# Alexander-H-Liu/End-to-end-ASR-Pytorch

Hardware: AMD Instinct MI355X
Metric: audio frames/sec training (LAS+CTC, LibriSpeech 80-mel) (higher is better)
Workload: dtype f32; 1 GPU; cfg3: {"B": 32, "T": 1600, "D": 80, "V": 5000, "L": 64}; global_batch=32, parallelism=dp1

## Files before the change

### end-to-end-asr-pytorch_amd/_lib.py

```python
import ctypes
import os

_HERE = os.path.dirname(os.path.abspath(__file__))
LIB_PATH = os.path.join(_HERE, "csrc", "libasrk.so")

c_int, c_i64, c_f32, c_vp, c_sz = (ctypes.c_int, ctypes.c_int64, ctypes.c_float, ctypes.c_void_p,
                                   ctypes.c_size_t)
c_f64 = ctypes.c_double

SIGNATURES = {
    "asrk_version": (c_int, []),
    "asrk_strerror": (ctypes.c_char_p, [c_int]),
    "asrk_init": (c_int, [c_int]),
    "asrk_profile_enable": (None, [c_int]),
    "asrk_profile_families": (None, [ctypes.c_uint]),
    "asrk_profile_reset": (None, []),
    "asrk_profile_get": (c_int, [c_int, ctypes.POINTER(ctypes.c_double), ctypes.POINTER(c_i64)]),
    "asrk_profile_get_work": (c_int, [c_int, ctypes.POINTER(ctypes.c_double)]),
    "asrk_gemm_f32": (c_int, [c_int, c_int, c_int, c_int, c_int, c_f32, c_vp, c_int, c_vp, c_int,
                              c_f32, c_vp, c_int, c_vp, c_vp, c_int, c_int, c_vp, c_sz, c_vp]),
    "asrk_gemm_ws_bytes": (c_sz, [c_int, c_int, c_int, c_int]),
    "asrk_gemm_takes_split": (c_int, [c_int, c_int, c_int, c_int]),
    "asrk_gemm_plan_info": (c_int, [c_int, c_int, c_int, c_int, c_int, c_int, c_int, c_int, c_int, c_f32, c_int, c_int,
                                    c_int, c_vp]),
    "asrk_split_panel_bytes": (ctypes.c_size_t, [c_int, c_int, c_int]),
    "asrk_split_panel_f32": (c_int, [c_vp, c_int, c_int, c_int, c_int, c_vp, c_int, c_vp]),
    "asrk_gemm_panels_f32": (c_int, [c_int, c_int, c_int, c_f32, c_vp, c_int, c_int, c_int, c_int,
                                     c_vp, c_int, c_int, c_int, c_int, c_f32, c_vp, c_int, c_vp, c_vp, c_int, c_vp]),
    "asrk_gemm_panels_splitk_ws_bytes": (c_sz, [c_int, c_int, c_int]),
    "asrk_gemm_panels_splitk_f32": (c_int, [c_int, c_int, c_int, c_f32, c_vp, c_int, c_int, c_int, c_int,
                                            c_vp, c_int, c_int, c_int, c_int, c_f32, c_vp, c_int, c_vp, c_vp, c_int,
                                            c_vp, c_sz, c_int, c_vp]),
    "asrk_copy3d_f32": (c_int, [c_vp, c_vp, c_int, c_int, c_int, c_i64, c_i64, c_i64, c_i64, c_int,
                                c_vp]),
    "asrk_colsum_f32": (c_int, [c_vp, c_int, c_int, c_int, c_vp, c_int, c_vp]),
    "asrk_tanh_fwd_f32": (c_int, [c_vp, c_vp, c_i64, c_vp]),
    "asrk_tanh_bwd_f32": (c_int, [c_vp, c_vp, c_vp, c_i64, c_vp]),
    "asrk_log_softmax_fwd_f32": (c_int, [c_vp, c_vp, c_int, c_int, c_int, c_vp]),
    "asrk_log_softmax_bwd_f32": (c_int, [c_vp, c_vp, c_vp, c_int, c_int, c_int, c_vp]),
    "asrk_cross_entropy_fwd_f32": (c_int, [c_vp, c_int, c_int, c_int, c_vp, c_int, c_vp, c_vp, c_vp]),
    "asrk_cross_entropy_bwd_f32": (c_int, [c_vp, c_int, c_int, c_int, c_vp, c_int, c_vp, c_vp, c_vp,
                                           c_vp]),
    "asrk_cross_entropy_ls_fwd_f32": (c_int, [c_vp, c_int, c_int, c_int, c_vp, c_int, c_vp, c_vp, c_vp, c_vp]),
    "asrk_cross_entropy_ls_bwd_f32": (c_int, [c_vp, c_int, c_int, c_int, c_vp, c_int, c_f32, c_vp, c_vp, c_vp,
                                              c_vp]),
    "asrk_ctc_prefix_score_f32": (c_int, [c_vp, c_vp, c_vp, c_vp, c_vp, c_vp, c_vp, c_int, c_int, c_int,
                                          c_int, c_int, c_int, c_f32, c_vp]),
    "asrk_ctc_prefix_score_multi_f32": (c_int, [c_vp, c_vp, c_vp, c_vp, c_vp, c_vp, c_vp, c_vp, c_vp, c_int, c_int,
                                                c_int, c_int, c_int, c_int, c_int, c_f32, c_vp]),
    "asrk_ctc_prefix_beam_ws_bytes": (c_sz, [c_int, c_int]),
    "asrk_ctc_prefix_beam_ws_offsets": (c_int, [c_int, c_int, c_int] + [ctypes.POINTER(c_i64)] * 6),
    "asrk_ctc_prefix_beam_f32": (c_int, [c_vp, c_int, c_int, c_vp, c_int, c_int, c_vp, c_f32, c_int, c_int, c_int,
                                         c_int, c_int, c_vp, c_sz, c_vp]),
    "asrk_ctc_prefix_beam_multi_ws_bytes": (c_sz, [c_int, c_int, c_int, ctypes.POINTER(c_sz)]),
    "asrk_ctc_prefix_beam_multi_f32": (c_int, [c_vp, c_i64, c_int, c_int, c_int, c_vp, c_int, c_int, c_vp, c_f32,
                                               c_vp, c_vp, c_int, c_vp, c_vp, c_vp, c_vp, c_sz, c_vp]),
    "asrk_fbank_frames_f32": (c_int, [c_vp, c_i64, c_vp, c_vp, c_int, c_int, c_int, c_int, c_f32, c_int,
                                      c_vp]),
    "asrk_power_spectrum_f32": (c_int, [c_vp, c_vp, c_i64, c_int, c_vp]),
    "asrk_log_floor_f32": (c_int, [c_vp, c_i64, c_f32, c_vp]),
    "asrk_delta_f32": (c_int, [c_vp, c_vp, c_vp, c_int, c_int, c_int, c_int, c_vp]),
    "asrk_cmvn_f32": (c_int, [c_vp, c_vp, c_int, c_int, c_f32, c_vp]),
    "asrk_transpose_f32": (c_int, [c_vp, c_vp, c_int, c_int, c_vp]),
    "asrk_fbank_frames_batch_f32": (c_int, [c_vp, c_int, c_i64, c_vp, c_vp, c_int, c_int, c_vp, c_vp, c_int, c_int,
                                            c_int, c_f32, c_f32, c_int, c_vp]),
    "asrk_delta_cmvn_batch_f32": (c_int, [c_vp, c_vp, c_int, c_int, c_vp, c_int, c_int, c_int, c_f32, c_vp, c_int,
                                          c_vp]),
    "asrk_fbank_logmel_batch_f32": (c_int, [c_vp, c_int, c_i64, c_vp, c_vp, c_int, c_int, c_vp, c_vp, c_vp, c_vp, c_vp,
                                            c_int, c_int, c_vp, c_int, c_int, c_int, c_f32, c_f32, c_int, c_f32, c_vp]),
    "asrk_fbank_frames_dither_f32": (c_int, [c_vp, c_i64, c_vp, c_vp, c_int, c_int, c_int, c_int, c_f32, c_int, c_f32,
                                             ctypes.c_uint64, c_vp]),
    "asrk_fbank_frames_batch_dither_f32": (c_int, [c_vp, c_int, c_i64, c_vp, c_vp, c_int, c_int, c_vp, c_vp, c_int,
                                                   c_int, c_int, c_f32, c_f32, c_int, c_f32, c_vp, c_vp]),
    "asrk_fbank_logmel_batch_dither_f32": (c_int, [c_vp, c_int, c_i64, c_vp, c_vp, c_int, c_int, c_vp, c_vp, c_vp, c_vp,
                                                   c_vp, c_int, c_int, c_vp, c_int, c_int, c_int, c_f32, c_f32, c_int,
                                                   c_f32, c_f32, c_vp, c_vp]),
    "asrk_spec_augment_f32": (c_int, [c_vp, c_vp, c_int, c_int, c_int, c_int, c_int, c_vp, c_vp, c_int, c_int, c_f32,
                                      c_vp]),
    "asrk_resample_rows_f32": (c_int, [c_vp, c_int, c_i64, c_vp, c_vp, c_vp, c_vp, c_int, c_vp, c_vp, c_int, c_vp, c_i64,
                                       c_f32, c_vp]),
    "asrk_reverb_mix_ws_bytes": (c_sz, [c_int, c_i64]),
    "asrk_reverb_mix_f32": (c_int, [c_vp, c_int, c_i64, c_vp, c_vp, c_vp, c_i64, c_vp, c_vp, c_vp, c_vp, c_int, c_vp,
                                    c_vp, c_vp, c_i64, c_vp, c_vp, c_vp, c_int, c_vp, c_i64, c_f32, c_vp, c_sz, c_vp]),
    "asrk_lstm_ws_bytes": (c_sz, []),
    "asrk_lstm_xchg_bytes": (c_sz, [c_int, c_int, c_int, c_int, c_int, c_int]),
    "asrk_lstm_plan_workgroups": (c_int, [c_int, c_int, c_int, c_int, c_int, c_int]),
    "asrk_lstm_plan_info": (c_int, [c_int, c_int, c_int, c_int, c_int, c_int, c_int, c_vp]),
    "asrk_lstm_rec_fwd_f32": (c_int, [c_vp, c_vp, c_vp, c_vp, c_vp, c_int, c_int, c_int, c_int,
                                      c_vp, c_int, c_vp, c_int, c_vp]),
    "asrk_lstm_rec_bwd_f32": (c_int, [c_vp, c_vp, c_vp, c_vp, c_vp, c_int, c_int, c_int, c_int,
                                      c_vp, c_int, c_vp, c_vp, c_int, c_vp]),
    "asrk_lstm_rec_fwd_pyr_f32": (c_int, [c_vp, c_vp, c_vp, c_vp, c_vp, c_int, c_int, c_int, c_int,
                                          c_vp, c_int, c_vp, c_vp, c_int, c_int, c_int, c_vp]),
    "asrk_lstm_rec_fwd_len_f32": (c_int, [c_vp, c_vp, c_vp, c_vp, c_vp, c_vp, c_int, c_int, c_int, c_int,
                                          c_vp, c_int, c_vp, c_vp, c_int, c_int, c_int, c_vp]),
    "asrk_lstm_rec_bwd_pyr_f32": (c_int, [c_vp, c_vp, c_vp, c_vp, c_vp, c_int, c_int, c_int, c_int,
                                          c_vp, c_int, c_vp, c_vp, c_int, c_int, c_int, c_vp]),
    "asrk_lstm_plan_is_bf": (c_int, [c_int, c_int, c_int, c_int, c_int, c_int]),
    "asrk_lstm_rec_fwd_pyr_panel_f32": (c_int, [c_vp, c_vp, c_vp, c_vp, c_vp, c_int, c_int, c_int, c_int,
                                                c_vp, c_int, c_vp, c_vp, c_int, c_int, c_vp, c_int, c_vp]),
    "asrk_lstm_rec_bwd_pyr_panel_f32": (c_int, [c_vp, c_vp, c_vp, c_vp, c_vp, c_int, c_int, c_int, c_int,
                                                c_vp, c_int, c_vp, c_vp, c_int, c_int, c_vp, c_vp, c_int, c_vp]),
    "asrk_gru_rec_fwd_f32": (c_int, [c_vp, c_vp, c_vp, c_vp, c_int, c_int, c_int, c_int,
                                     c_vp, c_int, c_vp, c_vp, c_int, c_int, c_int, c_vp]),
    "asrk_gru_rec_bwd_f32": (c_int, [c_vp, c_vp, c_vp, c_vp, c_vp, c_int, c_int, c_int, c_int,
                                     c_vp, c_int, c_vp, c_vp, c_int, c_int, c_int, c_vp]),
    "asrk_lstm_check_error": (c_int, [c_vp, c_vp]),
    "asrk_loc_conv_fwd_f32": (c_int, [c_vp, c_vp, c_vp, c_int, c_int, c_int, c_int, c_int, c_vp]),
    "asrk_loc_conv_bwd_f32": (c_int, [c_vp, c_vp, c_vp, c_vp, c_vp, c_int, c_int, c_int, c_int, c_int,
                                      c_vp]),
    "asrk_attn_energy_fwd_f32": (c_int, [c_int, c_vp, c_vp, c_vp, c_vp, c_vp, c_vp, c_vp, c_vp, c_vp,
                                         c_int, c_int, c_int, c_int, c_int, c_f32, c_vp]),
    "asrk_attn_energy_bwd_f32": (c_int, [c_int, c_vp, c_vp, c_vp, c_vp, c_vp, c_vp, c_vp, c_vp, c_vp,
                                         c_vp, c_vp, c_vp, c_vp, c_vp, c_int, c_int, c_int, c_int,
                                         c_int, c_f32, c_vp]),
    "asrk_attn_context_fwd_f32": (c_int, [c_vp, c_vp, c_vp, c_int, c_int, c_int, c_i64, c_vp]),
    "asrk_attn_context_bwd_f32": (c_int, [c_vp, c_vp, c_vp, c_int, c_int, c_int, c_i64, c_vp]),
    "asrk_lstm_cell_fwd_f32": (c_int, [c_vp, c_vp, c_vp, c_vp, c_int, c_int, c_vp]),
    "asrk_lstm_cell_bwd_f32": (c_int, [c_vp, c_vp, c_vp, c_vp, c_vp, c_vp, c_int, c_int, c_vp]),
    "asrk_gru_cell_fwd_f32": (c_int, [c_vp, c_vp, c_i64, c_i64, c_vp, c_i64, c_vp, c_i64, c_int, c_int, c_vp]),
    "asrk_gru_cell_bwd_f32": (c_int, [c_vp, c_vp, c_i64, c_i64, c_vp, c_i64, c_vp, c_i64, c_vp, c_vp, c_i64,
                                      c_int, c_int, c_vp]),
    "asrk_embedding_fwd_f32": (c_int, [c_vp, c_vp, c_vp, c_i64, c_int, c_int, c_vp]),
    "asrk_embedding_bwd_f32": (c_int, [c_vp, c_vp, c_vp, c_i64, c_int, c_int, c_vp]),
    "asrk_emb_fuse_bwd_ws_bytes": (c_sz, [c_int] * 6),
    "asrk_emb_fuse_fwd_f32": (c_int, [c_vp, c_int, c_vp, c_vp, c_int, c_vp, c_int, c_int, c_f32, c_int, c_int, c_vp,
                                      c_vp, c_vp]),
    "asrk_emb_fuse_bwd_f32": (c_int, [c_vp, c_vp, c_int, c_vp, c_vp, c_int, c_vp, c_int, c_int, c_f32, c_vp, c_int,
                                      c_int, c_vp, c_vp, c_vp, c_vp, c_vp, c_sz, c_vp]),
    "asrk_cos_emb_loss_fwd_f32": (c_int, [c_vp, c_vp, c_i64, c_vp, c_int, c_int, c_int, c_vp, c_vp, c_vp, c_vp]),
    "asrk_cos_emb_loss_bwd_f32": (c_int, [c_vp, c_vp, c_i64, c_vp, c_int, c_int, c_int, c_vp, c_vp, c_vp, c_vp, c_vp]),
    "asrk_cos_emb_table_grad_f32": (c_int, [c_vp, c_vp, c_int, c_int, c_i64, c_vp, c_vp]),
    "asrk_nll_loss_fwd_f32": (c_int, [c_vp, c_int, c_int, c_int, c_vp, c_int, c_vp, c_vp]),
    "asrk_nll_loss_bwd_f32": (c_int, [c_int, c_int, c_int, c_vp, c_int, c_vp, c_vp, c_vp]),
    "asrk_l2norm_fwd_f32": (c_int, [c_vp, c_vp, c_vp, c_int, c_int, c_f32, c_vp]),
    "asrk_l2norm_bwd_f32": (c_int, [c_vp, c_vp, c_vp, c_vp, c_int, c_int, c_f32, c_vp]),
    "asrk_layer_norm_fwd_f32": (c_int, [c_vp, c_vp, c_vp, c_vp, c_vp, c_vp, c_int, c_int, c_f32, c_vp]),
    "asrk_layer_norm_bwd_f32": (c_int, [c_vp, c_vp, c_vp, c_vp, c_vp, c_vp, c_vp, c_vp, c_int, c_int,
                                        c_vp]),
    "asrk_dropout_f32": (c_int, [c_vp, c_vp, c_i64, c_f32, ctypes.c_uint64, ctypes.c_uint64, c_vp]),
    "asrk_adadelta_step_f32": (c_int, [c_vp, c_vp, c_vp, c_vp, c_i64, c_f64, c_f64, c_f64, c_vp, c_vp]),
    "asrk_adadelta_multi_f32": (c_int, [c_int, c_vp, c_vp, c_vp, c_vp, c_vp, c_f64, c_f64, c_f64, c_vp, c_vp]),
    "asrk_adam_multi_f32": (c_int, [c_int, c_vp, c_vp, c_vp, c_vp, c_vp, c_f64, c_f64, c_f64, c_f64, c_i64,
                                    c_vp, c_vp]),
    "asrk_adam_step_f32": (c_int, [c_vp, c_vp, c_vp, c_vp, c_i64, c_f64, c_f64, c_f64, c_f64, c_i64, c_vp,
                                   c_vp]),
    "asrk_token_crop_i64": (c_int, [c_vp, c_i64, c_int, c_int, c_i64, c_i64, c_int, c_vp, c_i64, c_vp, c_vp]),
    "asrk_edit_distance_i64": (c_int, [c_vp, c_i64, c_vp, c_vp, c_i64, c_vp, c_int, c_int, c_vp, c_vp]),
    "asrk_grad_norm_ws_bytes": (c_sz, [c_int, c_vp]),
    "asrk_grad_norm_multi_f32": (c_int, [c_int, c_vp, c_vp, c_f32, c_vp, c_vp, c_vp, c_sz, c_vp]),
    "asrk_fill_f32": (c_int, [c_vp, c_i64, c_f32, c_vp]),
    "asrk_topk_f32": (c_int, [c_vp, c_int, c_int, c_int, c_int, c_vp, c_vp, c_vp]),
    "asrk_beam_select_f32": (c_int, [c_vp] * 4 + [c_int] * 6 + [c_vp] * 19 + [c_vp]),
    "asrk_gather_rows_multi_f32": (c_int, [c_int, c_vp, c_vp, c_vp, c_vp, c_vp, c_vp, c_vp, c_int, c_vp]),
    "asrk_conv_out_size": (c_int, [c_int, c_int, c_int, c_int]),
    "asrk_im2col_f32": (c_int, [c_vp, c_vp] + [c_int] * 10 + [c_i64] * 4 + [c_vp]),
    "asrk_im2col_ld_f32": (c_int, [c_vp, c_vp] + [c_int] * 11 + [c_i64] * 4 + [c_vp]),
    "asrk_col2im_f32": (c_int, [c_vp, c_vp] + [c_int] * 10 + [c_i64] * 4 + [c_vp]),
    "asrk_im2col_cl_f32": (c_int, [c_vp, c_vp] + [c_int] * 10 + [c_i64] * 4 + [c_vp]),
    "asrk_col2im_cl_f32": (c_int, [c_vp, c_vp] + [c_int] * 10 + [c_i64] * 4 + [c_vp]),
    "asrk_conv_weight_reorder_f32": (c_int, [c_vp, c_vp, c_int, c_int, c_int, c_int, c_vp]),
    "asrk_conv3x3_supported": (c_int, [c_int] * 4),
    "asrk_conv3x3_plan_info": (c_int, [c_int] * 6 + [c_vp, c_int]),
    "asrk_conv3x3_weight_f32": (c_int, [c_vp, c_vp, c_int, c_int, c_int, c_vp]),
    "asrk_conv3x3_f32": (c_int, [c_vp] * 5 + [c_int] * 6 + [c_vp]),
    "asrk_conv3x3_wgrad_ws_bytes": (c_sz, [c_int] * 5),
    "asrk_conv3x3_wgrad_f32": (c_int, [c_vp] * 5 + [c_int] * 5 + [c_vp, c_sz, c_vp]),
    "asrk_conv3x3_first_supported": (c_int, [c_int] * 4),
    "asrk_conv3x3_first_f32": (c_int, [c_vp] * 4 + [c_int] * 5 + [c_i64] * 4 + [c_int, c_vp]),
    "asrk_conv3x3_len_f32": (c_int, [c_vp] * 5 + [c_int] * 6 + [c_vp]),
    "asrk_conv3x3_first_len_f32": (c_int, [c_vp] * 5 + [c_int] * 5 + [c_i64] * 4 + [c_int, c_vp]),
    "asrk_im2col_ld_len_f32": (c_int, [c_vp] * 3 + [c_int] * 11 + [c_i64] * 4 + [c_vp]),
    "asrk_im2col_cl_len_f32": (c_int, [c_vp] * 3 + [c_int] * 10 + [c_i64] * 4 + [c_vp]),
    "asrk_conv_zero_tail_f32": (c_int, [c_vp, c_vp, c_int, c_int, c_i64, c_vp]),
    "asrk_conv3x3_first_wgrad_ws_bytes": (c_sz, [c_int] * 5),
    "asrk_conv3x3_first_wgrad_f32": (c_int, [c_vp] * 5 + [c_int] * 5 + [c_i64] * 4 + [c_vp, c_sz, c_vp]),
    "asrk_relu_fwd_f32": (c_int, [c_vp, c_i64, c_vp]),
    "asrk_relu_bwd_f32": (c_int, [c_vp, c_vp, c_vp, c_i64, c_vp]),
    "asrk_maxpool2x2_fwd_f32": (c_int, [c_vp, c_vp, c_vp] + [c_int] * 4 + [c_i64] * 4 + [c_vp]),
    "asrk_maxpool2x2_bwd_f32": (c_int, [c_vp, c_vp, c_vp] + [c_int] * 4 + [c_i64] * 4 + [c_vp]),
    "asrk_speller_plan": (c_int, [c_vp, ctypes.POINTER(c_int), ctypes.POINTER(c_int)]),
    "asrk_speller_plan_info": (c_int, [c_vp, ctypes.POINTER(c_int)]),
    "asrk_speller_ctx_variant": (c_int, [c_vp, ctypes.POINTER(c_int)]),
    "asrk_speller_fwd_f32": (c_int, [c_vp, c_vp]),
    "asrk_speller_bwd_f32": (c_int, [c_vp, c_vp, c_vp]),
    "asrk_speller_step_f32": (c_int, [c_vp, c_int, c_vp, c_i64, c_vp, c_vp]),
    "asrk_speller_dvalue_f32": (c_int, [c_vp, c_i64, c_i64, c_vp, c_i64, c_i64, c_vp, c_int, c_int, c_int,
                                        c_int, c_vp]),
    "asrk_joint_score_f32": (c_int, [c_vp, c_vp, c_vp, c_vp, c_vp, c_vp, c_int, c_int, c_int, c_f64, c_f64,
                                     c_f64, c_vp]),
    "asrk_lstm_cell_fused_f32": (c_int, [c_vp, c_i64, c_int, c_vp, c_vp, c_vp, c_vp, c_vp, c_vp, c_vp, c_vp, c_int,
                                         c_int, c_vp]),
    "asrk_transpose_ld_f32": (c_int, [c_vp, c_i64, c_vp, c_i64, c_int, c_int, c_vp]),
    "asrk_flac_info": (c_int, [ctypes.c_char_p, ctypes.POINTER(c_int), ctypes.POINTER(c_int), ctypes.POINTER(c_int),
                               ctypes.POINTER(c_i64), c_vp]),
    "asrk_flac_decode_i32": (c_int, [ctypes.c_char_p, c_vp, c_i64, ctypes.POINTER(c_i64)]),
    "asrk_ctc_loss_fwd_f32": (c_int, [c_vp, c_i64, c_i64, c_int, c_int, c_int, c_vp, c_i64, c_int,
                                      c_vp, c_vp, c_int, c_vp, c_vp, c_vp, c_vp, c_vp]),
    "asrk_ctc_loss_bwd_f32": (c_int, [c_vp, c_i64, c_i64, c_int, c_int, c_int, c_vp, c_i64, c_int,
                                      c_vp, c_vp, c_int, c_vp, c_vp, c_vp, c_vp, c_vp, c_vp, c_i64,
                                      c_i64, c_vp]),
    "asrk_ctc_loss_fwd_ex_f32": (c_int, [c_vp, c_i64, c_i64, c_int, c_int, c_int, c_vp, c_i64, c_int,
                                         c_vp, c_vp, c_int, c_vp, c_vp, c_vp, c_vp, c_int, c_vp, c_vp, c_vp]),
    "asrk_ctc_loss_bwd_ex_f32": (c_int, [c_vp, c_i64, c_i64, c_int, c_int, c_int, c_vp, c_i64, c_int,
                                         c_vp, c_vp, c_int, c_vp, c_vp, c_vp, c_vp, c_vp, c_vp, c_i64,
                                         c_i64, c_int, c_vp]),
    "asrk_ctc_align_ws_bytes": (c_sz, [c_int, c_int, c_int, c_int]),
    "asrk_ctc_align_f32": (c_int, [c_vp, c_i64, c_i64, c_int, c_int, c_int, c_vp, c_i64, c_int, c_vp, c_vp, c_int,
                                   c_int, c_vp, c_vp, c_vp, c_vp, c_vp, c_vp, c_sz, c_vp]),
}

_lib = None


class AsrkError(RuntimeError):
    pass


def load():
    global _lib
    if _lib is not None:
        return _lib
    if not os.path.exists(LIB_PATH):
        raise AsrkError(
            "libasrk.so not found at %s - build it with `python __graft_entry__.py` "
            "(hipcc --offload-arch=gfx950). There is no CPU fallback for the product path." % LIB_PATH)
    try:
        import torch
    except ImportError:
        pass
    lib = ctypes.CDLL(LIB_PATH)
    for name, (res, args) in SIGNATURES.items():
        fn = getattr(lib, name)
        fn.restype = res
        fn.argtypes = args
    _lib = lib
    return lib


def strerror(rc):
    return load().asrk_strerror(int(rc)).decode()


def check(rc, what=""):
    if rc != 0:
        raise AsrkError("%s failed: %s (rc=%d)" % (what or "asrk call", strerror(rc), rc))
```

### end-to-end-asr-pytorch_amd/csrc/lstm_rec.hip

```cpp
#include "lstm_rec_common.h"

extern "C" int asrk_cu_count_(void);
extern "C" size_t asrk_split_panel_stride_(int rows, int K);

using namespace asrk_rec;

namespace {

__global__ __launch_bounds__(256) void sentinel_fill_kernel(u32x4 *__restrict__ p, size_t n16) {
    const u32x4 v = {0xFFFFFFFFu, 0xFFFFFFFFu, 0xFFFFFFFFu, 0xFFFFFFFFu};
    for (size_t base = (size_t)blockIdx.x * 1024; base < n16; base += (size_t)gridDim.x * 1024) {
#pragma unroll
        for (int u = 0; u < 4; ++u) {
            const size_t i = base + u * 256 + threadIdx.x;
            if (i < n16) p[i] = v;
        }
    }
}

inline int sentinel_fill(void *xchg, size_t floats, hipStream_t s) {
    const size_t n16 = floats / 4;
    if (n16 * 4 != floats || (reinterpret_cast<uintptr_t>(xchg) & 15) != 0)
        return (int)hipMemsetAsync(xchg, 0xFF, floats * 4, s);
    hipLaunchKernelGGL(sentinel_fill_kernel, dim3(2048), dim3(256), 0, s, reinterpret_cast<u32x4 *>(xchg), n16);
    return (int)hipGetLastError();
}

__global__ __launch_bounds__(256) void sentinel_fill_tail_kernel(u32x4 *__restrict__ x, int groups, int T, int r0,
                                                                 unsigned step16) {
    const u32x4 v = {0xFFFFFFFFu, 0xFFFFFFFFu, 0xFFFFFFFFu, 0xFFFFFFFFu};
    const unsigned n = (unsigned)(T - r0) * step16;
    const int g = blockIdx.y;
    u32x4 *q = x + ((size_t)g * T + r0) * step16;
    for (unsigned i = blockIdx.x * 256 + threadIdx.x; i < n; i += gridDim.x * 256) q[i] = v;
}

inline int sentinel_fill_tail(void *xchg, int groups, int T, size_t step_floats, hipStream_t s) {
    const int r0 = std::max(0, T - 2);
    const unsigned step16 = (unsigned)(step_floats / 4);
    const unsigned n = (unsigned)(T - r0) * step16;
    hipLaunchKernelGGL(sentinel_fill_tail_kernel, dim3(std::max(1u, std::min(64u, (n + 1023) / 1024)), groups), dim3(256),
                       0, s, reinterpret_cast<u32x4 *>(xchg), groups, T, r0, step16);
    return (int)hipGetLastError();
}

inline int canary_words(int nwg) { return ((4 * nwg + 63) / 64) * 64; }

unsigned long long *g_dbg_buf = nullptr;
int g_dbg_steps = 0;

inline void chunk_groups(int ndir, int nbg, int gmax, int &ndir_l, int &nbg_l, int &launches) {
    ndir_l = gmax >= ndir ? ndir : 1;
    nbg_l = std::max(1, std::min(nbg, gmax / ndir_l));
    launches = ((ndir + ndir_l - 1) / ndir_l) * ((nbg + nbg_l - 1) / nbg_l);
}

FwdPlan plan_fwd(int T, int B, int H, int ndir, int ncu, int flags) {
    const AsrkKnobs &kn = asrk_knobs_();
    FwdPlan best{};
    best.ok = false;
    long best_cost = -1;
    const int kg = (H + 15) / 16;
    const int kgw_need = (kg + 3) / 4;
    const int KGW = kgw_need <= 4 ? 4 : kgw_need <= 8 ? 8 : kgw_need <= 16 ? 16 : 0;
    if (!KGW) return best;
    const int HP = KGW * 4 * 16 + 8;
    static const int combos[6][2] = {{1, 1}, {1, 2}, {2, 1}, {2, 2}, {1, 4}, {4, 1}};
    const int oc = 1;
    for (auto &c : combos) {
        const int MT = c[0], NT = c[1];
        if (kn.is_set(kn.fwd_mt) && kn.fwd_mt != MT) continue;
        if (kn.is_set(kn.fwd_nt) && kn.fwd_nt != NT) continue;
        const int U = 4 * MT, BG = 16 * NT;
        const int nwg = (H + U - 1) / U, nbg = (B + BG - 1) / BG;
        const long wgs = (long)ndir * nbg * nwg;
        if (wgs > (long)ncu * oc) continue;
        const size_t red1 = (size_t)4 * MT * NT * RED_PITCH * 16;
        size_t lds = (size_t)MT * 16 * HP * 4 + 2 * red1 + 16;
        int db = 1;
        const size_t lds_cap = (size_t)158 * 1024 / (wgs > ncu ? oc : 1);
        if (lds > lds_cap) {
            lds -= red1;
            db = 0;
        }
        if (lds > lds_cap) continue;
        const long cost = (long)MT * NT * 1000 - nbg;
        if (best_cost < 0 || cost < best_cost) {
            best_cost = cost;
            best = FwdPlan{MT, NT, KGW, U, nwg, nbg, BG, HP, kg, db, lds,
                           (size_t)ndir * nbg * T * ((size_t)kg * NT * 256 + canary_words(nwg)), true,
                           ndir, nbg};
        }
    }
    if (best.ok) {
        const bool no_bf = (flags & ASRK_REC_F32_MFMA) != 0;
        if (!no_bf && best.MT == 2 && (H == 512 || H == 1024)) {
            const size_t wl = (size_t)2 * 2 * (H / 32) * 1024;
            const size_t red1 = (size_t)4 * 2 * best.NT * RED_PITCH * 16;
            size_t lds = wl + 2 * red1 + 16;
            int db = 1;
            if (lds > (size_t)158 * 1024) { lds -= red1; db = 0; }
            if (lds <= (size_t)158 * 1024) {
                best.bf = 1;
                best.db = db;
                best.lds = lds;
                best.xfloats = (size_t)ndir * best.nbg * T *
                               ((size_t)(H / 32) * best.NT * 3 * 256 + canary_words(best.nwg));
            }
            const bool no16 = kn.get(kn.rec_bf_mt4, 1) == 0;
            const int nbg16 = (B + 15) / 16;
            if (best.bf && !no16 && H == 1024 && (long)ndir * nbg16 * (H / 16) <= ncu) {
                best.MT = 4; best.NT = 1; best.U = 16; best.BG = 16;
                best.nwg = H / 16; best.nbg = nbg16; best.ndir_l = ndir; best.nbg_l = nbg16;
                best.db = 0;
                best.lds = (size_t)4 * (H / 32) * 1024 + (size_t)4 * 4 * RED_PITCH * 16 + 16;
                best.xfloats = (size_t)ndir * nbg16 * T * ((size_t)(H / 32) * 3 * 256 + canary_words(best.nwg));
            }
        }
        return best;
    }
    for (auto &c : combos) {
        const int MT = c[0], NT = c[1];
        const int U = 4 * MT, BG = 16 * NT;
        const int nwg = (H + U - 1) / U, nbg = (B + BG - 1) / BG;
        if (nwg > ncu) continue;
        const size_t red1 = (size_t)4 * MT * NT * RED_PITCH * 16;
        size_t lds = (size_t)MT * 16 * HP * 4 + 2 * red1 + 16;
        int db = 1;
        if (lds > (size_t)158 * 1024) { lds -= red1; db = 0; }
        if (lds > (size_t)158 * 1024) continue;
        int ndir_l, nbg_l, launches;
        chunk_groups(ndir, nbg, ncu / nwg, ndir_l, nbg_l, launches);
        const long cost = (long)launches * MT * NT * 1000;
        if (best_cost < 0 || cost < best_cost) {
            best_cost = cost;
            best = FwdPlan{MT, NT, KGW, U, nwg, nbg, BG, HP, kg, db, lds,
                           (size_t)ndir_l * nbg_l * T * ((size_t)kg * NT * 256 + canary_words(nwg)), true,
                           ndir_l, nbg_l};
        }
    }
    return best;
}


inline size_t bwd_lds(int kg, int UB, int NT, int RK, int &HPb, int &KP) {
    const int CH = bwd_ring_kgroups(NT, RK);
    HPb = ((kg - RK + CH - 1) / CH) * CH * 16;
    KP = 4 * HPb + 8;
    return (size_t)UB * KP * 4 + (size_t)HPb * 4 + (size_t)2 * 4 * NT * RED_PITCH * 16 + 16;
}
inline int bwd_rk_options(int kg, int H, int NT, int (&opts)[2]) {
    opts[0] = 0;
    const int kg_plain = (H & 15) ? kg - 1 : kg;
    if (NT == 1 && 32 + bwd_ring_kgroups(1, 32) <= kg_plain) {
        opts[1] = 32;
        return 2;
    }
    return 1;
}

BwdPlan plan_bwd(int T, int B, int H, int ndir, int ncu, int flags) {
    const AsrkKnobs &kn = asrk_knobs_();
    BwdPlan best{};
    best.ok = false;
    const int kg = (H + 15) / 16;
    static const int ubs[3] = {16, 8, 4};
    static const int nts[3] = {1, 2, 4};
    const int oc = 1;
    for (int UB : ubs) {
        if (kn.is_set(kn.bwd_ub) && kn.bwd_ub != UB) continue;
        for (int NT : nts) {
            if (kn.is_set(kn.bwd_nt) && kn.bwd_nt != NT) continue;
            int rks[2];
            const int nrk = bwd_rk_options(kg, H, NT, rks);
            for (int ri = 0; ri < nrk; ++ri) {
                const int RK = rks[ri];
                int HPb, KP;
                const size_t lds = bwd_lds(kg, UB, NT, RK, HPb, KP);
                const int BG = 16 * NT;
                const int nwg = (H + UB - 1) / UB, nbg = (B + BG - 1) / BG;
                const long wgs = (long)ndir * nbg * nwg;
                if (wgs > (long)ncu * oc) continue;
                if (lds > (size_t)158 * 1024 / (wgs > ncu ? oc : 1)) continue;
                best = BwdPlan{NT, UB, nwg, nbg, BG, HPb, KP, kg, lds,
                               (size_t)ndir * nbg * T * ((size_t)4 * kg * NT * 256 + canary_words(nwg)),
                               true, ndir, nbg, RK};
                const bool no_bf = (flags & ASRK_REC_F32_MFMA) != 0;
                if (!no_bf && NT == 1 && UB == 16 && BG == 16 && (H == 512 || H == 1024)) {
                    const int KS = H / 32, KL = H == 1024 ? 11 : 0;
                    best.bf = 1;
                    best.lds = (size_t)4 * KL * 3 * 1024 + (size_t)2 * 4 * RED_PITCH * 16 + 2 * 6144 + 16;
                    best.xfloats = (size_t)ndir * nbg * T * ((size_t)4 * KS * 3 * 256 + canary_words(nwg));
                }
                return best;
            }
        }
    }
    long best_cost = -1;
    for (int UB : ubs) {
        for (int NT : nts) {
            int rks[2];
            const int nrk = bwd_rk_options(kg, H, NT, rks);
            for (int ri = 0; ri < nrk; ++ri) {
                const int RK = rks[ri];
                int HPb, KP;
                const size_t lds = bwd_lds(kg, UB, NT, RK, HPb, KP);
                const int BG = 16 * NT;
                const int nwg = (H + UB - 1) / UB, nbg = (B + BG - 1) / BG;
                if (nwg > ncu || lds > (size_t)158 * 1024) continue;
                int ndir_l, nbg_l, launches;
                chunk_groups(ndir, nbg, ncu / nwg, ndir_l, nbg_l, launches);
                const long cost = (long)launches * NT * 1000 + (16 / UB);
                if (best_cost < 0 || cost < best_cost) {
                    best_cost = cost;
                    best = BwdPlan{NT, UB, nwg, nbg, BG, HPb, KP, kg, lds,
                                   (size_t)ndir_l * nbg_l * T * ((size_t)4 * kg * NT * 256 + canary_words(nwg)),
                                   true, ndir_l, nbg_l, RK};
                }
            }
        }
    }
    return best;
}

int rec_fwd_impl(bool gru, float *G, const float *whh_f, const float *whh_r, float *Y, float *C, int T, int B,
                 int H, int ndir, void *xchg, int xchg_prefilled, void *ws, float *Y2, int pyr_mode,
                 int pyr_rate, int flags, void *stream, const int64_t *lens = nullptr, void *x2_panel = nullptr);
int rec_bwd_impl(bool gru, float *gates, const float *whh_f, const float *whh_r, const float *C,
                 const float *dY, int T, int B, int H, int ndir, void *xchg, int xchg_prefilled, void *ws,
                 float *db, int pyr_mode, int pyr_rate, int flags, void *stream, void *dg_panel = nullptr,
                 void *dgt_panel = nullptr);

}


extern "C" void asrk_lstm_set_debug_(void *buf, int steps) {
    g_dbg_buf = reinterpret_cast<unsigned long long *>(buf);
    g_dbg_steps = steps;
}

extern "C" size_t asrk_lstm_ws_bytes(void) { return WS_WORDS * sizeof(unsigned); }

extern "C" int asrk_lstm_plan_workgroups(int T, int B, int H, int ndir, int backward, int flags) {
    int info[ASRK_LSTM_PLAN_INFO_LEN];
    return asrk_lstm_plan_info(T, B, H, ndir, backward, flags, 0, info) == ASRK_OK ? info[11] : 0;
}

extern "C" size_t asrk_lstm_xchg_bytes(int T, int B, int H, int ndir, int backward, int flags) {
    int info[ASRK_LSTM_PLAN_INFO_LEN];
    if (asrk_lstm_plan_info(T, B, H, ndir, backward, flags, 0, info) != ASRK_OK) return 0;
    return ((size_t)info[13] << 31) | (size_t)info[12];
}

extern "C" int asrk_lstm_rec_fwd_f32(float *G, const float *whh_f, const float *whh_r, float *Y,
                                     float *C, int T, int B, int H, int ndir, void *xchg,
                                     int xchg_prefilled, void *ws, int flags, void *stream) {
    return asrk_lstm_rec_fwd_pyr_f32(G, whh_f, whh_r, Y, C, T, B, H, ndir, xchg, xchg_prefilled, ws, nullptr,
                                     0, 1, flags, stream);
}

extern "C" int asrk_lstm_rec_fwd_pyr_f32(float *G, const float *whh_f, const float *whh_r, float *Y,
                                         float *C, int T, int B, int H, int ndir, void *xchg,
                                         int xchg_prefilled, void *ws, float *Y2, int pyr_mode,
                                         int pyr_rate, int flags, void *stream) {
    if (!C) return ASRK_EINVAL;
    return rec_fwd_impl(false, G, whh_f, whh_r, Y, C, T, B, H, ndir, xchg, xchg_prefilled, ws, Y2, pyr_mode,
                        pyr_rate, flags, stream);
}

extern "C" int asrk_lstm_rec_fwd_pyr_panel_f32(float *G, const float *whh_f, const float *whh_r, float *Y,
                                               float *C, int T, int B, int H, int ndir, void *xchg,
                                               int xchg_prefilled, void *ws, float *Y2, int pyr_mode,
                                               int pyr_rate, void *x2_panel, int flags, void *stream) {
    if (!C || !x2_panel) return ASRK_EINVAL;
    return rec_fwd_impl(false, G, whh_f, whh_r, Y, C, T, B, H, ndir, xchg, xchg_prefilled, ws, Y2, pyr_mode,
                        pyr_rate, flags, stream, nullptr, x2_panel);
}

extern "C" int asrk_lstm_plan_is_bf(int T, int B, int H, int ndir, int backward, int flags) {
    int info[ASRK_LSTM_PLAN_INFO_LEN];
    return asrk_lstm_plan_info(T, B, H, ndir, backward, flags, 0, info) == ASRK_OK ? info[0] : 0;
}

extern "C" int asrk_lstm_plan_info(int T, int B, int H, int ndir, int backward, int flags, int ncu, int *info) {
    if (!info || ncu < 0) return ASRK_EINVAL;
    for (int i = 0; i < ASRK_LSTM_PLAN_INFO_LEN; ++i) info[i] = 0;
    if (flags < 0) return ASRK_EINVAL;
    if (T < 0 || B <= 0 || H <= 0 || (ndir != 1 && ndir != 2)) return ASRK_EINVAL;
    if (T == 0) return ASRK_OK;
    if (H % 4 != 0) return ASRK_ESHAPE;
    if (ncu == 0) ncu = asrk_cu_count_();
    if (ncu <= 0) return ASRK_EDEVICE;
    int nbg_l, ndir_l, nbg;
    size_t xbytes;
    if (backward) {
        const BwdPlan pl = plan_bwd(T, B, H, ndir, ncu, flags);
        if (!pl.ok) return ASRK_ESHAPE;
        info[0] = pl.bf; info[1] = pl.UB; info[2] = pl.NT; info[3] = pl.bf ? 0 : pl.RK; info[4] = 0;
        info[8] = pl.nwg; info[10] = (int)pl.lds;
        ndir_l = pl.ndir_l; nbg_l = pl.nbg_l; nbg = pl.nbg; xbytes = pl.xfloats * 4;
    } else {
        const FwdPlan pl = plan_fwd(T, B, H, ndir, ncu, flags);
        if (!pl.ok) return ASRK_ESHAPE;
        info[0] = pl.bf; info[1] = pl.MT; info[2] = pl.NT; info[3] = pl.bf ? H / 128 : pl.KGW; info[4] = pl.db;
        info[8] = pl.nwg; info[10] = (int)pl.lds;
        ndir_l = pl.ndir_l; nbg_l = pl.nbg_l; nbg = pl.nbg; xbytes = pl.xfloats * 4;
    }
    info[5] = ((ndir + ndir_l - 1) / ndir_l) * ((nbg + nbg_l - 1) / nbg_l);
    info[6] = ndir_l; info[7] = nbg_l; info[9] = nbg;
    info[11] = ndir_l * nbg_l * info[8];
    info[12] = (int)(xbytes & 0x7fffffffu); info[13] = (int)(xbytes >> 31);
    info[14] = ncu;
    return ASRK_OK;
}

extern "C" int asrk_lstm_rec_fwd_len_f32(float *G, const float *whh_f, const float *whh_r, float *Y,
                                         float *C, const int64_t *lens, int T, int B, int H, int ndir, void *xchg,
                                         int xchg_prefilled, void *ws, float *Y2, int pyr_mode,
                                         int pyr_rate, int flags, void *stream) {
    if (!C || !lens) return ASRK_EINVAL;
    return rec_fwd_impl(false, G, whh_f, whh_r, Y, C, T, B, H, ndir, xchg, xchg_prefilled, ws, Y2, pyr_mode,
                        pyr_rate, flags, stream, lens);
}

extern "C" int asrk_gru_rec_fwd_f32(float *G, const float *whh_f, const float *whh_r, float *Y, int T, int B,
                                    int H, int ndir, void *xchg, int xchg_prefilled, void *ws, float *Y2,
                                    int pyr_mode, int pyr_rate, int flags, void *stream) {
    return rec_fwd_impl(true, G, whh_f, whh_r, Y, nullptr, T, B, H, ndir, xchg, xchg_prefilled, ws, Y2,
                        pyr_mode, pyr_rate, flags, stream);
}

extern "C" int asrk_gru_rec_bwd_f32(float *gates, const float *whh_f, const float *whh_r, const float *Y,
                                    const float *dY, int T, int B, int H, int ndir, void *xchg,
                                    int xchg_prefilled, void *ws, float *db, int pyr_mode, int pyr_rate,
                                    int flags, void *stream) {
    return rec_bwd_impl(true, gates, whh_f, whh_r, Y, dY, T, B, H, ndir, xchg, xchg_prefilled, ws, db,
                        pyr_mode, pyr_rate, flags, stream);
}

namespace {
int rec_fwd_impl(bool gru, float *G, const float *whh_f, const float *whh_r, float *Y, float *C, int T, int B,
                 int H, int ndir, void *xchg, int xchg_prefilled, void *ws, float *Y2, int pyr_mode,
                 int pyr_rate, int flags, void *stream, const int64_t *lens, void *x2_panel) {
    const AsrkKnobs &kn = asrk_knobs_();
    if (flags < 0 || pyr_mode < 0 || pyr_mode > 2 || pyr_rate < 1) return ASRK_EINVAL;
    const bool y2_empty = pyr_mode == 1 && T / pyr_rate == 0;
    if (pyr_mode != 0 && !Y2 && !y2_empty) return ASRK_EINVAL;
    if (T < 0 || B <= 0 || H <= 0 || (ndir != 1 && ndir != 2)) return ASRK_EINVAL;
    if (T == 0) return ASRK_OK;
    if (!G || !whh_f || (ndir == 2 && !whh_r) || !Y || (!gru && !C) || !ws || !xchg) return ASRK_EINVAL;
    if (H % 4 != 0) return ASRK_ESHAPE;
    if ((reinterpret_cast<uintptr_t>(xchg) & 15) != 0) return ASRK_EINVAL;
    const int ncu = asrk_cu_count_();
    if (ncu <= 0) return ASRK_EDEVICE;
    FwdPlan pl = plan_fwd(T, B, H, ndir, ncu, flags);
    if (!pl.ok) return ASRK_ESHAPE;
    hipStream_t s = (hipStream_t)stream;
    RecFwdArgs a;
    a.G = G; a.whh[0] = whh_f; a.whh[1] = ndir == 2 ? whh_r : whh_f;
    a.Y = Y; a.C = C; a.X = reinterpret_cast<float *>(xchg);
    a.err = reinterpret_cast<unsigned *>(ws);
    a.T = T; a.B = B; a.H = H; a.ldg = ndir * 4 * H; a.ldy = ndir * H;
    a.U = pl.U; a.nwg = pl.nwg; a.BG = pl.BG; a.HP = pl.HP; a.kgp = pl.kgp;
    a.canw = canary_words(pl.nwg);
    a.poll_mode = kn.get(kn.fwd_poll, 0);
    a.poll_mode |= (kn.get(kn.fwd_presleep, 8) & 0xff) << 8;
    a.dbg = g_dbg_buf; a.dbg_steps = kn.is_set(kn.dbg_noload) ? -1 : g_dbg_steps;
    a.Y2 = pyr_mode ? Y2 : nullptr; a.pyr_mode = pyr_mode; a.pyr_rate = pyr_rate;
    a.lens = lens;
    a.P2 = nullptr; a.p2_stride = 0;
    if (x2_panel) {
        if (!pl.bf || pyr_mode == 2 || lens || (ndir * H) % 8 != 0 || (reinterpret_cast<uintptr_t>(x2_panel) & 15))
            return ASRK_ESHAPE;
        const int r = pyr_mode == 1 ? pyr_rate : 1;
        a.P2 = reinterpret_cast<unsigned char *>(x2_panel);
        a.p2_stride = asrk_split_panel_stride_((T / r) * B, r * ndir * H);
        if (pyr_mode == 0) { a.pyr_rate = 1; }
    }
    const bool one_launch = pl.ndir_l >= ndir && pl.nbg_l >= pl.nbg;
    a.rearm = (flags & ASRK_REC_REARM) && one_launch ? 1 : 0;
    asrk_prof_begin_(PROF_LSTM_FWD, s);
    int rc = ASRK_OK;
    bool first = true;
    for (int d0 = 0; d0 < ndir && rc == ASRK_OK; d0 += pl.ndir_l)
        for (int g0 = 0; g0 < pl.nbg && rc == ASRK_OK; g0 += pl.nbg_l) {
            a.ndir = std::min(pl.ndir_l, ndir - d0);
            a.nbg = std::min(pl.nbg_l, pl.nbg - g0);
            a.dir0 = d0; a.bg0 = g0;
            if (!(first && xchg_prefilled)) { const int frc = sentinel_fill(xchg, pl.xfloats, s); if (frc) return frc; }
            first = false;
            const int grid = a.ndir * a.nbg * pl.nwg;
            rc = pl.bf ? launch_fwd_bf(gru, a, pl, H, grid, s) : launch_fwd_f32(gru, a, pl, grid, s);
        }
    if (rc == ASRK_OK && (flags & ASRK_REC_REARM)) {
        const int frc = a.rearm ? sentinel_fill_tail(xchg, ndir * pl.nbg, T, pl.xfloats / ((size_t)ndir * pl.nbg * T), s)
                                : sentinel_fill(xchg, pl.xfloats, s);
        if (frc) rc = frc;
    }
    asrk_prof_end_(PROF_LSTM_FWD, s);
    return rc;
}
}

extern "C" int asrk_lstm_rec_bwd_f32(float *gates, const float *whh_f, const float *whh_r,
                                     const float *C, const float *dY, int T, int B, int H, int ndir,
                                     void *xchg, int xchg_prefilled, void *ws, float *db, int flags, void *stream) {
    return asrk_lstm_rec_bwd_pyr_f32(gates, whh_f, whh_r, C, dY, T, B, H, ndir, xchg, xchg_prefilled, ws, db,
                                     0, 1, flags, stream);
}

extern "C" int asrk_lstm_rec_bwd_pyr_f32(float *gates, const float *whh_f, const float *whh_r,
                                         const float *C, const float *dY, int T, int B, int H, int ndir,
                                         void *xchg, int xchg_prefilled, void *ws, float *db,
                                         int pyr_mode, int pyr_rate, int flags, void *stream) {
    return rec_bwd_impl(false, gates, whh_f, whh_r, C, dY, T, B, H, ndir, xchg, xchg_prefilled, ws, db,
                        pyr_mode, pyr_rate, flags, stream);
}

extern "C" int asrk_lstm_rec_bwd_pyr_panel_f32(float *gates, const float *whh_f, const float *whh_r,
                                               const float *C, const float *dY, int T, int B, int H, int ndir,
                                               void *xchg, int xchg_prefilled, void *ws, float *db,
                                               int pyr_mode, int pyr_rate, void *dg_panel, void *dgt_panel, int flags,
                                               void *stream) {
    if (!dg_panel && !dgt_panel) return ASRK_EINVAL;
    return rec_bwd_impl(false, gates, whh_f, whh_r, C, dY, T, B, H, ndir, xchg, xchg_prefilled, ws, db,
                        pyr_mode, pyr_rate, flags, stream, dg_panel, dgt_panel);
}

namespace {
int rec_bwd_impl(bool gru, float *gates, const float *whh_f, const float *whh_r, const float *C,
                 const float *dY, int T, int B, int H, int ndir, void *xchg, int xchg_prefilled, void *ws,
                 float *db, int pyr_mode, int pyr_rate, int flags, void *stream, void *dg_panel, void *dgt_panel) {
    const AsrkKnobs &kn = asrk_knobs_();
    if (flags < 0 || pyr_mode < 0 || pyr_mode > 2 || pyr_rate < 1) return ASRK_EINVAL;
    const bool dy_empty = pyr_mode == 1 && T / pyr_rate == 0;
    if (T < 0 || B <= 0 || H <= 0 || (ndir != 1 && ndir != 2)) return ASRK_EINVAL;
    if (T == 0) return ASRK_OK;
    if (!gates || !whh_f || (ndir == 2 && !whh_r) || !C || (!dY && !dy_empty) || !ws || !xchg) return ASRK_EINVAL;
    if (H % 4 != 0) return ASRK_ESHAPE;
    if ((reinterpret_cast<uintptr_t>(xchg) & 15) != 0) return ASRK_EINVAL;
    const int ncu = asrk_cu_count_();
    if (ncu <= 0) return ASRK_EDEVICE;
    BwdPlan pl = plan_bwd(T, B, H, ndir, ncu, flags);
    if (!pl.ok) return ASRK_ESHAPE;
    hipStream_t s = (hipStream_t)stream;
    RecBwdArgs a;
    a.G = gates; a.whh[0] = whh_f; a.whh[1] = ndir == 2 ? whh_r : whh_f;
    a.C = C; a.dY = dY; a.X = reinterpret_cast<float *>(xchg);
    a.err = reinterpret_cast<unsigned *>(ws);
    a.T = T; a.B = B; a.H = H; a.ldg = ndir * 4 * H; a.ldy = ndir * H;
    a.UB = pl.UB; a.nwg = pl.nwg; a.BG = pl.BG; a.HPb = pl.HPb; a.KP = pl.KP;
    a.kgp = pl.kgp; a.canw = canary_words(pl.nwg);
    a.poll_mode = kn.get(kn.bwd_poll, 1);
    if (kn.is_set(kn.bwd_presleep)) a.poll_mode |= (kn.bwd_presleep & 0xff) << 8;
    a.dbg = g_dbg_buf; a.dbg_steps = kn.is_set(kn.dbg_noload) ? -1 : g_dbg_steps;
    a.db = db;
    a.pyr_mode = pyr_mode; a.pyr_rate = pyr_rate;
    a.PG = nullptr; a.pg_stride = 0;
    if (dg_panel) {
        if (!pl.bf || gru || (reinterpret_cast<uintptr_t>(dg_panel) & 15)) return ASRK_ESHAPE;
        a.PG = reinterpret_cast<unsigned char *>(dg_panel);
        a.pg_stride = asrk_split_panel_stride_(T * B, ndir * 4 * H);
    }
    a.PT = nullptr; a.pt_stride = 0;
    if (dgt_panel) {
        if (!pl.bf || gru || B % 16 != 0 || (reinterpret_cast<uintptr_t>(dgt_panel) & 15)) return ASRK_ESHAPE;
        a.PT = reinterpret_cast<unsigned char *>(dgt_panel);
        a.pt_stride = asrk_split_panel_stride_(ndir * 4 * H, T * B);
    }
    const bool one_launch = pl.ndir_l >= ndir && pl.nbg_l >= pl.nbg;
    a.rearm = (flags & ASRK_REC_REARM) && one_launch ? 1 : 0;
    a.no_dg = (flags & ASRK_REC_BWD_NO_DG) && (dg_panel || dgt_panel) ? 1 : 0;
    if (db) ASRK_HIP(hipMemsetAsync(db, 0, (size_t)ndir * 4 * H * sizeof(float), s));
    asrk_prof_begin_(PROF_LSTM_BWD, s);
    int rc = ASRK_OK;
    bool first = true;
    for (int d0 = 0; d0 < ndir && rc == ASRK_OK; d0 += pl.ndir_l)
        for (int g0 = 0; g0 < pl.nbg && rc == ASRK_OK; g0 += pl.nbg_l) {
            a.ndir = std::min(pl.ndir_l, ndir - d0);
            a.nbg = std::min(pl.nbg_l, pl.nbg - g0);
            a.dir0 = d0; a.bg0 = g0;
            if (!(first && xchg_prefilled)) { const int frc = sentinel_fill(xchg, pl.xfloats, s); if (frc) return frc; }
            first = false;
            const int grid = a.ndir * a.nbg * pl.nwg;
            rc = pl.bf ? launch_bwd_bf(gru, a, pl, grid, s) : launch_bwd_f32(gru, a, pl, grid, s);
        }
    if (rc == ASRK_OK && (flags & ASRK_REC_REARM)) {
        const int frc = a.rearm ? sentinel_fill_tail(xchg, ndir * pl.nbg, T, pl.xfloats / ((size_t)ndir * pl.nbg * T), s)
                                : sentinel_fill(xchg, pl.xfloats, s);
        if (frc) rc = frc;
    }
    asrk_prof_end_(PROF_LSTM_BWD, s);
    return rc;
}
}

extern "C" int asrk_lstm_check_error(void *ws, void *stream) {
    if (!ws) return ASRK_EINVAL;
    hipStream_t s = (hipStream_t)stream;
    unsigned e = 0;
    unsigned *errp = reinterpret_cast<unsigned *>(ws);
    ASRK_HIP(hipMemcpyAsync(&e, errp, sizeof(unsigned), hipMemcpyDeviceToHost, s));
    ASRK_HIP(hipStreamSynchronize(s));
    if (e != 0) {
        ASRK_HIP(hipMemsetAsync(errp, 0, sizeof(unsigned), s));
        return ASRK_ETIMEOUT;
    }
    return ASRK_OK;
}
```

### end-to-end-asr-pytorch_amd/csrc/lstm_rec_bwd_bf.hip

```cpp
#include "lstm_rec_common.h"

namespace asrk_rec {
namespace {

template <bool GRU, int KS, int NREG>
__global__ __launch_bounds__(256) void lstm_rec_bwd_bf_kernel(RecBwdArgs p) {
    extern __shared__ __attribute__((aligned(16))) float smem[];
    constexpr int CH = 8;
    constexpr int KL = KS - NREG;
    constexpr int KQ = KS / 4;
    static_assert(KS >= CH, "ring longer than the slice");
    static_assert(KS % 4 == 0, "unit range of a wave is a whole number of k-steps");
    const int tid = threadIdx.x, lane = tid & 63, wave = __builtin_amdgcn_readfirstlane(tid >> 6);
    const int ngroups = p.ndir * p.nbg;
    const int group = blockIdx.x % ngroups, wg = blockIdx.x / ngroups;
    const int dir = p.dir0 + group % p.ndir, bg = p.bg0 + group / p.ndir;
    const int u0 = wg * 16, b0 = bg * 16;
    const int nb = min(16, p.B - b0);
    const int H = p.H;

    unsigned char *Wl = reinterpret_cast<unsigned char *>(smem);
    f32x4 *red = reinterpret_cast<f32x4 *>(Wl + (size_t)4 * KL * 3 * 1024);
    unsigned char *stage = reinterpret_cast<unsigned char *>(red + 2 * 4 * RED_PITCH);
    unsigned char *stage_t = stage + 4 * 3 * 2 * 16 * 16;
    int *abort_flag = reinterpret_cast<int *>(stage_t + 4 * 3 * 2 * 16 * 16);

    const int m16 = lane & 15, q4 = lane >> 4;
    bf16x8_t areg[NREG > 0 ? NREG : 1][3];
    {
        const float *W = p.whh[dir];
#pragma unroll
        for (int js = 0; js < KS; ++js) {
            const int gate = js / KQ;
            const bool live = !GRU || gate < 3;
            unsigned h0[8], h1[8], h2[8];
#pragma unroll
            for (int e = 0; e < 8; ++e) {
                const int j = (wave * KQ + js % KQ) * 32 + q4 * 8 + e;
                split3(live ? W[((size_t)gate * H + j) * H + u0 + m16] : 0.f, h0[e], h1[e], h2[e]);
            }
            u32x4 w0, w1, w2;
#pragma unroll
            for (int q = 0; q < 4; ++q) {
                w0[q] = h0[2 * q] | (h0[2 * q + 1] << 16);
                w1[q] = h1[2 * q] | (h1[2 * q + 1] << 16);
                w2[q] = h2[2 * q] | (h2[2 * q + 1] << 16);
            }
            if (js < NREG) {
                areg[js][0] = __builtin_bit_cast(bf16x8_t, w0);
                areg[js][1] = __builtin_bit_cast(bf16x8_t, w1);
                areg[js][2] = __builtin_bit_cast(bf16x8_t, w2);
            } else {
                unsigned char *d = Wl + ((size_t)((wave * KL + (js - NREG)) * 3) * 64 + lane) * 16;
                *reinterpret_cast<u32x4 *>(d) = w0;
                *reinterpret_cast<u32x4 *>(d + 1024) = w1;
                *reinterpret_cast<u32x4 *>(d + 2048) = w2;
            }
        }
        if (tid == 0) *abort_flag = 0;
    }
    __syncthreads();
    const unsigned char *a_lds = Wl + ((size_t)(wave * KL * 3) * 64 + lane) * 16;

    const int ul = tid & 15, bl = tid >> 4;
    const int c_unit = u0 + ul, c_b = b0 + bl;
    const bool c_valid = bl < nb;
    const int c_red = (red_slot((ul >> 2) * 16 + bl)) * 4 + (ul & 3);
    float dc_carry = 0.f;
    float dbsum[4] = {0.f, 0.f, 0.f, 0.f};

    const size_t gate_floats = (size_t)KS * 3 * 256;
    const size_t data_floats = 4 * gate_floats;
    const size_t step_floats = data_floats + (size_t)p.canw;
    float *xgroup = p.X + (size_t)group * p.T * step_floats;
    const unsigned voff = (m16 < nb && p.dbg_steps != -1) ? (unsigned)(lane * 16) : 0x7ff00000u;
    const unsigned frag_base = (unsigned)(wave * KQ * 3 * 1024);
    auto frag_off = [](int js) { return (unsigned)(((js / KQ) * KS + js % KQ) * 3 * 1024); };
    const int can_lo = wave * p.nwg, can_cnt = p.nwg;
    unsigned char *st_w = stage + (ul >> 3) * 256 + bl * 16 + (ul & 7) * 2;
    unsigned char *st_t = stage_t + (bl >> 3) * 256 + ul * 16 + (bl & 7) * 2;
    int pt_src[2];
    size_t pt_dst[2];
    int pt_half[2];
    bool pt_on[2];
#pragma unroll
    for (int i = 0; i < 2; ++i) {
        const int idx = tid + 256 * i;
        const int u = idx & 15, rest = idx >> 4, hb = rest & 1, gp = rest >> 1;
        const int r = gp / 3, pl = gp - r * 3;
        pt_on[i] = idx < 384;
        pt_src[i] = ((gp * 2 + hb) * 16 + u) * 16;
        const int row = (dir * 4 + r) * H + u0 + u;
        pt_dst[i] = (size_t)(row >> 6) * p.pt_stride + (size_t)pl * 1024 + (row & 63) * 16;
        pt_half[i] = hb;
    }
    const int xks = u0 >> 5, xq4 = (u0 & 31) >> 3;
    int ch_src[2], pg_row[2];
    unsigned ch_dst[2];
    size_t pg_col[2];
    bool ch_on[2];
#pragma unroll
    for (int i = 0; i < 2; ++i) {
        const int idx = lane + 64 * i;
        const int nl = idx / 24, c = idx - nl * 24, n = wave * 4 + nl;
        const int r = c / 6, pl = (c % 6) >> 1, half = c & 1;
        ch_on[i] = idx < 96 && n < nb;
        ch_src[i] = ((r * 3 + pl) * 2 + half) * 256 + n * 16;
        ch_dst[i] = (unsigned)((((r * KS + xks) * 3 + pl) * 64 + (xq4 + half) * 16 + n) * 16);
        pg_row[i] = b0 + n;
        pg_col[i] = (size_t)((((dir * 4 + r) * H + u0 + half * 8) >> 3) * 3 + pl) * 1024;
    }

    for (int s = 0; s < p.T; ++s) {
        const int t = dir == 0 ? p.T - 1 - s : s;
        const int tp = dir == 0 ? t - 1 : t + 1;

        float vi = 0.f, vf = 0.f, vg = 0.f, vo = 0.f, vc = 0.f, vcp = 0.f, vdy = 0.f;
        if (c_valid) {
            const size_t row = (size_t)t * p.B + c_b;
            const float *g = p.G + row * p.ldg + dir * 4 * H + c_unit;
            vi = g[0];
            vf = g[(size_t)H];
            vg = g[(size_t)2 * H];
            vo = g[(size_t)3 * H];
            vc = p.C[row * p.ldy + dir * H + c_unit];
            if (p.pyr_mode == 0) {
                vdy = p.dY[row * p.ldy + dir * H + c_unit];
            } else {
                const int r = p.pyr_rate, tq = t / r, tr = t - tq * r;
                if (p.pyr_mode == 1 ? tq < p.T / r : tr == 0) {
                    const size_t ld2 = p.pyr_mode == 1 ? (size_t)r * p.ldy : (size_t)p.ldy;
                    const size_t off = p.pyr_mode == 1 ? (size_t)tr * p.ldy : 0;
                    vdy = p.dY[((size_t)tq * p.B + c_b) * ld2 + off + dir * H + c_unit];
                }
            }
            if (tp >= 0 && tp < p.T) vcp = p.C[((size_t)tp * p.B + c_b) * p.ldy + dir * H + c_unit];
        }

        f32x4 acc[3];
        acc[0] = acc[1] = acc[2] = f32x4{0.f, 0.f, 0.f, 0.f};

        auto mfma6 = [&](const bf16x8_t (&a)[3], const u32x4 (&b)[3]) {
            acc[0] = __builtin_amdgcn_mfma_f32_16x16x32_bf16(a[2], __builtin_bit_cast(bf16x8_t, b[0]), acc[0], 0, 0, 0);
            acc[1] = __builtin_amdgcn_mfma_f32_16x16x32_bf16(a[1], __builtin_bit_cast(bf16x8_t, b[1]), acc[1], 0, 0, 0);
            acc[2] = __builtin_amdgcn_mfma_f32_16x16x32_bf16(a[0], __builtin_bit_cast(bf16x8_t, b[2]), acc[2], 0, 0, 0);
            acc[0] = __builtin_amdgcn_mfma_f32_16x16x32_bf16(a[1], __builtin_bit_cast(bf16x8_t, b[0]), acc[0], 0, 0, 0);
            acc[1] = __builtin_amdgcn_mfma_f32_16x16x32_bf16(a[0], __builtin_bit_cast(bf16x8_t, b[1]), acc[1], 0, 0, 0);
            acc[2] = __builtin_amdgcn_mfma_f32_16x16x32_bf16(a[0], __builtin_bit_cast(bf16x8_t, b[0]), acc[2], 0, 0, 0);
        };
        auto a_frag = [&](bf16x8_t (&a)[3], int js) {
            if (js < NREG) {
                a[0] = areg[js][0]; a[1] = areg[js][1]; a[2] = areg[js][2];
            } else {
                const unsigned char *q = a_lds + (size_t)(js - NREG) * 3 * 1024;
                a[0] = *reinterpret_cast<const bf16x8_t *>(q);
                a[1] = *reinterpret_cast<const bf16x8_t *>(q + 1024);
                a[2] = *reinterpret_cast<const bf16x8_t *>(q + 2048);
            }
        };

        REC_STAMP(0);
        if (s > 0) {
            __amdgpu_buffer_rsrc_t rs = __builtin_amdgcn_make_buffer_rsrc(
                (void *)(xgroup + (size_t)(s - 1) * step_floats), 0, (int)(step_floats * 4), 0x00020000);
            u32x4 bf[CH][3];
            unsigned spins = 0;
            unsigned long long t0 = 0;
            bool ok = true;
            for (int z = (p.poll_mode >> 8) & 0xff; z > 0; z -= 8) __builtin_amdgcn_s_sleep(8);
            ok = wait_canaries(reinterpret_cast<const unsigned *>(
                                       xgroup + (size_t)(s - 1) * step_floats + data_floats) + can_lo,
                               can_cnt, p.err, lane, p.poll_mode);
            REC_STAMP(7);
            bool bad = false;
            if (ok) {
#pragma unroll
                for (int c = 0; c < CH; ++c)
#pragma unroll
                    for (int pl = 0; pl < 3; ++pl)
                        bf[c][pl] = __builtin_amdgcn_raw_buffer_load_b128(
                            rs, voff, frag_base + frag_off(c) + (unsigned)(pl * 1024), 0);
                __builtin_amdgcn_sched_barrier(0);
                REC_STAMP(1);
#pragma unroll
                for (int js = 0; js < KS; ++js) {
                    bf16x8_t a[3];
                    a_frag(a, js);
                    mfma6(a, bf[js % CH]);
                    __builtin_amdgcn_sched_barrier(0);
                    if (js + CH < KS) {
#pragma unroll
                        for (int pl = 0; pl < 3; ++pl)
                            bf[js % CH][pl] = __builtin_amdgcn_raw_buffer_load_b128(
                                rs, voff, frag_base + frag_off(js + CH) + (unsigned)(pl * 1024), 0);
                        __builtin_amdgcn_sched_barrier(0);
                    }
                }
            }
            bad = any_nan(acc[0] + acc[1] + acc[2]);
            if (ok && __any(bad)) {
                acc[0] = acc[1] = acc[2] = f32x4{0.f, 0.f, 0.f, 0.f};
#pragma unroll
                for (int c0 = 0; c0 < KS; c0 += CH) {
                    while (ok) {
#pragma unroll
                        for (int c = 0; c < CH; ++c)
#pragma unroll
                            for (int pl = 0; pl < 3; ++pl)
                                bf[c][pl] = __builtin_amdgcn_raw_buffer_load_b128(
                                    rs, voff, frag_base + frag_off(c0 + c) + (unsigned)(pl * 1024), 16);
                        __builtin_amdgcn_sched_barrier(0);
                        bool b2 = false;
#pragma unroll
                        for (int c = 0; c < CH; ++c)
#pragma unroll
                            for (int pl = 0; pl < 3; ++pl) b2 |= has_sentinel(__builtin_bit_cast(f32x4, bf[c][pl]));
                        if (!__any(b2)) break;
                        if (!spin_ok(spins, t0, p.err, lane)) ok = false;
                    }
                    if (ok) {
#pragma unroll
                        for (int c = 0; c < CH; ++c) {
                            bf16x8_t a[3];
                            a_frag(a, c0 + c);
                            mfma6(a, bf[c]);
                        }
                    }
                }
            }
            if (!ok && lane == 0) *abort_flag = 1;
        }
        REC_STAMP(2);
        f32x4 *redw = red + (s & 1) * 4 * RED_PITCH;
        redw[wave * RED_PITCH + red_slot(lane)] = acc[0] + acc[1] + acc[2];
        REC_STAMP(3);
        __syncthreads();
        if (*abort_flag) break;
        REC_STAMP(4);

        const float *redf = reinterpret_cast<const float *>(redw);
        float *xstep = xgroup + (size_t)s * step_floats;
        float dgs[4] = {0.f, 0.f, 0.f, 0.f}, xg[4] = {0.f, 0.f, 0.f, 0.f};
        if (c_valid) {
            float rec = 0.f;
#pragma unroll
            for (int w = 0; w < 4; ++w) rec += redf[w * RED_PITCH * 4 + c_red];
            if (GRU) {
                const float dh = vdy + rec + dc_carry;
                const float r = vi, z = vf, n = vg, hn = vo, hp = vcp;
                const float dn = dh * (1.f - z) * (1.f - n * n);
                const float dz = dh * (hp - n) * z * (1.f - z);
                const float dr = dn * hn * r * (1.f - r);
                dc_carry = dh * z;
                dgs[0] = dr; dgs[1] = dz; dgs[2] = dn; dgs[3] = dn * r;
                xg[0] = dr; xg[1] = dz; xg[2] = dn * r; xg[3] = 0.f;
            } else {
                const float dh = vdy + rec;
                const float tc = fast_tanh(vc);
                const float dcell = dh * vo * (1.f - tc * tc) + dc_carry;
                dc_carry = dcell * vf;
                dgs[0] = dcell * vg * vi * (1.f - vi);
                dgs[1] = dcell * vcp * vf * (1.f - vf);
                dgs[2] = dcell * vi * (1.f - vg * vg);
                dgs[3] = dh * tc * vo * (1.f - vo);
#pragma unroll
                for (int r = 0; r < 4; ++r) xg[r] = dgs[r];
            }
#pragma unroll
            for (int r = 0; r < 4; ++r) dbsum[r] += dgs[r];
        }
#pragma unroll
        for (int r = 0; r < 4; ++r) {
            unsigned h0, h1, h2;
            split3(xg[r], h0, h1, h2);
            *reinterpret_cast<unsigned short *>(st_w + (r * 3 + 0) * 512) = (unsigned short)h0;
            *reinterpret_cast<unsigned short *>(st_w + (r * 3 + 1) * 512) = (unsigned short)h1;
            *reinterpret_cast<unsigned short *>(st_w + (r * 3 + 2) * 512) = (unsigned short)h2;
            if (!GRU && p.PT) {
                *reinterpret_cast<unsigned short *>(st_t + (r * 3 + 0) * 512) = (unsigned short)h0;
                *reinterpret_cast<unsigned short *>(st_t + (r * 3 + 1) * 512) = (unsigned short)h1;
                *reinterpret_cast<unsigned short *>(st_t + (r * 3 + 2) * 512) = (unsigned short)h2;
            }
        }
        __builtin_amdgcn_fence(__ATOMIC_RELEASE, "wavefront");
        __builtin_amdgcn_wave_barrier();
        __builtin_amdgcn_fence(__ATOMIC_ACQUIRE, "wavefront");
        {
            __amdgpu_buffer_rsrc_t xrs = __builtin_amdgcn_make_buffer_rsrc(
                (void *)xstep, 0, (int)(step_floats * 4), 0x00020000);
            u32x4 v[2];
#pragma unroll
            for (int i = 0; i < 2; ++i)
                if (ch_on[i]) {
                    v[i] = *reinterpret_cast<const u32x4 *>(stage + ch_src[i]);
                    __builtin_amdgcn_raw_buffer_store_b128(v[i], xrs, ch_dst[i], 0, 16);
                }
            if (lane == 0)
                __hip_atomic_store(reinterpret_cast<unsigned *>(xstep + data_floats) + 4 * wg + wave,
                                   (unsigned)(s + 1), RLX_AGENT);
            if (!GRU && p.PG) {
#pragma unroll
                for (int i = 0; i < 2; ++i)
                    if (ch_on[i]) {
                        const int m = t * p.B + pg_row[i];
                        *reinterpret_cast<u32x4 *>(p.PG + (size_t)(m >> 6) * p.pg_stride + pg_col[i] + (m & 63) * 16) = v[i];
                    }
            }
        }
        REC_STAMP(5);
        if (c_valid && !p.no_dg) {
            float *g = p.G + ((size_t)t * p.B + c_b) * p.ldg + dir * 4 * H + c_unit;
#pragma unroll
            for (int r = 0; r < 4; ++r) g[(size_t)r * H] = dgs[r];
        }
        if (!GRU && p.PT) {
            __syncthreads();
#pragma unroll
            for (int i = 0; i < 2; ++i)
                if (pt_on[i]) {
                    const int c = (t * p.B + b0 + pt_half[i] * 8) >> 3;
                    *reinterpret_cast<u32x4 *>(p.PT + pt_dst[i] + (size_t)c * 3072) =
                        *reinterpret_cast<const u32x4 *>(stage_t + pt_src[i]);
                }
        }
        if (p.rearm && s >= 2)
            rearm_region(xgroup + (size_t)(s - 2) * step_floats, step_floats, wg, p.nwg, tid, (int)blockDim.x);
        REC_STAMP(6);
    }
    if (p.db && !*abort_flag) {
        __syncthreads();
        float *sdb = reinterpret_cast<float *>(red);
#pragma unroll
        for (int r = 0; r < 4; ++r) sdb[tid * 4 + r] = c_valid ? dbsum[r] : 0.f;
        __syncthreads();
        if (tid < 64) {
            const int u = tid & 15, r = tid >> 4;
            float a = 0.f;
            for (int b = 0; b < 16; ++b) a += sdb[(b * 16 + u) * 4 + r];
            unsafeAtomicAdd(p.db + (size_t)dir * 4 * H + (size_t)r * H + u0 + u, a);
        }
    }
}

template <bool GRU, int KS, int NREG>
int launch_bwd_bf(const RecBwdArgs &a, int grid, size_t lds, hipStream_t s) {
    auto kern = lstm_rec_bwd_bf_kernel<GRU, KS, NREG>;
    ASRK_HIP(hipFuncSetAttribute(reinterpret_cast<const void *>(kern),
                                 hipFuncAttributeMaxDynamicSharedMemorySize, (int)lds));
    hipLaunchKernelGGL(kern, dim3(grid), dim3(256), lds, s, a);
    ASRK_LAUNCH_CHECK();
    return ASRK_OK;
}

}

int launch_bwd_bf(bool gru, const RecBwdArgs &a, const BwdPlan &pl, int grid, hipStream_t s) {
    if (a.H == 1024) return gru ? launch_bwd_bf<true, 32, 21>(a, grid, pl.lds, s) : launch_bwd_bf<false, 32, 21>(a, grid, pl.lds, s);
    return gru ? launch_bwd_bf<true, 16, 16>(a, grid, pl.lds, s) : launch_bwd_bf<false, 16, 16>(a, grid, pl.lds, s);
}

}
```

### end-to-end-asr-pytorch_amd/csrc/lstm_rec_common.h

```cpp
#pragma once
#include "common.h"
#include "knobs.h"
#include <algorithm>
#include <cstdlib>

namespace asrk_rec {

constexpr int WS_WORDS = 1024;
constexpr unsigned SENT = 0xFFFFFFFFu;
constexpr unsigned long long TIMEOUT_TICKS = 300000000ull;

struct RecFwdArgs {
    float *G;
    const float *whh[2];
    float *Y, *C;
    float *X;
    unsigned *err;
    int T, B, H, ndir, ldg, ldy;
    int U, nwg, nbg, BG, HP, kgp, canw, poll_mode;
    int dir0, bg0;
    unsigned long long *dbg;
    int dbg_steps;
    float *Y2;
    int pyr_mode, pyr_rate;
    const int64_t *lens;
    int rearm;
    unsigned char *P2;
    size_t p2_stride;
};

struct RecBwdArgs {
    float *G;
    const float *whh[2];
    const float *C, *dY;
    float *X;
    unsigned *err;
    int T, B, H, ndir, ldg, ldy;
    int UB, nwg, nbg, BG, HPb, KP, kgp, canw, poll_mode;
    int dir0, bg0;
    unsigned long long *dbg;
    int dbg_steps;
    float *db;
    int pyr_mode, pyr_rate;
    int rearm;
    int no_dg;
    unsigned char *PG;
    size_t pg_stride;
    unsigned char *PT;
    size_t pt_stride;
};

#define REC_STAMP_W(ph)                                                                       \
    do {                                                                                      \
        if (p.dbg && blockIdx.x == 0 && lane == 0 && s < p.dbg_steps && wave < 4)             \
            p.dbg[((size_t)s * 4 + wave) * 8 + (ph)] = __builtin_readcyclecounter();          \
    } while (0)
#define REC_STAMP(ph)                                                                         \
    do {                                                                                      \
        if (p.dbg && blockIdx.x == 0 && lane == 0 && s < p.dbg_steps)                         \
            p.dbg[((size_t)s * 4 + wave) * 8 + (ph)] = __builtin_readcyclecounter();          \
    } while (0)

__device__ __forceinline__ bool has_sentinel(const f32x4 &v) {
    const u32x4 u = __builtin_bit_cast(u32x4, v);
    return (u[0] == SENT) | (u[1] == SENT) | (u[2] == SENT) | (u[3] == SENT);
}

__device__ __forceinline__ bool any_nan(const f32x4 &v) {
    return (v[0] != v[0]) | (v[1] != v[1]) | (v[2] != v[2]) | (v[3] != v[3]);
}

__device__ __forceinline__ bool spin_ok(unsigned &spins, unsigned long long &t0, unsigned *err,
                                        int lane) {
    __builtin_amdgcn_s_sleep(1);
    if ((++spins & 127u) == 0) {
        const unsigned long long now = wall_clock64();
        if (t0 == 0) t0 = now;
        const unsigned e = __hip_atomic_load(err, RLX_AGENT);
        if (e != 0 || now - t0 > TIMEOUT_TICKS) {
            if (lane == 0) __hip_atomic_store(err, 1u, RLX_AGENT);
            return false;
        }
    }
    return true;
}

__device__ __forceinline__ bool wait_canaries(const unsigned *cb, int cnt, unsigned *err, int lane,
                                              int mode) {
    const bool pipelined = mode & 1;
    unsigned spins = 0;
    unsigned long long t0 = 0;
    if (cnt > 128 || !pipelined) {
        for (;;) {
            bool good = true;
            for (int j = lane; j < cnt; j += 64) good &= (__hip_atomic_load(cb + j, RLX_AGENT) != SENT);
            if (__all(good)) return true;
            if (!spin_ok(spins, t0, err, lane)) return false;
        }
    }
    const bool a0 = lane < cnt, a1 = lane + 64 < cnt;
    const unsigned *p0 = cb + (a0 ? lane : 0), *p1 = cb + (a1 ? lane + 64 : 0);
    unsigned x0 = a0 ? __hip_atomic_load(p0, RLX_AGENT) : 0u, y0 = a1 ? __hip_atomic_load(p1, RLX_AGENT) : 0u;
    __builtin_amdgcn_s_sleep(3);
    unsigned x1 = a0 ? __hip_atomic_load(p0, RLX_AGENT) : 0u, y1 = a1 ? __hip_atomic_load(p1, RLX_AGENT) : 0u;
    __builtin_amdgcn_s_sleep(3);
    unsigned x2 = a0 ? __hip_atomic_load(p0, RLX_AGENT) : 0u, y2 = a1 ? __hip_atomic_load(p1, RLX_AGENT) : 0u;
    for (;;) {
        const bool good = (x0 != SENT) & (y0 != SENT);
        if (__all(good)) return true;
        x0 = x1; y0 = y1; x1 = x2; y1 = y2;
        if (!spin_ok(spins, t0, err, lane)) return false;
        __builtin_amdgcn_s_sleep(2);
        x2 = a0 ? __hip_atomic_load(p0, RLX_AGENT) : 0u;
        y2 = a1 ? __hip_atomic_load(p1, RLX_AGENT) : 0u;
    }
}

__host__ __device__ constexpr int bwd_ring_kgroups(int NT, int RK = 0) { return NT == 1 ? 8 : 16 / NT; }


__device__ __forceinline__ void rearm_region(float *region, size_t floats, int wg, int nwg, int tid, int nthreads) {
    const unsigned n16 = (unsigned)(floats >> 2);
    const unsigned per = (n16 + (unsigned)nwg - 1u) / (unsigned)nwg;
    const unsigned lo = (unsigned)wg * per, hi = min(lo + per, n16);
    u32x4 *q = reinterpret_cast<u32x4 *>(region);
    const u32x4 v = {SENT, SENT, SENT, SENT};
    for (unsigned i = lo + (unsigned)tid; i < hi; i += (unsigned)nthreads) q[i] = v;
}

__device__ __forceinline__ float fast_sigmoid(float x) {
    return __builtin_amdgcn_rcpf(1.0f + __expf(-x));
}
__device__ __forceinline__ float fast_tanh(float x) {
    return 1.0f - 2.0f * __builtin_amdgcn_rcpf(__expf(2.0f * x) + 1.0f);
}

constexpr int RED_PITCH = 72;
__device__ __forceinline__ int red_slot(int lane) { return lane + 2 * (lane >> 4); }

template <int ACC>
__device__ __forceinline__ f32x4 acc_sum(const f32x4 (&a)[ACC]) {
    f32x4 r = a[0];
#pragma unroll
    for (int i = 1; i < ACC; ++i) r += a[i];
    return r;
}


typedef __bf16 bf16x8_t __attribute__((ext_vector_type(8)));
typedef unsigned int u32x2 __attribute__((ext_vector_type(2)));

__device__ __forceinline__ void split3(float a, unsigned &b0, unsigned &b1, unsigned &b2) {
    const __bf16 h0 = (__bf16)a;
    const float r1 = a - (float)h0;
    const __bf16 h1 = (__bf16)r1;
    const __bf16 h2 = (__bf16)(r1 - (float)h1);
    b0 = __builtin_bit_cast(unsigned short, h0);
    b1 = __builtin_bit_cast(unsigned short, h1);
    b2 = __builtin_bit_cast(unsigned short, h2);
}

struct FwdPlan {
    int MT, NT, KGW, U, nwg, nbg, BG, HP, kgp, db;
    size_t lds, xfloats;
    bool ok;
    int ndir_l, nbg_l;
    int bf;
};


struct BwdPlan {
    int NT, UB, nwg, nbg, BG, HPb, KP, kgp;
    size_t lds, xfloats;
    bool ok;
    int ndir_l, nbg_l;
    int RK;
    int bf;
};


int launch_fwd_f32(bool gru, const RecFwdArgs &a, const FwdPlan &pl, int grid, hipStream_t s);
int launch_fwd_bf(bool gru, const RecFwdArgs &a, const FwdPlan &pl, int H, int grid, hipStream_t s);
int launch_bwd_f32(bool gru, const RecBwdArgs &a, const BwdPlan &pl, int grid, hipStream_t s);
int launch_bwd_bf(bool gru, const RecBwdArgs &a, const BwdPlan &pl, int grid, hipStream_t s);

}
```

### end-to-end-asr-pytorch_amd/ops.py

```python
import collections
import contextlib
import ctypes

import numpy as np
import torch
from torch.autograd import Function

from . import _lib

_ws_cache = {}


def _L():
    return _lib.load()


def _require_gpu(t):
    if not t.is_cuda:
        raise _lib.AsrkError("asrk ops need tensors on the MI355X (got %s); the product path has no "
                             "CPU fallback" % t.device)


def _p(t):
    return ctypes.c_void_p(t.data_ptr()) if t is not None else ctypes.c_void_p(0)


_raw_stream = getattr(torch._C, "_cuda_getCurrentRawStream", None)
_raw_device = getattr(torch._C, "_cuda_getDevice", None)


def _stream():
    if _raw_stream is not None and _raw_device is not None:
        return ctypes.c_void_p(_raw_stream(_raw_device()))
    return ctypes.c_void_p(torch.cuda.current_stream().cuda_stream)


def _f32c(t):
    if t.dtype != torch.float32:
        t = t.float()
    return t if t.is_contiguous() else t.contiguous()


def lstm_workspace(device):
    key = (device.type, device.index if device.index is not None else torch.cuda.current_device())
    ws = _ws_cache.get(key)
    if ws is None:
        ws = torch.zeros(int(_L().asrk_lstm_ws_bytes()), dtype=torch.uint8, device=device)
        _ws_cache[key] = ws
    return ws


import os as _os
_GEMM_SPLIT_FLAG = {0: 1, 1: 0, 2: 2}
_gemm_state = {"split": max(0, min(2, int(_os.environ.get("ASRK_GEMM_SPLIT", "1")))), "lds_hint": 0}


def set_gemm_split(mode):
    _gemm_state["split"] = max(0, min(2, int(mode)))


def get_gemm_split():
    return _gemm_state["split"]


def gemm_flags():
    return _GEMM_SPLIT_FLAG[_gemm_state["split"]] | ((_gemm_state["lds_hint"] & 0xff) << 8)


def gemm_takes_split(M, N, K):
    return bool(_L().asrk_gemm_takes_split(M, N, K, gemm_flags()))


def rec_flags(backward):
    return 1 if _os.environ.get("ASRK_REC_BF_BWD" if backward else "ASRK_REC_BF", "1") == "0" else 0


ASRK_REC_REARM = 2
ASRK_REC_BWD_NO_DG = 4
_XCHG_REARM = _os.environ.get("ASRK_XCHG_REARM", "1") != "0"
_XCHG_POOL_CAP = int(float(_os.environ.get("ASRK_XCHG_POOL_GB", "24")) * (1 << 30))
_xchg_pool = {"free": {}, "bytes": 0, "tick": 0, "stats": {"hit": 0, "miss": 0, "evicted": 0}}


def _size_class(n):
    if n <= 4096:
        return 4096
    q = 1 << (int(n - 1).bit_length() - 3)
    return (n + q - 1) // q * q


def _pool_evict(pool, need):
    while pool["bytes"] + need > _XCHG_POOL_CAP:
        victim = None
        for key, lst in pool["free"].items():
            for i, e in enumerate(lst):
                if victim is None or e[2] < victim[2][2]:
                    victim = (key, i, e)
        if victim is None:
            return
        key, i, e = victim
        pool["free"][key].pop(i)
        pool["bytes"] -= e[0].numel()
        pool["stats"]["evicted"] += 1


class _Exchange:

    __slots__ = ("buf", "prefilled", "flags", "key", "need", "armed")

    def __init__(self, L, T, B, H, ndir, backward, device):
        base = rec_flags(backward)
        n = int(L.asrk_lstm_xchg_bytes(T, B, H, ndir, backward, base))
        if n == 0:
            raise _lib.AsrkError("LSTM shape T=%d B=%d H=%d ndir=%d is not supported by the persistent "
                                 "gfx950 recurrence kernels" % (T, B, H, ndir))
        self.flags = base | (ASRK_REC_REARM if _XCHG_REARM else 0)
        self.need = n
        self.key = (device.index, torch.cuda.current_stream(device).cuda_stream)
        if not _XCHG_REARM:
            self.buf, self.prefilled, self.armed = torch.empty(n, dtype=torch.uint8, device=device), 0, 0
            return
        free = _xchg_pool["free"].get(self.key, ())
        best = None
        for i, e in enumerate(free):
            if e[0].numel() >= n:
                rank = (e[1] < n, e[0].numel())
                if best is None or rank < best[0]:
                    best = (rank, i)
        if best is not None:
            e = free.pop(best[1])
            _xchg_pool["bytes"] -= e[0].numel()
            self.buf, self.armed = e[0], e[1]
        else:
            self.buf, self.armed = torch.empty(_size_class(n), dtype=torch.uint8, device=device), 0
        self.prefilled = 1 if self.armed >= n else 0
        _xchg_pool["stats"]["hit" if self.prefilled else "miss"] += 1

    def done(self):
        if not _XCHG_REARM:
            return
        n = self.buf.numel()
        if n > _XCHG_POOL_CAP:
            return
        _pool_evict(_xchg_pool, n)
        _xchg_pool["tick"] += 1
        _xchg_pool["free"].setdefault(self.key, []).append([self.buf, max(self.armed, self.need), _xchg_pool["tick"]])
        _xchg_pool["bytes"] += n


def drop_exchange_pool():
    _xchg_pool["free"].clear()
    _xchg_pool["bytes"] = 0


def pool_stats():
    return {"exchange": dict(_xchg_pool["stats"], held_bytes=_xchg_pool["bytes"]),
            "panels": dict(_panel_pool["stats"], held_bytes=_panel_pool["bytes"])}


def check_errors(device=None):
    for key, ws in list(_ws_cache.items()):
        rc = _L().asrk_lstm_check_error(_p(ws), _stream())
        if rc != 0:
            drop_exchange_pool()
        _lib.check(rc, "lstm grid sync")


_defer = {"enabled": True, "side": {}, "pending": {}, "cb_armed": False, "release": []}


def set_deferred_weight_grads(flag):
    join_deferred()
    _defer["enabled"] = bool(flag)


def join_deferred():
    for dev, ev in list(_defer["pending"].items()):
        torch.cuda.current_stream(dev).wait_event(ev)
    _defer["pending"].clear()


def deferred_stream(device):
    dev = torch.device(device)
    if dev.index is None:
        dev = torch.device(dev.type, torch.cuda.current_device())
    return _defer["side"].get(dev) if dev in _defer["pending"] else None


def _end_of_backward():
    _defer["cb_armed"] = False
    join_deferred()
    rel, _defer["release"] = _defer["release"], []
    for pnl in rel:
        pnl.release()


def _can_defer(*weights):
    return _defer["enabled"] and all(w is None or (w.is_leaf and w.grad is None) for w in weights)


_BG_FORCED = _os.environ.get("ASRK_SIDE_BG")
_BG_HINT = int(_BG_FORCED) if _BG_FORCED is not None else 0


_gemm_phase_hooks = []


def on_gemm_phase(fn):
    _gemm_phase_hooks.append(fn)
    return fn


def remove_gemm_phase_hook(fn):
    if fn in _gemm_phase_hooks:
        _gemm_phase_hooks.remove(fn)


def _gemm_phase_begins():
    for fn in list(_gemm_phase_hooks):
        fn()


def _defer_beside_bptt():
    return _BG_HINT > 0 or _os.environ.get("ASRK_DEFER_WIDE", "0") == "1"


def _note_bptt_plan(L, T, B, H, ndir):
    global _BG_HINT
    if _BG_FORCED is None:
        wgs = int(L.asrk_lstm_plan_workgroups(T, B, H, ndir, 1, rec_flags(1)))
        cus = torch.cuda.get_device_properties(torch.cuda.current_device()).multi_processor_count
        _BG_HINT = 96 if 0 < 2 * wgs <= cus else 0


class _SideStream:

    def __init__(self, device, inputs, background=True):
        self.device = torch.device(device)
        self.inputs = inputs
        self.hint = _BG_HINT if background else 0

    def __enter__(self):
        dev = self.device
        side = _defer["side"].get(dev)
        if side is None:
            side = torch.cuda.Stream(device=dev)
            _defer["side"][dev] = side
        main = torch.cuda.current_stream(dev)
        ev = torch.cuda.Event()
        ev.record(main)
        side.wait_event(ev)
        for t in self.inputs:
            if t is not None:
                t.record_stream(side)
        self.main, self.side = main, side
        self.ctx = torch.cuda.stream(side)
        self.ctx.__enter__()
        self.prev_hint = _gemm_state["lds_hint"]
        if self.hint:
            _gemm_state["lds_hint"] = self.hint
        return self

    def keep(self, *outs):
        for t in outs:
            if t is not None:
                t.record_stream(self.main)

    def __exit__(self, *exc):
        _gemm_state["lds_hint"] = self.prev_hint
        self.ctx.__exit__(*exc)
        done = torch.cuda.Event()
        done.record(self.side)
        _defer["pending"][self.device] = done
        if not _defer["cb_armed"]:
            try:
                torch.autograd.Variable._execution_engine.queue_callback(_end_of_backward)
                _defer["cb_armed"] = True
            except RuntimeError:
                join_deferred()
        return False


_grad_dest = {"fn": None}


def set_grad_destination(fn):
    _grad_dest["fn"] = fn


def grad_out(weight, shape, device):
    fn = _grad_dest["fn"]
    if fn is not None and weight is not None:
        t = fn(weight, tuple(shape))
        if t is not None:
            return t
    return torch.empty(shape, dtype=torch.float32, device=device)


def grad_has_destination(*weights):
    fn = _grad_dest["fn"]
    return fn is not None and all(w is not None and fn(w, tuple(w.shape)) is not None for w in weights)


def gemm(transA, transB, M, N, K, A, lda, B, ldb, C, ldc, alpha=1.0, beta=0.0, bias=None, bias2=None,
         splitk=0):
    _require_gpu(C)
    ra, ca = (K, M) if transA else (M, K)
    rb, cb = (N, K) if transB else (K, N)
    for name, t, r, c, ld in (("A", A, ra, ca, lda), ("B", B, rb, cb, ldb), ("C", C, M, N, ldc)):
        avail = t.untyped_storage().nbytes() // t.element_size() - t.storage_offset()
        if r > 0 and c > 0 and (ld < c or avail < (r - 1) * ld + c):
            raise _lib.AsrkError("gemm: operand {} ({} elements behind the pointer) too small for {}x{} "
                                 "with ld {}".format(name, avail, r, c, ld))
    L = _L()
    flags = gemm_flags()
    nws = int(L.asrk_gemm_ws_bytes(M, N, K, flags)) if splitk <= 0 else 0
    ws = torch.empty((nws,), dtype=torch.uint8, device=C.device) if nws else None
    _lib.check(L.asrk_gemm_f32(int(transA), int(transB), M, N, K, alpha, _p(A), lda, _p(B), ldb,
                               beta, _p(C), ldc, _p(bias), _p(bias2), splitk, flags, _p(ws), nws, _stream()),
               "gemm")


class SplitPanel:

    def __init__(self, src, ld, rows, K, trans):
        _require_gpu(src)
        L = _L()
        need = (K - 1) * ld + rows if trans else (rows - 1) * ld + K
        avail = src.untyped_storage().nbytes() // src.element_size() - src.storage_offset()
        if ld < (rows if trans else K) or avail < need:
            raise _lib.AsrkError("split panel: source too small for {}x{} (trans={}) with ld {}".format(
                rows, K, trans, ld))
        self.rows, self.K = rows, K
        self.flags = 0
        self.buf = torch.empty((L.asrk_split_panel_bytes(rows, K, self.flags),), dtype=torch.uint8,
                               device=src.device)
        _lib.check(L.asrk_split_panel_f32(_p(src), ld, rows, K, int(trans), _p(self.buf), self.flags, _stream()),
                   "split_panel")


import weakref as _weakref
_REC_PANELS = _os.environ.get("ASRK_REC_PANELS", "1") != "0"
_REC_SKIP_DG = True
_panel_pool = {"free": {}, "bytes": 0, "tick": 0, "seen": {}, "stats": {"hit": 0, "miss": 0, "skipped": 0, "evicted": 0}}
_panel_state = {"hint": False, "handover": None,
                "stats": {"emitted": 0, "consumed": 0, "dg": 0, "dgt": 0, "no_dg": 0, "dw_ih_splitk": 0}}


class _BlankPanel:
    __slots__ = ("buf", "rows", "K", "flags", "key")

    @staticmethod
    def take(rows, K, device):
        key = (device.index, torch.cuda.current_stream(device).cuda_stream, rows, K)
        free = _panel_pool["free"].get(key)
        if free:
            e = free.pop()
            _panel_pool["bytes"] -= e[0].numel()
            _panel_pool["stats"]["hit"] += 1
            return _BlankPanel(rows, K, key, e[0])
        seen = _panel_pool["seen"]
        if key not in seen:
            if len(seen) > 4096:
                seen.clear()
            seen[key] = 1
            _panel_pool["stats"]["skipped"] += 1
            return None
        _panel_pool["stats"]["miss"] += 1
        n = int(_L().asrk_split_panel_bytes(rows, K, 0))
        buf = torch.empty((n,), dtype=torch.uint8, device=device)
        _lib.check(_L().asrk_fill_f32(_p(buf), n // 4, 0.0, _stream()), "fill")
        return _BlankPanel(rows, K, key, buf)

    def __init__(self, rows, K, key, buf):
        self.rows, self.K, self.flags, self.key, self.buf = rows, K, 0, key, buf

    def release(self):
        n = self.buf.numel()
        if n > _XCHG_POOL_CAP:
            return
        _pool_evict(_panel_pool, n)
        _panel_pool["tick"] += 1
        _panel_pool["free"].setdefault(self.key, []).append([self.buf, 0, _panel_pool["tick"]])
        _panel_pool["bytes"] += n


def set_panel_hint(flag):
    _panel_state["hint"] = bool(flag)


def _take_handover(x):
    h, _panel_state["handover"] = _panel_state["handover"], None
    if h is None:
        return None
    ref, version, panel = h
    if ref() is x and x._version == version and panel.rows == x.shape[0] * x.shape[1] and panel.K == x.shape[2]:
        return panel
    panel.release()
    return None


def gemm_panels(M, N, K, A, a_row0, a_k0, B, b_row0, b_k0, C, ldc, alpha=1.0, beta=0.0, bias=None, bias2=None,
                splitk=None):
    _require_gpu(C)
    avail = C.untyped_storage().nbytes() // C.element_size() - C.storage_offset()
    if ldc < N or avail < (M - 1) * ldc + N:
        raise _lib.AsrkError("gemm_panels: C too small for {}x{} with ld {}".format(M, N, ldc))
    if A.flags != B.flags:
        raise _lib.AsrkError("gemm_panels: the two panels were built in different layouts")
    L = _L()
    if splitk is None:
        _lib.check(L.asrk_gemm_panels_f32(M, N, K, alpha, _p(A.buf), A.rows, A.K, a_row0, a_k0, _p(B.buf), B.rows,
                                          B.K, b_row0, b_k0, beta, _p(C), ldc, _p(bias), _p(bias2), A.flags,
                                          _stream()), "gemm_panels")
        return
    nws = int(L.asrk_gemm_panels_splitk_ws_bytes(M, N, splitk))
    ws = torch.empty((nws,), dtype=torch.uint8, device=C.device)
    _lib.check(L.asrk_gemm_panels_splitk_f32(M, N, K, alpha, _p(A.buf), A.rows, A.K, a_row0, a_k0, _p(B.buf), B.rows,
                                             B.K, b_row0, b_k0, beta, _p(C), ldc, _p(bias), _p(bias2), splitk, _p(ws),
                                             nws, A.flags, _stream()), "gemm_panels")


def zeros(shape, device):
    t = torch.empty(shape, dtype=torch.float32, device=device)
    if t.numel():
        _lib.check(_L().asrk_fill_f32(_p(t), t.numel(), 0.0, _stream()), "fill")
    return t


def copy_flat(dst, src):
    n = src.numel()
    if n:
        copy3d(src, dst, 1, 1, n, 0, 0, 0, 0)


def copy3d(src, dst, n0, n1, n2, ss0, ss1, ds0, ds1, accumulate=False):
    _require_gpu(dst)
    _lib.check(_L().asrk_copy3d_f32(_p(src), _p(dst), n0, n1, n2, ss0, ss1, ds0, ds1,
                                    int(accumulate), _stream()), "copy3d")


def colsum(X, M, N, ldx, out, accumulate=False):
    _lib.check(_L().asrk_colsum_f32(_p(X), M, N, ldx, _p(out), int(accumulate), _stream()), "colsum")


class LinearFn(Function):

    @staticmethod
    def forward(ctx, x, weight, bias):
        _require_gpu(x)
        x2 = _f32c(x).reshape(-1, x.shape[-1])
        w = _f32c(weight)
        M, K = x2.shape
        N = w.shape[0]
        if w.dim() != 2 or w.shape[1] != K or (bias is not None and bias.numel() != N):
            raise RuntimeError("linear: input [..., {}] cannot be multiplied with weight {} (bias {})".format(
                K, tuple(w.shape), None if bias is None else tuple(bias.shape)))
        y = torch.empty((M, N), dtype=torch.float32, device=x.device)
        gemm(0, 1, M, N, K, x2, K, w, K, y, N, bias=bias)
        ctx.save_for_backward(x2, w)
        ctx.has_bias = bias is not None
        ctx.bias_ref = bias
        ctx.in_shape = x.shape
        return y.reshape(*x.shape[:-1], N)

    @staticmethod
    def backward(ctx, dy):
        x2, w = ctx.saved_tensors
        M, K = x2.shape
        N = w.shape[0]
        dy2 = _f32c(dy).reshape(M, N)
        dx = dw = db = None
        if ctx.needs_input_grad[0]:
            dx = torch.empty((M, K), dtype=torch.float32, device=dy.device)
            gemm(0, 0, M, K, N, dy2, N, w, K, dx, K)
            dx = dx.reshape(ctx.in_shape)
        def param_grads():
            dw_ = db_ = None
            if ctx.needs_input_grad[1]:
                dw_ = grad_out(w, (N, K), dy.device)
                gemm(1, 0, N, K, M, dy2, N, x2, K, dw_, K)
            if ctx.has_bias and ctx.needs_input_grad[2]:
                db_ = torch.empty((N,), dtype=torch.float32, device=dy.device)
                colsum(dy2, M, N, N, db_)
            return dw_, db_

        if M >= 1024 and _can_defer(w, ctx.bias_ref) and _defer_beside_bptt():
            with _SideStream(dy.device, (dy2, x2)) as side:
                dw, db = param_grads()
                side.keep(dw, db)
        else:
            dw, db = param_grads()
        return dx, dw, db


def linear(x, weight, bias=None):
    if not torch.is_grad_enabled():
        _require_gpu(x)
        x2 = _f32c(x).reshape(-1, x.shape[-1])
        w = _f32c(weight)
        M, K = x2.shape
        N = w.shape[0]
        if w.dim() != 2 or w.shape[1] != K or (bias is not None and bias.numel() != N):
            raise RuntimeError("linear: input [..., {}] cannot be multiplied with weight {} (bias {})".format(
                K, tuple(w.shape), None if bias is None else tuple(bias.shape)))
        y = torch.empty((M, N), dtype=torch.float32, device=x.device)
        gemm(0, 1, M, N, K, x2, K, w, K, y, N, bias=bias)
        return y.reshape(*x.shape[:-1], N)
    return LinearFn.apply(x, weight, bias)


class TanhFn(Function):
    @staticmethod
    def forward(ctx, x):
        _require_gpu(x)
        xc = _f32c(x)
        y = torch.empty_like(xc)
        _lib.check(_L().asrk_tanh_fwd_f32(_p(xc), _p(y), xc.numel(), _stream()), "tanh")
        ctx.save_for_backward(y)
        return y

    @staticmethod
    def backward(ctx, dy):
        (y,) = ctx.saved_tensors
        dyc = _f32c(dy)
        dx = torch.empty_like(y)
        _lib.check(_L().asrk_tanh_bwd_f32(_p(y), _p(dyc), _p(dx), y.numel(), _stream()), "tanh_bwd")
        return dx


def tanh(x):
    return TanhFn.apply(x)


def tanh_(x):
    _require_gpu(x)
    assert x.is_contiguous() and x.dtype == torch.float32
    _lib.check(_L().asrk_tanh_fwd_f32(_p(x), _p(x), x.numel(), _stream()), "tanh")
    return x


class LogSoftmaxFn(Function):

    @staticmethod
    def forward(ctx, x):
        _require_gpu(x)
        xc = _f32c(x)
        V = xc.shape[-1]
        rows = xc.numel() // V
        y = torch.empty_like(xc)
        _lib.check(_L().asrk_log_softmax_fwd_f32(_p(xc), _p(y), rows, V, V, _stream()), "log_softmax")
        ctx.save_for_backward(y)
        return y

    @staticmethod
    def backward(ctx, dy):
        (y,) = ctx.saved_tensors
        V = y.shape[-1]
        rows = y.numel() // V
        dyc = _f32c(dy)
        dx = torch.empty_like(y)
        _lib.check(_L().asrk_log_softmax_bwd_f32(_p(y), _p(dyc), _p(dx), rows, V, V, _stream()),
                   "log_softmax_bwd")
        return dx


def log_softmax(x):
    if not torch.is_grad_enabled():
        _require_gpu(x)
        xc = _f32c(x)
        V = xc.shape[-1]
        y = torch.empty_like(xc)
        _lib.check(_L().asrk_log_softmax_fwd_f32(_p(xc), _p(y), xc.numel() // V, V, V, _stream()), "log_softmax")
        return y
    return LogSoftmaxFn.apply(x)


def topk(x, k):
    _require_gpu(x)
    xc = _f32c(x.detach())
    V = xc.shape[-1]
    rows = xc.numel() // V
    vals = torch.empty(xc.shape[:-1] + (k,), dtype=torch.float32, device=x.device)
    idx = torch.empty(xc.shape[:-1] + (k,), dtype=torch.int64, device=x.device)
    _lib.check(_L().asrk_topk_f32(_p(xc), rows, V, V, k, _p(vals), _p(idx), _stream()), "topk")
    return vals, idx


def argmax(x):
    return topk(x, 1)[1].squeeze(-1)


def token_crop(ids, pad_idx=0, eos_idx=1, ignore_repeat=False):
    _require_gpu(ids)
    x = ids.to(torch.int64)
    if x.dim() != 2:
        raise _lib.AsrkError("token_crop expects [B, T] ids")
    if x.stride(1) != 1:
        x = x.contiguous()
    B, T = x.shape
    out = torch.zeros((B, max(T, 1)), dtype=torch.int64, device=x.device)
    n = torch.zeros((B,), dtype=torch.int32, device=x.device)
    _lib.check(_L().asrk_token_crop_i64(_p(x), x.stride(0) if B else T, B, T, pad_idx, eos_idx, int(ignore_repeat),
                                        _p(out), out.stride(0), _p(n), _stream()), "token_crop")
    return out, n


def edit_distance(a, a_len, b, b_len):
    _require_gpu(a)
    a, b = a.to(torch.int64).contiguous(), b.to(torch.int64).contiguous()
    a_len, b_len = a_len.to(torch.int32).contiguous(), b_len.to(torch.int32).contiguous()
    B = a.shape[0]
    if b.shape[0] != B or a_len.numel() != B or b_len.numel() != B:
        raise _lib.AsrkError("edit_distance: batch sizes differ")
    if b.shape[1] > 4096 and a.shape[1] <= 4096:
        a, a_len, b, b_len = b, b_len, a, a_len
    d = torch.empty((B,), dtype=torch.int32, device=a.device)
    _lib.check(_L().asrk_edit_distance_i64(_p(a), a.shape[1], _p(a_len), _p(b), b.shape[1], _p(b_len), B,
                                           b.shape[1], _p(d), _stream()), "edit_distance")
    return d


class SwapBTFn(Function):

    @staticmethod
    def forward(ctx, x):
        _require_gpu(x)
        xc = _f32c(x)
        A, B, F = xc.shape
        y = torch.empty((B, A, F), dtype=torch.float32, device=x.device)
        copy3d(xc, y, A, B, F, B * F, F, F, A * F)
        return y

    @staticmethod
    def backward(ctx, dy):
        return SwapBTFn.apply(dy)


def swap_bt(x):
    return SwapBTFn.apply(x)


class PyramidFn(Function):

    @staticmethod
    def forward(ctx, x, rate, style):
        _require_gpu(x)
        xc = _f32c(x)
        T, B, F = xc.shape
        ctx.meta = (T, B, F, rate, style)
        if style == "concat":
            To = T // rate
            y = torch.empty((To, B, rate * F), dtype=torch.float32, device=x.device)
            for j in range(rate):
                copy3d(xc[j:], y[:, :, j * F:], To, B, F, rate * B * F, F, B * rate * F, rate * F)
        else:
            To = (T + rate - 1) // rate
            y = torch.empty((To, B, F), dtype=torch.float32, device=x.device)
            copy3d(xc, y, To, B, F, rate * B * F, F, B * F, F)
        return y

    @staticmethod
    def backward(ctx, dy):
        T, B, F, rate, style = ctx.meta
        dyc = _f32c(dy)
        if style == "concat" and T % rate == 0:
            dx = torch.empty((T, B, F), dtype=torch.float32, device=dy.device)
        else:
            dx = zeros((T, B, F), dy.device)
        if style == "concat":
            To = T // rate
            for j in range(rate):
                copy3d(dyc[:, :, j * F:], dx[j:], To, B, F, B * rate * F, rate * F, rate * B * F, F)
        else:
            To = (T + rate - 1) // rate
            copy3d(dyc, dx, To, B, F, B * F, F, rate * B * F, F)
        return dx, None, None


def pyramid(x_tm, rate, style):
    return PyramidFn.apply(x_tm, rate, style)


def _pyramid_out(T, B, F, rate, style, dev, zero=False):
    mode = {None: 0, 'concat': 1, 'drop': 2}[style if rate > 1 else None]
    if mode == 0:
        return 0, None
    shape = (T // rate, B, rate * F) if mode == 1 else ((T + rate - 1) // rate, B, F)
    return mode, zeros(shape, dev) if zero else torch.empty(shape, dtype=torch.float32, device=dev)


def _db_in_kernel(has_bias, B):
    return has_bias and B <= 32


@contextlib.contextmanager
def _bptt_launch(L, T, B, H, ndir, has_bias, G, dev):
    _note_bptt_plan(L, T, B, H, ndir)
    x = _Exchange(L, T, B, H, ndir, 1, dev)
    db_all = torch.empty((ndir, 4 * H), dtype=torch.float32, device=dev) if has_bias else None
    yield x, db_all
    x.done()
    if has_bias and not _db_in_kernel(has_bias, B):
        colsum(G, T * B, ndir * 4 * H, ndir * 4 * H, db_all)
    _gemm_phase_begins()


STREAM = "STREAM"
SIDE_ALL = "SIDE_ALL"
SIDE_REVERSE_SHARED = "SIDE_REVERSE_SHARED"
SIDE_REVERSE = "SIDE_REVERSE"
IH_PANELS, IH_SPLITK, IH_F32 = "panels", "panels_splitk", "f32"
LstmBwdPlan = collections.namedtuple("LstmBwdPlan", "pG pGT db_in_kernel skip_dg rows_ih dw_ih_route dw_hh_panels "
                                                    "schedule defer_release")


def lstm_bwd_plan(T, B, Din, H, ndir, has_bias, needs_dx, stacked, can_defer, to_scratch, beside_bptt, bf_bwd, share_env,
                  skip_dg_switch, takes_split, take_panel):
    M = T * B
    pG = pGT = None
    if bf_bwd and needs_dx and stacked and takes_split(M, Din, 8 * H):
        pG = take_panel(M, 8 * H)
    share0 = share_env and T > 1 and H % 128 == 0 and B % 8 == 0 and takes_split(4 * H, H, (T - 1) * B)
    if bf_bwd and share0 and B % 16 == 0 and not beside_bptt:
        pGT = take_panel(ndir * 4 * H, M)
    rows_ih = 8 * H if stacked and (needs_dx or not can_defer) and to_scratch else 4 * H
    wide_ih = Din % 4 == 0 and takes_split(rows_ih, Din, M)
    narrow_ih = pGT is not None and Din % 4 == 0 and not wide_ih
    if narrow_ih and stacked and to_scratch:
        rows_ih = 8 * H
    db_in_kernel = _db_in_kernel(has_bias, B)
    skip_dg = bool(skip_dg_switch and pGT is not None and Din % 4 == 0 and (not needs_dx or pG is not None)
                   and (db_in_kernel or not has_bias))
    if not (can_defer and (beside_bptt or not needs_dx)):
        schedule = STREAM
    elif needs_dx or ndir == 1:
        schedule = SIDE_ALL
    elif pGT is None:
        schedule = SIDE_REVERSE
    elif Din % 4 == 0:
        schedule = STREAM
    else:
        schedule = SIDE_REVERSE_SHARED
    panels = bool(share0) and schedule != SIDE_REVERSE
    route = IH_SPLITK if narrow_ih else IH_PANELS if panels and wide_ih else IH_F32
    return LstmBwdPlan(pG, pGT, db_in_kernel, skip_dg, rows_ih, route, panels, schedule, schedule == SIDE_REVERSE_SHARED)


class LSTMLayerFn(Function):

    @staticmethod
    def forward(ctx, x, w_ih_f, w_hh_f, b_ih_f, b_hh_f, w_ih_r, w_hh_r, b_ih_r, b_hh_r, pyr_rate=1,
                pyr_style=None):
        _require_gpu(x)
        L = _L()
        xc = _f32c(x)
        T, B, Din = xc.shape
        H = w_hh_f.shape[1]
        ndir = 2 if w_ih_r is not None else 1
        dev = x.device
        M = T * B
        G = torch.empty((M, ndir * 4 * H), dtype=torch.float32, device=dev)
        w_ih_f, w_hh_f = _f32c(w_ih_f), _f32c(w_hh_f)
        w_stack = None
        if ndir == 2:
            w_ih_r, w_hh_r = _f32c(w_ih_r), _f32c(w_hh_r)
        if ndir == 2 and H >= 768 and _os.environ.get("ASRK_STACK_DIRS", "1") != "0":
            if (w_ih_f.untyped_storage().data_ptr() == w_ih_r.untyped_storage().data_ptr()
                    and w_ih_r.storage_offset() == w_ih_f.storage_offset() + 4 * H * Din):
                w_stack = w_ih_f.as_strided((8 * H, Din), (Din, 1))
            else:
                w_stack = torch.empty((8 * H, Din), dtype=torch.float32, device=dev)
                copy_flat(w_stack[:4 * H], w_ih_f)
                copy_flat(w_stack[4 * H:], w_ih_r)
            if b_ih_f is not None:
                b1 = torch.empty((2, 8 * H), dtype=torch.float32, device=dev)
                for row, (bf_, br_) in enumerate(((b_ih_f, b_ih_r), (b_hh_f, b_hh_r))):
                    copy_flat(b1[row, :4 * H], _f32c(bf_.detach()))
                    copy_flat(b1[row, 4 * H:], _f32c(br_.detach()))
                b1, b2 = b1[0], b1[1]
            else:
                b1 = b2 = None
            x_panel = _take_handover(x) if x is xc else None
            if x_panel is not None and gemm_takes_split(M, 8 * H, Din):
                pW = SplitPanel(w_stack, Din, 8 * H, Din, False)
                gemm_panels(M, 8 * H, Din, x_panel, 0, 0, pW, 0, 0, G, 8 * H, bias=b1, bias2=b2)
                del pW
                _panel_state["stats"]["consumed"] += 1
            else:
                gemm(0, 1, M, 8 * H, Din, xc, Din, w_stack, Din, G, 8 * H, bias=b1, bias2=b2)
            if x_panel is not None:
                x_panel.release()
        else:
            gemm(0, 1, M, 4 * H, Din, xc, Din, w_ih_f, Din, G, ndir * 4 * H, bias=b_ih_f, bias2=b_hh_f)
            if ndir == 2:
                gemm(0, 1, M, 4 * H, Din, xc, Din, w_ih_r, Din, G[:, 4 * H:], ndir * 4 * H, bias=b_ih_r,
                     bias2=b_hh_r)
        Y = torch.empty((M, ndir * H), dtype=torch.float32, device=dev)
        C = torch.empty((M, ndir * H), dtype=torch.float32, device=dev)
        ws = lstm_workspace(dev)
        xc_ = _Exchange(L, T, B, H, ndir, 0, dev)
        mode, Y2 = _pyramid_out(T, B, ndir * H, pyr_rate, pyr_style, dev)
        rate = max(1, pyr_rate)
        out_panel = None
        if (_REC_PANELS and _panel_state["hint"] and mode in (0, 1) and (mode == 0 or T // rate > 0) and
                (ndir * H) % 8 == 0 and L.asrk_lstm_plan_is_bf(T, B, H, ndir, 0, rec_flags(0))):
            r_ = rate if mode == 1 else 1
            out_panel = _BlankPanel.take((T // r_) * B, r_ * ndir * H, dev)
        if out_panel is not None:
            _panel_state["stats"]["emitted"] += 1
            _lib.check(L.asrk_lstm_rec_fwd_pyr_panel_f32(_p(G), _p(w_hh_f), _p(w_hh_r), _p(Y), _p(C), T, B, H, ndir,
                                                         _p(xc_.buf), xc_.prefilled, _p(ws), _p(Y2), mode, rate,
                                                         _p(out_panel.buf), xc_.flags, _stream()), "lstm_rec_fwd")
        else:
            _lib.check(L.asrk_lstm_rec_fwd_pyr_f32(_p(G), _p(w_hh_f), _p(w_hh_r), _p(Y), _p(C), T, B, H, ndir,
                                                   _p(xc_.buf), xc_.prefilled, _p(ws), _p(Y2), mode, rate,
                                                   xc_.flags, _stream()), "lstm_rec_fwd")
        xc_.done()
        ctx.pyr = (mode, max(1, pyr_rate))
        ctx.dims = (T, B, Din, H, ndir)
        ctx.has_bias = b_ih_f is not None
        ctx.bias_refs = (b_ih_f, b_hh_f, b_ih_r, b_hh_r)
        ctx.save_for_backward(xc, w_ih_f, w_hh_f, w_ih_r, w_hh_r, G, C, Y, w_stack)
        ctx.consumed = False
        out = Y2 if mode else Y.view(T, B, ndir * H)
        if _panel_state["handover"] is not None:
            _panel_state["handover"][2].release()
            _panel_state["handover"] = None
        if out_panel is not None:
            _panel_state["handover"] = (_weakref.ref(out), out._version, out_panel)
        return out

    @staticmethod
    def backward(ctx, dY):
        L = _L()
        xc, w_ih_f, w_hh_f, w_ih_r, w_hh_r, G, C, Y, w_stack = ctx.saved_tensors
        if ctx.consumed:
            raise RuntimeError("LSTMLayerFn: backward twice (the gate buffer is reused in place)")
        ctx.consumed = True
        T, B, Din, H, ndir = ctx.dims
        dev = dY.device
        M = T * B
        ldg, ldy = ndir * 4 * H, ndir * H
        mode, rate = ctx.pyr
        dYc = _f32c(dY)
        ws = lstm_workspace(dev)
        needs_dx = ctx.needs_input_grad[0]
        w_ih, w_hh = (w_ih_f, w_ih_r), (w_hh_f, w_hh_r)
        with _bptt_launch(L, T, B, H, ndir, ctx.has_bias, G, dev) as (xc_, db_all):
            plan = lstm_bwd_plan(T, B, Din, H, ndir, ctx.has_bias, needs_dx, w_stack is not None,
                                 _can_defer(w_ih_f, w_hh_f, w_ih_r, w_hh_r, *ctx.bias_refs),
                                 not grad_has_destination(*w_ih[:ndir]), _defer_beside_bptt(),
                                 bool(_REC_PANELS and L.asrk_lstm_plan_is_bf(T, B, H, ndir, 1, rec_flags(1))),
                                 _os.environ.get("ASRK_SHARE_PANELS", "1") != "0", _REC_SKIP_DG, gemm_takes_split,
                                 lambda rows, K: _BlankPanel.take(rows, K, dev))
            pG, pGT = plan.pG, plan.pGT
            stats = _panel_state["stats"]
            stats["dg"] += pG is not None
            stats["dgt"] += pGT is not None
            stats["no_dg"] += plan.skip_dg
            stats["dw_ih_splitk"] += (plan.dw_ih_route == IH_SPLITK) * (1 if plan.rows_ih == 8 * H else ndir)
            db = db_all if plan.db_in_kernel else None
            if pG is not None or pGT is not None:
                _lib.check(L.asrk_lstm_rec_bwd_pyr_panel_f32(_p(G), _p(w_hh_f), _p(w_hh_r), _p(C), _p(dYc), T, B, H,
                                                             ndir, _p(xc_.buf), xc_.prefilled, _p(ws), _p(db), mode, rate,
                                                             _p(pG.buf if pG is not None else None),
                                                             _p(pGT.buf if pGT is not None else None),
                                                             xc_.flags | (ASRK_REC_BWD_NO_DG if plan.skip_dg else 0),
                                                             _stream()), "lstm_rec_bwd")
            else:
                _lib.check(L.asrk_lstm_rec_bwd_pyr_f32(_p(G), _p(w_hh_f), _p(w_hh_r), _p(C), _p(dYc), T, B, H,
                                                       ndir, _p(xc_.buf), xc_.prefilled, _p(ws), _p(db), mode, rate,
                                                       xc_.flags, _stream()), "lstm_rec_bwd")
        dG = G
        f32 = dict(dtype=torch.float32, device=dev)
        dx = None
        if needs_dx:
            dx = torch.empty((M, Din), **f32)
            if pG is not None:
                pWT = SplitPanel(w_stack, Din, Din, 8 * H, True)
                gemm_panels(M, Din, 8 * H, pG, 0, 0, pWT, 0, 0, dx, Din)
                del pWT
                pG.release()
            elif w_stack is not None:
                gemm(0, 0, M, Din, 8 * H, dG, ldg, w_stack, Din, dx, Din)
            else:
                gemm(0, 0, M, Din, 4 * H, dG, ldg, w_ih_f, Din, dx, Din)
                if ndir == 2:
                    gemm(0, 0, M, Din, 4 * H, dG[:, 4 * H:], ldg, w_ih_r, Din, dx, Din, beta=1.0)
            dx = dx.view(T, B, Din)
        panels = {} if pGT is None else {"dGT": pGT}
        dw_ih_stack = []

        def panel(name, src, ld, rows):
            if name not in panels:
                panels[name] = SplitPanel(src, ld, rows, M, True)
            return panels[name]

        def dg_gemm(Mo, No, Ko, m0, k0, pB, b_row0, b_k0, out, ldo, splitk=None):
            gemm_panels(Mo, No, Ko, panel("dGT", dG, ldg, ldg), m0, k0, pB, b_row0, b_k0, out, ldo, splitk=splitk)

        def dw_ih_of(d):
            stacked = plan.rows_ih == 8 * H
            if not (stacked and dw_ih_stack):
                out = torch.empty((8 * H, Din), **f32) if stacked else grad_out(w_ih[d], (4 * H, Din), dev)
                m0 = 0 if stacked else d * 4 * H
                if plan.dw_ih_route == IH_F32:
                    gemm(1, 0, plan.rows_ih, Din, M, dG[:, m0:], ldg, xc, Din, out, Din)
                else:
                    dg_gemm(plan.rows_ih, Din, M, m0, 0, panel("XT", xc, Din, Din), 0, 0, out, Din,
                            0 if plan.dw_ih_route == IH_SPLITK else None)
                if not stacked:
                    return out
                dw_ih_stack.append(out)
            return dw_ih_stack[0][d * 4 * H:(d + 1) * 4 * H]

        def dw_hh_of(d):
            if T <= 1:
                return zeros((4 * H, H), dev)
            out, Mh = grad_out(w_hh[d], (4 * H, H), dev), (T - 1) * B
            if plan.dw_hh_panels:
                dg_gemm(4 * H, H, Mh, d * 4 * H, B if d == 0 else 0, panel("YT", Y, ldy, ldy), d * H, 0 if d == 0 else B,
                        out, H)
            elif d == 0:
                gemm(1, 0, 4 * H, H, Mh, dG[B:], ldg, Y, ldy, out, H)
            else:
                gemm(1, 0, 4 * H, H, Mh, dG[:, 4 * H:], ldg, Y[B:, H:], ldy, out, H)
            return out

        def param_grads(d):
            if plan.dw_hh_panels:
                dw_hh = dw_hh_of(d)
                dw_ih = dw_ih_of(d)
            else:
                dw_ih = dw_ih_of(d)
                dw_hh = dw_hh_of(d)
            db = db2 = None
            if ctx.has_bias:
                db = db_all[d]
                db2 = db.clone()
            return dw_ih, dw_hh, db, db2

        if plan.schedule == STREAM:
            grads = [param_grads(d) for d in range(ndir)]
        elif plan.schedule == SIDE_ALL:
            with _SideStream(dev, (dG, xc, Y, db_all)) as side:
                grads = [param_grads(d) for d in range(ndir)]
                side.keep(*[t for g in grads for t in g])
        else:
            inputs = (dG, xc, Y, db_all)
            if plan.schedule == SIDE_REVERSE_SHARED:
                inputs += (pGT.buf, panel("YT", Y, ldy, ldy).buf)
            with _SideStream(dev, inputs, background=False) as side:
                g1 = param_grads(1)
                side.keep(*g1)
            grads = [param_grads(0), g1]
        if pGT is not None:
            if plan.defer_release or _defer["pending"]:
                _defer["release"].append(pGT)
            else:
                pGT.release()
        if ndir == 1:
            grads.append((None, None, None, None))
        return (dx,) + grads[0] + grads[1] + (None, None)


class Copy3dFn(Function):

    @staticmethod
    def forward(ctx, src, out_shape, n0, n1, n2, ss0, ss1, ds0, ds1):
        _require_gpu(src)
        s = _f32c(src)
        dst = zeros(out_shape, src.device)
        copy3d(s, dst, n0, n1, n2, ss0, ss1, ds0, ds1)
        ctx.meta = (tuple(src.shape), n0, n1, n2, ss0, ss1, ds0, ds1)
        return dst

    @staticmethod
    def backward(ctx, g):
        shape, n0, n1, n2, ss0, ss1, ds0, ds1 = ctx.meta
        gs = zeros(shape, g.device)
        copy3d(_f32c(g), gs, n0, n1, n2, ds0, ds1, ss0, ss1)
        return (gs,) + (None,) * 8


def _pad_lstm_params(params, H, Hp):
    w_ih, w_hh, b_ih, b_hh = params
    Din = w_ih.shape[1]
    w_ih_p = Copy3dFn.apply(w_ih, (4 * Hp, Din), 4, H, Din, H * Din, Din, Hp * Din, Din)
    w_hh_p = Copy3dFn.apply(w_hh, (4 * Hp, Hp), 4, H, H, H * H, H, Hp * Hp, Hp)
    b_ih_p = Copy3dFn.apply(b_ih, (4 * Hp,), 1, 4, H, 0, H, 0, Hp)
    b_hh_p = Copy3dFn.apply(b_hh, (4 * Hp,), 1, 4, H, 0, H, 0, Hp)
    return w_ih_p, w_hh_p, b_ih_p, b_hh_p


def lstm_layer(x_tm, params_f, params_r=None, pyramid=None):
    H = params_f[1].shape[1]
    if pyramid is not None and pyramid[0] > 1:
        if H % 4 != 0 or _os.environ.get("ASRK_FUSE_PYRAMID", "1") == "0":
            return PyramidFn.apply(lstm_layer(x_tm, params_f, params_r), pyramid[0], pyramid[1])
        pr = params_r if params_r is not None else (None, None, None, None)
        return LSTMLayerFn.apply(x_tm, *params_f, *pr, pyramid[0], pyramid[1])
    if H % 4 != 0:
        Hp = (H + 3) // 4 * 4
        ndir = 2 if params_r is not None else 1
        pf = _pad_lstm_params(params_f, H, Hp)
        pr = _pad_lstm_params(params_r, H, Hp) if params_r is not None else (None,) * 4
        T, B = x_tm.shape[0], x_tm.shape[1]
        yp = LSTMLayerFn.apply(x_tm, *pf, *pr)
        return Copy3dFn.apply(yp, (T, B, ndir * H), T * B, ndir, H, ndir * Hp, Hp, ndir * H, H)
    pr = params_r if params_r is not None else (None, None, None, None)
    return LSTMLayerFn.apply(x_tm, *params_f, *pr)


def lstm_layer_packed(x_tm, params_f, params_r, lens, pyramid=None):
    _require_gpu(x_tm)
    if torch.is_grad_enabled() and x_tm.requires_grad:
        raise _lib.AsrkError("lstm_layer_packed is inference-only")
    L = _L()
    xc = _f32c(x_tm)
    T, B, Din = xc.shape
    w_ih_f, w_hh_f, b_ih_f, b_hh_f = (None if t is None else _f32c(t.detach()) for t in params_f)
    H = w_hh_f.shape[1]
    if H % 4 != 0:
        raise _lib.AsrkError("lstm_layer_packed: hidden size must be a multiple of 4")
    ndir = 2 if params_r is not None else 1
    dev = xc.device
    M = T * B
    G = torch.empty((M, ndir * 4 * H), dtype=torch.float32, device=dev)
    gemm(0, 1, M, 4 * H, Din, xc, Din, w_ih_f, Din, G, ndir * 4 * H, bias=b_ih_f, bias2=b_hh_f)
    w_hh_r = None
    if ndir == 2:
        w_ih_r, w_hh_r, b_ih_r, b_hh_r = (None if t is None else _f32c(t.detach()) for t in params_r)
        gemm(0, 1, M, 4 * H, Din, xc, Din, w_ih_r, Din, G[:, 4 * H:], ndir * 4 * H, bias=b_ih_r, bias2=b_hh_r)
    lens_d = torch.as_tensor(lens).to(device=dev, dtype=torch.int64).contiguous()
    Y = zeros((M, ndir * H), dev)
    C = torch.empty((M, ndir * H), dtype=torch.float32, device=dev)
    rate, style = pyramid if pyramid is not None else (1, None)
    mode, Y2 = _pyramid_out(T, B, ndir * H, rate, style, dev, zero=True)
    ws = lstm_workspace(dev)
    xc_ = _Exchange(L, T, B, H, ndir, 0, dev)
    _lib.check(L.asrk_lstm_rec_fwd_len_f32(_p(G), _p(w_hh_f), _p(w_hh_r), _p(Y), _p(C), _p(lens_d), T, B, H, ndir,
                                           _p(xc_.buf), xc_.prefilled, _p(ws), _p(Y2), mode, max(1, rate), xc_.flags,
                                           _stream()), "lstm_rec_fwd_len")
    xc_.done()
    return Y2 if mode else Y.view(T, B, ndir * H)


CTC_ZERO_INFINITY = 1


class CTCLossFn(Function):

    @staticmethod
    def forward(ctx, log_probs, targets, input_lengths, target_lengths, blank, reduction, zero_infinity=False,
                count_out=None):
        _require_gpu(log_probs)
        L = _L()
        if log_probs.dtype != torch.float32:
            log_probs = log_probs.float()
        if log_probs.stride(2) != 1:
            log_probs = log_probs.contiguous()
        T, B, V = log_probs.shape
        dev = log_probs.device
        targets = torch.as_tensor(targets).to(device=dev, dtype=torch.int64)
        if targets.dim() != 2:
            raise _lib.AsrkError("CTCLoss: only padded 2-D targets [B, L] are supported "
                                 "(reference passes txt [B,L], bin/train_asr.py:123)")
        targets = targets.contiguous()
        il = torch.as_tensor(input_lengths).to(device=dev, dtype=torch.int64).contiguous()
        tl = torch.as_tensor(target_lengths).to(device=dev, dtype=torch.int64).contiguous()
        Lmax = targets.shape[1]
        S = 2 * Lmax + 1
        alpha = torch.empty((B, T, S), dtype=torch.float32, device=dev)
        lpg = torch.empty((B, T, S), dtype=torch.float32, device=dev)
        beta = torch.empty((B, T, S), dtype=torch.float32, device=dev) if ctx.needs_input_grad[0] else None
        nll = torch.empty((B,), dtype=torch.float32, device=dev)
        if zero_infinity:
            loss = torch.empty((B,), dtype=torch.float32, device=dev)
            if count_out is not None and B == 0:
                count_out.zero_()
            _lib.check(L.asrk_ctc_loss_fwd_ex_f32(_p(log_probs), log_probs.stride(0), log_probs.stride(1), T,
                                                  B, V, _p(targets), targets.stride(0), Lmax, _p(il),
                                                  _p(tl), blank, _p(alpha), _p(beta), _p(lpg), _p(nll),
                                                  CTC_ZERO_INFINITY, _p(loss), _p(count_out), _stream()), "ctc_fwd")
        else:
            loss = nll
            _lib.check(L.asrk_ctc_loss_fwd_f32(_p(log_probs), log_probs.stride(0), log_probs.stride(1), T,
                                               B, V, _p(targets), targets.stride(0), Lmax, _p(il),
                                               _p(tl), blank, _p(alpha), _p(beta), _p(lpg), _p(nll),
                                               _stream()), "ctc_fwd")
        ctx.save_for_backward(log_probs, targets, il, tl, alpha, beta, lpg, nll)
        ctx.meta = (T, B, V, Lmax, blank, reduction, bool(zero_infinity))
        if reduction == "mean":
            return (loss / tl.clamp(min=1).to(torch.float32)).mean()
        if reduction == "sum":
            return loss.sum()
        return loss

    @staticmethod
    def backward(ctx, gout):
        L = _L()
        log_probs, targets, il, tl, alpha, beta, lpg, nll = ctx.saved_tensors
        T, B, V, Lmax, blank, reduction, zero_infinity = ctx.meta
        dev = log_probs.device
        if reduction == "mean":
            gscale = gout.to(torch.float32) / (tl.clamp(min=1).to(torch.float32) * B)
        elif reduction == "sum":
            gscale = gout.to(torch.float32).expand(B)
        else:
            gscale = gout.to(torch.float32)
        gscale = gscale.contiguous()
        if log_probs.stride(1) > log_probs.stride(0):
            grad = torch.empty((B, T, V), dtype=torch.float32, device=dev).transpose(0, 1)
        else:
            grad = torch.empty((T, B, V), dtype=torch.float32, device=dev)
        if zero_infinity:
            _lib.check(L.asrk_ctc_loss_bwd_ex_f32(_p(log_probs), log_probs.stride(0), log_probs.stride(1), T,
                                                  B, V, _p(targets), targets.stride(0), Lmax, _p(il),
                                                  _p(tl), blank, _p(alpha), _p(beta), _p(lpg), _p(nll), _p(gscale),
                                                  _p(grad), grad.stride(0), grad.stride(1), CTC_ZERO_INFINITY,
                                                  _stream()), "ctc_bwd")
        else:
            _lib.check(L.asrk_ctc_loss_bwd_f32(_p(log_probs), log_probs.stride(0), log_probs.stride(1), T,
                                               B, V, _p(targets), targets.stride(0), Lmax, _p(il),
                                               _p(tl), blank, _p(alpha), _p(beta), _p(lpg), _p(nll), _p(gscale),
                                               _p(grad), grad.stride(0), grad.stride(1), _stream()),
                       "ctc_bwd")
        return grad, None, None, None, None, None, None, None


class CTCLoss(torch.nn.Module):

    def __init__(self, blank=0, reduction="mean", zero_infinity=False):
        super().__init__()
        if reduction not in ("none", "mean", "sum"):
            raise ValueError("CTCLoss: unknown reduction %r" % (reduction,))
        self.blank = blank
        self.reduction = reduction
        self.zero_infinity = bool(zero_infinity)
        self.n_infeasible = None

    def forward(self, log_probs, targets, input_lengths, target_lengths):
        if not self.zero_infinity:
            return CTCLossFn.apply(log_probs, targets, input_lengths, target_lengths, self.blank,
                                   self.reduction)
        _require_gpu(log_probs)
        self.n_infeasible = torch.empty((), dtype=torch.int32, device=log_probs.device)
        return CTCLossFn.apply(log_probs, targets, input_lengths, target_lengths, self.blank,
                               self.reduction, True, self.n_infeasible)


ALIGN_BP_AUTO, ALIGN_BP_LDS, ALIGN_BP_GLOBAL = 0, 1, 2

CTCAlignment = collections.namedtuple("CTCAlignment", ["states", "tokens", "spans", "score"])


@torch.no_grad()
def ctc_align(log_probs, targets, input_lengths, target_lengths, blank=0, flags=ALIGN_BP_AUTO, stamps=None):
    _require_gpu(log_probs)
    L = _L()
    if log_probs.dim() != 3:
        raise _lib.AsrkError("ctc_align: log_probs must be [T, B, V]")
    if log_probs.dtype != torch.float32:
        log_probs = log_probs.float()
    if log_probs.stride(2) != 1:
        log_probs = log_probs.contiguous()
    T, B, V = log_probs.shape
    dev = log_probs.device
    targets = torch.as_tensor(targets).to(device=dev, dtype=torch.int64)
    if targets.dim() != 2:
        raise _lib.AsrkError("ctc_align: only padded 2-D targets [B, L] are supported")
    targets = targets.contiguous()
    il = torch.as_tensor(input_lengths).to(device=dev, dtype=torch.int64).contiguous()
    tl = torch.as_tensor(target_lengths).to(device=dev, dtype=torch.int64).contiguous()
    if targets.shape[0] != B or il.numel() != B or tl.numel() != B:
        raise _lib.AsrkError("ctc_align: targets / lengths do not match the batch of log_probs")
    Lmax = targets.shape[1]
    states = torch.empty((B, T), dtype=torch.int32, device=dev)
    tokens = torch.empty((B, T), dtype=torch.int32, device=dev)
    spans = torch.empty((B, Lmax, 2), dtype=torch.int32, device=dev)
    score = torch.empty((B,), dtype=torch.float32, device=dev)
    need = L.asrk_ctc_align_ws_bytes(B, T, Lmax, flags)
    ws = torch.empty((need,), dtype=torch.uint8, device=dev) if need else None
    _lib.check(L.asrk_ctc_align_f32(_p(log_probs), log_probs.stride(0), log_probs.stride(1), T, B, V, _p(targets),
                                    targets.stride(0), Lmax, _p(il), _p(tl), blank, flags, _p(states), _p(tokens),
                                    _p(spans), _p(score), _p(stamps), _p(ws), need, _stream()), "ctc_align")
    return CTCAlignment(states, tokens, spans, score)


def _check_label_smoothing(eps):
    if isinstance(eps, bool) or not isinstance(eps, (int, float)) or not 0.0 <= eps < 1.0:
        raise ValueError("label_smoothing must be a number in [0, 1), got %r" % (eps,))
    return float(eps)


class CrossEntropyFn(Function):

    @staticmethod
    def forward(ctx, logits, targets, ignore_index, label_smoothing=0.0):
        _require_gpu(logits)
        eps = _check_label_smoothing(label_smoothing)
        x = _f32c(logits)
        R, V = x.shape
        tg = targets.to(device=x.device, dtype=torch.int64).contiguous()
        lse = torch.empty((R,), dtype=torch.float32, device=x.device)
        ctx.ignore_index = ignore_index
        ctx.label_smoothing = eps
        if eps == 0.0:
            sums = torch.empty((2,), dtype=torch.float32, device=x.device)
            _lib.check(_L().asrk_cross_entropy_fwd_f32(_p(x), R, V, V, _p(tg), ignore_index, _p(lse),
                                                       _p(sums), _stream()), "cross_entropy")
            ctx.save_for_backward(x, tg, lse, sums)
            return sums[0] / sums[1]
        smooth = torch.empty((R,), dtype=torch.float32, device=x.device)
        sums = torch.empty((3,), dtype=torch.float32, device=x.device)
        _lib.check(_L().asrk_cross_entropy_ls_fwd_f32(_p(x), R, V, V, _p(tg), ignore_index, _p(lse), _p(smooth),
                                                      _p(sums), _stream()), "cross_entropy_ls")
        ctx.save_for_backward(x, tg, lse, sums)
        return ((1.0 - eps) * sums[0] + eps * sums[2]) / sums[1]

    @staticmethod
    def backward(ctx, gout):
        x, tg, lse, sums = ctx.saved_tensors
        R, V = x.shape
        gscale = (gout.to(torch.float32) / sums[1]).reshape(1).contiguous()
        dx = torch.empty_like(x)
        if ctx.label_smoothing == 0.0:
            _lib.check(_L().asrk_cross_entropy_bwd_f32(_p(x), R, V, V, _p(tg), ctx.ignore_index, _p(lse),
                                                       _p(gscale), _p(dx), _stream()), "cross_entropy_bwd")
        else:
            _lib.check(_L().asrk_cross_entropy_ls_bwd_f32(_p(x), R, V, V, _p(tg), ctx.ignore_index,
                                                          ctx.label_smoothing, _p(lse), _p(gscale), _p(dx),
                                                          _stream()), "cross_entropy_ls_bwd")
        return dx, None, None, None


class CrossEntropyLoss(torch.nn.Module):

    def __init__(self, ignore_index=-100, reduction="mean", label_smoothing=0.0):
        super().__init__()
        assert reduction == "mean"
        self.ignore_index = ignore_index
        self.label_smoothing = _check_label_smoothing(label_smoothing)

    def forward(self, logits, targets):
        if self.label_smoothing == 0.0:
            return CrossEntropyFn.apply(logits, targets, self.ignore_index)
        return CrossEntropyFn.apply(logits, targets, self.ignore_index, self.label_smoothing)


class NLLLossFn(Function):

    @staticmethod
    def forward(ctx, logp, targets, ignore_index):
        _require_gpu(logp)
        x = _f32c(logp)
        R, V = x.shape
        tg = targets.to(device=x.device, dtype=torch.int64).contiguous()
        if tg.numel() != R:
            raise RuntimeError("nll_loss: %d targets for %d rows" % (tg.numel(), R))
        sums = torch.empty((2,), dtype=torch.float32, device=x.device)
        _lib.check(_L().asrk_nll_loss_fwd_f32(_p(x), R, V, V, _p(tg), ignore_index, _p(sums), _stream()), "nll_loss")
        ctx.ignore_index, ctx.shape = ignore_index, (R, V)
        ctx.save_for_backward(tg, sums)
        return sums[0] / sums[1]

    @staticmethod
    def backward(ctx, gout):
        tg, sums = ctx.saved_tensors
        R, V = ctx.shape
        gscale = (gout.to(torch.float32) / sums[1]).reshape(1).contiguous()
        dx = torch.empty((R, V), dtype=torch.float32, device=tg.device)
        _lib.check(_L().asrk_nll_loss_bwd_f32(R, V, V, _p(tg), ctx.ignore_index, _p(gscale), _p(dx), _stream()),
                   "nll_loss_bwd")
        return dx, None, None


class NLLLoss(torch.nn.Module):

    def __init__(self, ignore_index=-100, reduction="mean"):
        super().__init__()
        assert reduction == "mean"
        self.ignore_index = ignore_index

    def forward(self, logp, targets):
        return NLLLossFn.apply(logp, targets, self.ignore_index)


class LayerNormFn(Function):

    @staticmethod
    def forward(ctx, x, weight, bias, eps):
        _require_gpu(x)
        xc = _f32c(x)
        D = xc.shape[-1]
        if weight.numel() != D or bias.numel() != D:
            raise RuntimeError("layer_norm: normalized_shape {} does not match input [..., {}]".format(
                tuple(weight.shape), D))
        rows = xc.numel() // D
        w, b = _f32c(weight), _f32c(bias)
        y = torch.empty_like(xc)
        mean = torch.empty((rows,), dtype=torch.float32, device=x.device)
        rstd = torch.empty((rows,), dtype=torch.float32, device=x.device)
        _lib.check(_L().asrk_layer_norm_fwd_f32(_p(xc), _p(w), _p(b), _p(y), _p(mean), _p(rstd), rows, D,
                                                float(eps), _stream()), "layer_norm")
        ctx.save_for_backward(xc, w, mean, rstd)
        return y

    @staticmethod
    def backward(ctx, dy):
        xc, w, mean, rstd = ctx.saved_tensors
        D = xc.shape[-1]
        rows = xc.numel() // D
        dyc = _f32c(dy)
        dx = torch.empty_like(xc) if ctx.needs_input_grad[0] else None
        want_p = ctx.needs_input_grad[1] or ctx.needs_input_grad[2]
        dw = torch.empty((D,), dtype=torch.float32, device=dy.device) if want_p else None
        db = torch.empty((D,), dtype=torch.float32, device=dy.device) if want_p else None
        _lib.check(_L().asrk_layer_norm_bwd_f32(_p(xc), _p(w), _p(dyc), _p(mean), _p(rstd), _p(dx), _p(dw),
                                                _p(db), rows, D, _stream()), "layer_norm_bwd")
        return dx, dw, db, None


def layer_norm(x, weight, bias, eps):
    return LayerNormFn.apply(x, weight, bias, eps)


class DropoutFn(Function):

    @staticmethod
    def forward(ctx, x, p, seed):
        _require_gpu(x)
        xc = _f32c(x)
        y = torch.empty_like(xc)
        _lib.check(_L().asrk_dropout_f32(_p(xc), _p(y), xc.numel(), float(p), seed, 0, _stream()), "dropout")
        ctx.p, ctx.seed = float(p), seed
        return y

    @staticmethod
    def backward(ctx, dy):
        dyc = _f32c(dy)
        dx = torch.empty_like(dyc)
        _lib.check(_L().asrk_dropout_f32(_p(dyc), _p(dx), dyc.numel(), ctx.p, ctx.seed, 0, _stream()),
                   "dropout_bwd")
        return dx, None, None


def dropout(x, p, training, seed=None):
    if not training or p == 0:
        return x
    if p >= 1:
        raise ValueError("dropout probability has to be in [0, 1), got {}".format(p))
    if seed is None:
        seed = int(torch.randint(0, 2 ** 62, (1,)).item())
    return DropoutFn.apply(x, p, seed)


def spec_augment(x, lens, params, n_fmask, n_tmask, fill=0.0, channels=1):
    _require_gpu(x)
    xc = _f32c(x.detach())
    if xc.dim() != 3:
        raise ValueError("spec_augment expects [B, T, F] features, got %s" % (tuple(xc.shape),))
    B, T, F = xc.shape
    P = 2 + 2 * int(n_fmask) + 2 * int(n_tmask)
    if channels <= 0 or F % channels != 0:
        raise ValueError("feature width %d is no multiple of %d channels" % (F, channels))
    if (lens.dtype != torch.int64 or lens.device != xc.device or tuple(lens.shape) != (B,)
            or not lens.is_contiguous()):
        raise ValueError("lens must be a contiguous int64 [B] tensor on x's device")
    if (params.dtype != torch.int32 or params.device != xc.device or tuple(params.shape) != (B, P)
            or not params.is_contiguous()):
        raise ValueError("params must be a contiguous int32 [B, %d] tensor on x's device" % P)
    y = torch.empty_like(xc)
    _lib.check(_L().asrk_spec_augment_f32(_p(xc), _p(y), B, T, F, F // channels, channels, _p(lens), _p(params),
                                          int(n_fmask), int(n_tmask), float(fill), _stream()), "spec_augment")
    return y


_RESAMPLE_TAPS = {}
RESAMPLE_LOWPASS_WIDTH = 6
RESAMPLE_ROLLOFF = 0.99


def resample_width(orig, new):
    return -(-100 * RESAMPLE_LOWPASS_WIDTH * orig // (99 * min(orig, new)))


def resample_taps(orig, new):
    W = float(RESAMPLE_LOWPASS_WIDTH)
    base = min(orig, new) * RESAMPLE_ROLLOFF
    width = resample_width(orig, new)
    j = np.arange(new, dtype=np.float64)[:, None]
    k = np.arange(2 * width + orig, dtype=np.float64)[None, :]
    t = np.clip((-j / new + (k - width) / orig) * base, -W, W)
    return np.sinc(t) * np.cos(np.pi * t / (2.0 * W)) ** 2 * (base / orig)


def _resample_taps_dev(orig, new, device):
    key = (orig, new, str(device))
    tab = _RESAMPLE_TAPS.get(key)
    if tab is None:
        tab = torch.from_numpy(np.ascontiguousarray(resample_taps(orig, new), dtype=np.float32)).to(device)
        _RESAMPLE_TAPS[key] = tab
    return tab


def resample_rows(x, n_host, ratio_idx, ratios, scale=1.0):
    _require_gpu(x)
    if x.dim() != 2 or x.dtype not in (torch.int16, torch.float32) or not x.is_contiguous():
        raise ValueError("resample_rows expects a contiguous [B, ld_in] int16 or float32 batch")
    B, ld_in = x.shape
    n = np.ascontiguousarray(np.asarray(n_host, dtype=np.int64).reshape(-1))
    idx = np.ascontiguousarray(np.asarray(ratio_idx, dtype=np.int32).reshape(-1))
    rat = np.ascontiguousarray(np.asarray(ratios, dtype=np.int32).reshape(-1, 2))
    if n.shape[0] != B or idx.shape[0] != B:
        raise ValueError("resample_rows: %d rows, %d lengths, %d ratio indices" % (B, n.shape[0], idx.shape[0]))
    if B and (rat.shape[0] == 0 or idx.min() < 0 or idx.max() >= rat.shape[0] or rat.min() < 1):
        raise ValueError("resample_rows: ratio index outside the %d ratio(s) given, or a non-positive ratio"
                         % rat.shape[0])
    n_out = (rat[idx, 1].astype(np.int64) * n + rat[idx, 0] - 1) // rat[idx, 0] if B else np.zeros(0, np.int64)
    ld_out = (int(n_out.max()) + 3) // 4 * 4 if B else 0
    y = torch.empty((B, ld_out), dtype=torch.float32, device=x.device)
    if B == 0:
        return y, n_out
    tabs = [None if (o, w) == (1, 1) else _resample_taps_dev(int(o), int(w), x.device) for o, w in rat.tolist()]
    taps = (ctypes.c_void_p * len(tabs))(*[None if t is None else t.data_ptr() for t in tabs])
    meta = torch.empty(B + (B + 1) // 2, dtype=torch.int64).pin_memory()
    meta[:B] = torch.from_numpy(n)
    meta[B:].view(torch.int32)[:B] = torch.from_numpy(idx)
    meta_dev = meta.to(x.device, non_blocking=True)
    _lib.check(_L().asrk_resample_rows_f32(_p(x), x.element_size(), ld_in, n.ctypes.data, meta_dev.data_ptr(),
                                           idx.ctypes.data, meta_dev.data_ptr() + 8 * B, B, rat.ctypes.data, taps,
                                           rat.shape[0], _p(y), ld_out, float(scale), _stream()), "resample_rows")
    return y, n_out


REVERB_MAX_TAPS = 8192


class RirBank:

    def __init__(self, responses, device="cuda"):
        hs = [np.ascontiguousarray(np.asarray(h, dtype=np.float32).reshape(-1)) for h in responses]
        if not hs:
            raise ValueError("RirBank: no impulse response")
        for h in hs:
            if not 1 <= h.shape[0] <= REVERB_MAX_TAPS or not np.all(np.isfinite(h)):
                raise ValueError("RirBank: an impulse response has 1..%d finite samples, got %d"
                                 % (REVERB_MAX_TAPS, h.shape[0]))
        self.lens = np.asarray([h.shape[0] for h in hs], dtype=np.int32)
        self.peaks = np.asarray([int(np.argmax(np.abs(h))) for h in hs], dtype=np.int32)
        self.ld = (int(self.lens.max()) + 3) // 4 * 4
        host = np.zeros((len(hs), self.ld), dtype=np.float32)
        for r, h in enumerate(hs):
            host[r, :h.shape[0]] = h
        self.taps = torch.from_numpy(host).to(device)
        self.meta = torch.from_numpy(np.concatenate([self.lens, self.peaks])).to(device)

    def __len__(self):
        return int(self.lens.shape[0])


def reverb_mix(x, n_host, bank=None, rir_idx=None, noise=None, m_host=None, snr_lin=None, scale=1.0):
    _require_gpu(x)
    if x.dim() != 2 or x.dtype not in (torch.int16, torch.float32) or not x.is_contiguous():
        raise ValueError("reverb_mix expects a contiguous [B, ld_in] int16 or float32 batch")
    B, ld_in = x.shape
    n = np.ascontiguousarray(np.asarray(n_host, dtype=np.int64).reshape(-1))
    idx = np.full(B, -1, dtype=np.int32) if rir_idx is None else \
        np.ascontiguousarray(np.asarray(rir_idx, dtype=np.int32).reshape(-1))
    m = np.zeros(B, dtype=np.int64) if m_host is None else \
        np.ascontiguousarray(np.asarray(m_host, dtype=np.int64).reshape(-1))
    snr = np.ones(B, dtype=np.float32) if snr_lin is None else \
        np.ascontiguousarray(np.asarray(snr_lin, dtype=np.float32).reshape(-1))
    if not (n.shape[0] == idx.shape[0] == m.shape[0] == snr.shape[0] == B):
        raise ValueError("reverb_mix: %d rows, %d lengths, %d response indices, %d noise lengths, %d ratios"
                         % (B, n.shape[0], idx.shape[0], m.shape[0], snr.shape[0]))
    if bank is None and B and idx.max() >= 0:
        raise ValueError("reverb_mix: a row asks for an impulse response and no bank was given")
    if bank is not None and bank.taps.device != x.device:
        raise ValueError("reverb_mix: the bank lives on %s, the batch on %s" % (bank.taps.device, x.device))
    if noise is None:
        if B and m.max() > 0:
            raise ValueError("reverb_mix: a row asks for noise and no noise batch was given")
        ld_v = 0
    else:
        _require_gpu(noise)
        if (noise.dim() != 2 or noise.shape[0] != B or noise.dtype != x.dtype or not noise.is_contiguous()
                or noise.device != x.device):
            raise ValueError("reverb_mix: noise must be a contiguous [B, ld_v] batch of x's dtype on x's device")
        ld_v = noise.shape[1]
    if B and not (np.all(np.isfinite(snr)) and snr.min() > 0.0):
        raise ValueError("reverb_mix: snr_lin must be positive and finite")
    ld_out = (int(n.max()) + 3) // 4 * 4 if B else 0
    out = torch.empty((B, ld_out), dtype=torch.float32, device=x.device)
    if B == 0:
        return out
    L = _L()
    ws_bytes = int(L.asrk_reverb_mix_ws_bytes(B, int(max(n.max(), 0))))
    ws = torch.empty((max(ws_bytes, 8) // 8,), dtype=torch.float64, device=x.device)
    meta = torch.empty(3 * B, dtype=torch.int64).pin_memory()
    meta[:B] = torch.from_numpy(n)
    meta[B:2 * B] = torch.from_numpy(m)
    meta[2 * B:].view(torch.int32)[:B] = torch.from_numpy(idx)
    meta[2 * B:].view(torch.float32)[B:2 * B] = torch.from_numpy(snr)
    md = meta.to(x.device, non_blocking=True)
    base = md.data_ptr()
    R = 0 if bank is None else len(bank)
    _lib.check(L.asrk_reverb_mix_f32(
        _p(x), x.element_size(), ld_in, n.ctypes.data, base,
        None if bank is None else _p(bank.taps), 0 if bank is None else bank.ld,
        None if bank is None else bank.lens.ctypes.data, None if bank is None else bank.meta.data_ptr(),
        None if bank is None else bank.peaks.ctypes.data, None if bank is None else bank.meta.data_ptr() + 4 * R, R,
        idx.ctypes.data, base + 16 * B, _p(noise), ld_v, m.ctypes.data, base + 8 * B, base + 20 * B, B, _p(out), ld_out,
        float(scale), _p(ws), ws_bytes, _stream()), "reverb_mix")
    return out
```

### include/asrk.h

```cpp
#ifndef ASRK_H
#define ASRK_H

#include <stddef.h>
#include <stdint.h>

#ifdef __cplusplus
extern "C" {
#endif

#define ASRK_OK 0
#define ASRK_EINVAL (-1)
#define ASRK_ESHAPE (-2)
#define ASRK_EWORKSPACE (-3)
#define ASRK_EDEVICE (-4)
#define ASRK_ETIMEOUT (-5)

int asrk_version(void);
const char *asrk_strerror(int rc);
int asrk_init(int device);

void asrk_profile_enable(int on);
void asrk_profile_families(unsigned mask);
void asrk_profile_reset(void);
int asrk_profile_get(int id, double *total_ms, int64_t *launches);
int asrk_profile_get_work(int id, double *flops);
#define ASRK_PROF_GEMM 0
#define ASRK_PROF_LSTM_FWD 1
#define ASRK_PROF_LSTM_BWD 2
#define ASRK_PROF_CTC 3
#define ASRK_PROF_ROWOPS 4
#define ASRK_PROF_ATTN 5
#define ASRK_PROF_CELL 6
#define ASRK_PROF_FBANK 7
#define ASRK_PROF_GEMM_BG 8
#define ASRK_PROF_SPELLER 9
#define ASRK_PROF_CONV 10
#define ASRK_PROF_SPLIT 11
#define ASRK_PROF_OPTIM 12

int asrk_gemm_f32(int transA, int transB, int M, int N, int K, float alpha,
                  const float *A, int lda, const float *B, int ldb, float beta,
                  float *C, int ldc, const float *bias, const float *bias2, int splitk,
                  int flags, void *ws, size_t ws_bytes, void *stream);

#define ASRK_GEMM_SPLIT_AUTO 0
#define ASRK_GEMM_SPLIT_OFF 1
#define ASRK_GEMM_SPLIT_ALWAYS 2
#define ASRK_GEMM_LDS_HINT(kib) (((kib) & 0xff) << 8)
size_t asrk_gemm_ws_bytes(int M, int N, int K, int flags);
int asrk_gemm_takes_split(int M, int N, int K, int flags);

#define ASRK_GEMM_PLAN_INFO_LEN 16
int asrk_gemm_plan_info(int transA, int transB, int M, int N, int K, int lda, int ldb, int ldc, int align,
                        float beta, int splitk, int flags, int ncu, int *info);

size_t asrk_split_panel_bytes(int rows, int K, int flags);
int asrk_split_panel_f32(const float *src, int ld, int rows, int K, int trans, void *panel, int flags, void *stream);
int asrk_gemm_panels_f32(int M, int N, int K, float alpha, const void *A_panel, int a_rows, int a_K,
                         int a_row0, int a_k0, const void *B_panel, int b_rows, int b_K, int b_row0, int b_k0,
                         float beta, float *C, int ldc, const float *bias, const float *bias2, int flags,
                         void *stream);
size_t asrk_gemm_panels_splitk_ws_bytes(int M, int N, int splitk);
int asrk_gemm_panels_splitk_f32(int M, int N, int K, float alpha, const void *A_panel, int a_rows, int a_K,
                                int a_row0, int a_k0, const void *B_panel, int b_rows, int b_K, int b_row0, int b_k0,
                                float beta, float *C, int ldc, const float *bias, const float *bias2, int splitk,
                                void *ws, size_t ws_bytes, int flags, void *stream);

int asrk_copy3d_f32(const float *src, float *dst, int n0, int n1, int n2,
                    int64_t s_stride0, int64_t s_stride1, int64_t d_stride0, int64_t d_stride1,
                    int accumulate, void *stream);

int asrk_colsum_f32(const float *X, int M, int N, int ldx, float *out, int accumulate,
                    void *stream);

int asrk_tanh_fwd_f32(const float *x, float *y, int64_t n, void *stream);
int asrk_tanh_bwd_f32(const float *y, const float *dy, float *dx, int64_t n, void *stream);

int asrk_log_softmax_fwd_f32(const float *x, float *y, int rows, int cols, int ld,
                             void *stream);
int asrk_log_softmax_bwd_f32(const float *y, const float *dy, float *dx, int rows, int cols,
                             int ld, void *stream);

int asrk_topk_f32(const float *x, int rows, int cols, int ld, int k, float *values,
                  int64_t *indices, void *stream);

int asrk_token_crop_i64(const int64_t *ids, int64_t ld, int B, int T, int64_t pad_idx, int64_t eos_idx,
                        int ignore_repeat, int64_t *out, int64_t ld_out, int32_t *out_len, void *stream);
int asrk_edit_distance_i64(const int64_t *a, int64_t lda, const int32_t *a_len, const int64_t *b, int64_t ldb,
                           const int32_t *b_len, int B, int max_b_len, int32_t *dist, void *stream);

int asrk_cross_entropy_fwd_f32(const float *logits, int rows, int V, int ld,
                               const int64_t *targets, int ignore_index, float *row_lse,
                               float *sums, void *stream);
int asrk_cross_entropy_bwd_f32(const float *logits, int rows, int V, int ld,
                               const int64_t *targets, int ignore_index, const float *row_lse,
                               const float *gscale, float *dlogits, void *stream);

int asrk_cross_entropy_ls_fwd_f32(const float *logits, int rows, int V, int ld, const int64_t *targets,
                                  int ignore_index, float *row_lse, float *row_smooth, float *sums, void *stream);
int asrk_cross_entropy_ls_bwd_f32(const float *logits, int rows, int V, int ld, const int64_t *targets,
                                  int ignore_index, float label_smoothing, const float *row_lse, const float *gscale,
                                  float *dlogits, void *stream);

size_t asrk_lstm_ws_bytes(void);
#define ASRK_REC_F32_MFMA 1
#define ASRK_REC_REARM 2
#define ASRK_REC_BWD_NO_DG 4
size_t asrk_lstm_xchg_bytes(int T, int B, int H, int ndir, int backward, int flags);
int asrk_lstm_plan_workgroups(int T, int B, int H, int ndir, int backward, int flags);
#define ASRK_LSTM_PLAN_INFO_LEN 16
int asrk_lstm_plan_info(int T, int B, int H, int ndir, int backward, int flags, int ncu, int *info);
int asrk_lstm_rec_fwd_f32(float *G, const float *whh_f, const float *whh_r, float *Y, float *C,
                          int T, int B, int H, int ndir, void *xchg, int xchg_prefilled, void *ws,
                          int flags, void *stream);
int asrk_lstm_rec_fwd_pyr_f32(float *G, const float *whh_f, const float *whh_r, float *Y, float *C,
                              int T, int B, int H, int ndir, void *xchg, int xchg_prefilled, void *ws,
                              float *Y2, int pyr_mode, int pyr_rate, int flags, void *stream);
int asrk_lstm_rec_bwd_pyr_f32(float *gates, const float *whh_f, const float *whh_r, const float *C,
                              const float *dY, int T, int B, int H, int ndir, void *xchg,
                              int xchg_prefilled, void *ws, float *db, int pyr_mode, int pyr_rate,
                              int flags, void *stream);
int asrk_lstm_plan_is_bf(int T, int B, int H, int ndir, int backward, int flags);
int asrk_lstm_rec_fwd_pyr_panel_f32(float *G, const float *whh_f, const float *whh_r, float *Y, float *C,
                                    int T, int B, int H, int ndir, void *xchg, int xchg_prefilled, void *ws,
                                    float *Y2, int pyr_mode, int pyr_rate, void *x2_panel, int flags, void *stream);
int asrk_lstm_rec_bwd_pyr_panel_f32(float *gates, const float *whh_f, const float *whh_r, const float *C,
                                    const float *dY, int T, int B, int H, int ndir, void *xchg,
                                    int xchg_prefilled, void *ws, float *db, int pyr_mode, int pyr_rate,
                                    void *dg_panel, void *dgt_panel, int flags, void *stream);
int asrk_lstm_rec_fwd_len_f32(float *G, const float *whh_f, const float *whh_r, float *Y, float *C,
                              const int64_t *lens, int T, int B, int H, int ndir, void *xchg,
                              int xchg_prefilled, void *ws, float *Y2, int pyr_mode, int pyr_rate, int flags,
                              void *stream);
int asrk_gru_rec_fwd_f32(float *G, const float *whh_f, const float *whh_r, float *Y, int T, int B, int H,
                         int ndir, void *xchg, int xchg_prefilled, void *ws, float *Y2, int pyr_mode,
                         int pyr_rate, int flags, void *stream);
int asrk_gru_rec_bwd_f32(float *gates, const float *whh_f, const float *whh_r, const float *Y,
                         const float *dY, int T, int B, int H, int ndir, void *xchg, int xchg_prefilled,
                         void *ws, float *db, int pyr_mode, int pyr_rate, int flags, void *stream);
int asrk_lstm_rec_bwd_f32(float *gates, const float *whh_f, const float *whh_r, const float *C,
                          const float *dY, int T, int B, int H, int ndir, void *xchg,
                          int xchg_prefilled, void *ws, float *db, int flags, void *stream);
int asrk_lstm_check_error(void *ws, void *stream);

size_t asrk_ctc_prefix_beam_ws_bytes(int beam, int T);
int asrk_ctc_prefix_beam_ws_offsets(int beam, int T, int buf, int64_t *nb_off, int64_t *len_off, int64_t *tok_off,
                                    int64_t *parent_off, int64_t *last_off, int64_t *gidx_off);
int asrk_ctc_prefix_beam_f32(const float *ctc, int T, int V, const unsigned char *allowed, int beam, int cand,
                             const float *lm, float lm_weight, int t0, int t1, int cur_buf, int init,
                             int lm_step_follows, void *ws, size_t ws_bytes, void *stream);
size_t asrk_ctc_prefix_beam_multi_ws_bytes(int U, int beam, int Tmax, size_t *slab_stride);
int asrk_ctc_prefix_beam_multi_f32(const float *ctc, int64_t ctc_row_stride, int U, int Tmax, int V,
                                   const unsigned char *allowed, int beam, int cand, const float *lm, float lm_weight,
                                   const int *frames, const int *t_start, int j, int *out_parent, int *out_last,
                                   int *out_gidx, void *ws, size_t ws_bytes, void *stream);

int asrk_loc_conv_fwd_f32(const float *prev_att, const float *Wc, float *c, int B, int N, int T,
                          int K, int ks, void *stream);
int asrk_loc_conv_bwd_f32(const float *dc, const float *prev_att, const float *Wc,
                          float *dprev_att, float *dWc_acc, int B, int N, int T, int K, int ks,
                          void *stream);
int asrk_attn_energy_fwd_f32(int loc, const float *key, const float *q, const float *c,
                             const float *Wp, const float *we, const float *be,
                             const int64_t *lens, float *attn, float *e_scratch, int B, int N, int T,
                             int A, int K, float temperature, void *stream);
int asrk_attn_energy_bwd_f32(int loc, const float *key, const float *q, const float *c,
                             const float *Wp, const float *we, const int64_t *lens,
                             const float *attn, const float *dattn, float *dkey_acc, float *dq,
                             float *dc, float *dWp_acc, float *dwe_acc, float *dbe_acc, int B,
                             int N, int T, int A, int K, float temperature, void *stream);
int asrk_attn_context_fwd_f32(const float *attn, const float *value, float *ctx, int BN, int T,
                              int Dv, int64_t ctx_stride, void *stream);
int asrk_attn_context_bwd_f32(const float *dctx, const float *value, float *dattn, int BN, int T,
                              int Dv, int64_t dctx_stride, void *stream);

int asrk_lstm_cell_fwd_f32(float *gates, const float *c_prev, float *c, float *h, int B, int H,
                           void *stream);
int asrk_lstm_cell_bwd_f32(float *gates, const float *c_prev, const float *c, const float *dh,
                           const float *dc_in, float *dc_prev, int B, int H, void *stream);

int asrk_gru_cell_fwd_f32(float *gi, const float *gh, int64_t ldi, int64_t ldh, const float *h_prev,
                          int64_t ldp, float *h_new, int64_t ldn, int B, int H, void *stream);
int asrk_gru_cell_bwd_f32(float *gi, float *gh, int64_t ldi, int64_t ldh, const float *h_prev,
                          int64_t ldp, const float *dh, int64_t ldd, const float *dh2, float *dh_prev,
                          int64_t ldo, int B, int H, void *stream);

int asrk_embedding_fwd_f32(const int64_t *idx, const float *W, float *out, int64_t n, int D, int V,
                           void *stream);
int asrk_embedding_bwd_f32(const int64_t *idx, const float *dout, float *dW_acc, int64_t n, int D,
                           int V, void *stream);

size_t asrk_emb_fuse_bwd_ws_bytes(int N, int V, int temp_len, int lam_len, int want_dtemp, int want_dlam);
int asrk_emb_fuse_fwd_f32(const float *dec_logit, int ld, const float *emb_logit, const float *temp, int temp_len,
                          const float *lam, int lam_len, int lam_is_logit, float eps, int N, int V, float *y,
                          float *stats, void *stream);
int asrk_emb_fuse_bwd_f32(const float *g, const float *dec_logit, int ld, const float *emb_logit, const float *temp,
                          int temp_len, const float *lam, int lam_len, int lam_is_logit, float eps, const float *stats,
                          int N, int V, float *d_dec, float *d_emb, float *dtemp, float *dlam, void *ws,
                          size_t ws_bytes, void *stream);
int asrk_cos_emb_loss_fwd_f32(const float *x, const float *table, int64_t table_rows, const int64_t *label, int B,
                              int L, int E, float *row_loss, float *count, float *loss, void *stream);
int asrk_cos_emb_loss_bwd_f32(const float *x, const float *table, int64_t table_rows, const int64_t *label, int B,
                              int L, int E, const float *count, const float *gout, float *dx, float *dy,
                              void *stream);
int asrk_cos_emb_table_grad_f32(const float *dy, const int64_t *label, int N, int E, int64_t table_rows,
                                float *dtable, void *stream);
int asrk_nll_loss_fwd_f32(const float *logp, int rows, int V, int ld, const int64_t *targets, int ignore_index,
                          float *sums, void *stream);
int asrk_nll_loss_bwd_f32(int rows, int V, int ld, const int64_t *targets, int ignore_index, const float *gscale,
                          float *dlogp, void *stream);
int asrk_l2norm_fwd_f32(const float *x, float *y, float *norm, int rows, int D, float eps, void *stream);
int asrk_l2norm_bwd_f32(const float *y, const float *dy, const float *norm, float *dx, int rows, int D, float eps,
                        void *stream);

typedef struct asrk_speller {
    int B, Te, A, Dv, K, ks, H, E, L;
    float temperature;
    int shared_kv;
    const float *key, *value;
    const int64_t *lens;
    const float *Wq, *bq, *Wc, *Wp, *we, *be, *W_ih, *W_hh, *b_ih, *b_hh;
    const float *eproj;
    float *q, *conv, *attn;
    int64_t attn_ld, attn_step;
    float *ctx, *gates, *h, *c, *states, *e_scratch;
    const float *prev0;
    const int *row_mem;
    int cell;
    int nlayer;
    const float *Wu_ih[2], *Wu_hh[2], *bu_ih[2], *bu_hh[2];
    float *hu[2], *cu[2], *gu[2];
    int att_mode, nhead;
    const float *Wm, *bm;
    float *ctxh;
    int row_group;
} asrk_speller_t;
#define ASRK_SPELLER_MAX_LAYERS 3

typedef struct asrk_speller_bwd {
    const float *dstates, *dattn_seq, *WT, *WqT;
    float *dkey, *dxh, *dq_pre, *dattn, *dprev, *dconv, *dq_part, *dwe_part, *dWp_part, *dbe_part,
        *dWc_part, *dc;
    int tc;
    const float *WuT[2];
    float *dxu[2], *dcu[2];
    const float *WmT;
    float *dctxh;
} asrk_speller_bwd_t;

int asrk_speller_plan(const asrk_speller_t *dims, int *tc_fwd, int *tc_bwd);
int asrk_speller_plan_info(const asrk_speller_t *dims, int *info);
int asrk_speller_ctx_variant(const asrk_speller_t *dims, int *variant);
int asrk_speller_fwd_f32(const asrk_speller_t *p, void *stream);
int asrk_speller_bwd_f32(const asrk_speller_t *p, const asrk_speller_bwd_t *g, void *stream);
int asrk_speller_step_f32(const asrk_speller_t *p, int slot, const float *prev_att, int64_t prev_ld,
                          const float *emb, void *stream);
int asrk_speller_dvalue_f32(const float *attn, int64_t attn_ld, int64_t attn_step, const float *dxh,
                            int64_t step_ld, int64_t row_ld, float *dvalue, int B, int L, int Te, int Dv,
                            void *stream);
int asrk_joint_score_f32(const float *att_logp, const int64_t *cand, const float *psi,
                         const float *prev_ctc, const float *lm_logp, float *out, int n, int V, int C,
                         double ctc_weight, double lm_weight, double logzero, void *stream);
int asrk_lstm_cell_fused_f32(const float *x, int64_t ldx, int In, const float *h, const float *c,
                             const float *W_ih, const float *W_hh, const float *b_ih,
                             const float *b_hh, float *h_out, float *c_out, int B, int H, void *stream);
int asrk_transpose_ld_f32(const float *in, int64_t ldi, float *out, int64_t ldo, int rows, int cols,
                          void *stream);

int asrk_layer_norm_fwd_f32(const float *x, const float *weight, const float *bias, float *y,
                            float *mean, float *rstd, int rows, int cols, float eps, void *stream);
int asrk_layer_norm_bwd_f32(const float *x, const float *weight, const float *dy, const float *mean,
                            const float *rstd, float *dx, float *dweight, float *dbias, int rows,
                            int cols, void *stream);
int asrk_dropout_f32(const float *x, float *y, int64_t n, float p, uint64_t seed, uint64_t offset,
                     void *stream);

int asrk_beam_select_f32(const float *topv, const int64_t *topi, const float *psi, const int64_t *cand, int U, int B, int C,
                         int t, int lmax, int fcap, const int *min_len, const int *max_len, int *alive, double *ssum,
                         int *utt_done, int64_t *prev_token, int64_t *parent, int64_t *col, float *pctc, int *hist_tok,
                         float *hist_sc, int *hist_par, int *fin_count, int *fin_kind, int *fin_t, int *fin_row,
                         float *fin_term, double *fin_ssum, int *live_utts, void *stream);

int asrk_gather_rows_multi_f32(int nseg, const float *const *src, float *const *dst, const int *row_floats, const int *mul,
                               const int *use_col, const int64_t *parent, const int64_t *col, int n, void *stream);

int asrk_conv_out_size(int in, int k, int stride, int pad);
int asrk_im2col_f32(const float *x, float *col, int B, int H, int W, int C, int KH, int KW, int SH, int SW,
                    int PH, int PW, int64_t sb, int64_t sh, int64_t sw, int64_t sc, void *stream);
int asrk_col2im_f32(const float *dcol, float *dx, int B, int H, int W, int C, int KH, int KW, int SH,
                    int SW, int PH, int PW, int64_t sb, int64_t sh, int64_t sw, int64_t sc, void *stream);
int asrk_im2col_ld_f32(const float *x, float *col, int ldcol, int B, int H, int W, int C, int KH, int KW, int SH, int SW,
                       int PH, int PW, int64_t sb, int64_t sh, int64_t sw, int64_t sc, void *stream);
int asrk_im2col_cl_f32(const float *x, float *col, int B, int H, int W, int C, int KH, int KW, int SH, int SW,
                       int PH, int PW, int64_t sb, int64_t sh, int64_t sw, int64_t sc, void *stream);
int asrk_col2im_cl_f32(const float *dcol, float *dx, int B, int H, int W, int C, int KH, int KW, int SH,
                       int SW, int PH, int PW, int64_t sb, int64_t sh, int64_t sw, int64_t sc, void *stream);
int asrk_conv_weight_reorder_f32(const float *src, float *dst, int Cout, int Cin, int KK, int inverse, void *stream);
int asrk_conv3x3_supported(int H, int W, int C, int Cout);
#define ASRK_CONV3X3_PLAN_INFO_LEN 12
int asrk_conv3x3_plan_info(int kind, int B, int H, int W, int C, int Cout, int *out, int n);
int asrk_conv3x3_weight_f32(const float *w, float *wf, int Cout, int Cin, int transpose, void *stream);
int asrk_conv3x3_f32(const float *x, const float *xmask, const float *wf, const float *bias, float *y, int B, int H, int W,
                     int C, int Cout, int relu, void *stream);
size_t asrk_conv3x3_wgrad_ws_bytes(int B, int H, int W, int C, int Cout);
int asrk_conv3x3_wgrad_f32(const float *x, const float *dy, const float *ymask, float *dw, float *db, int B, int H, int W,
                           int C, int Cout, void *ws, size_t ws_bytes, void *stream);
int asrk_conv3x3_first_supported(int H, int W, int C, int Cout);
int asrk_conv3x3_first_f32(const float *x, const float *w, const float *bias, float *y, int B, int H, int W, int C, int Cout,
                           int64_t sb, int64_t sh, int64_t sw, int64_t sc, int relu, void *stream);
size_t asrk_conv3x3_first_wgrad_ws_bytes(int B, int H, int W, int C, int Cout);
int asrk_conv3x3_first_wgrad_f32(const float *x, const float *dy, const float *ymask, float *dw, float *db, int B, int H,
                                 int W, int C, int Cout, int64_t sb, int64_t sh, int64_t sw, int64_t sc, void *ws,
                                 size_t ws_bytes, void *stream);
int asrk_conv3x3_len_f32(const float *x, const float *wf, const float *bias, float *y, const int64_t *hlen, int B, int H,
                         int W, int C, int Cout, int relu, void *stream);
int asrk_conv3x3_first_len_f32(const float *x, const float *w, const float *bias, float *y, const int64_t *hlen, int B, int H,
                               int W, int C, int Cout, int64_t sb, int64_t sh, int64_t sw, int64_t sc, int relu,
                               void *stream);
int asrk_im2col_ld_len_f32(const float *x, float *col, const int64_t *hlen, int ldcol, int B, int H, int W, int C, int KH,
                           int KW, int SH, int SW, int PH, int PW, int64_t sb, int64_t sh, int64_t sw, int64_t sc,
                           void *stream);
int asrk_im2col_cl_len_f32(const float *x, float *col, const int64_t *hlen, int B, int H, int W, int C, int KH, int KW,
                           int SH, int SW, int PH, int PW, int64_t sb, int64_t sh, int64_t sw, int64_t sc, void *stream);
int asrk_conv_zero_tail_f32(float *y, const int64_t *hlen, int B, int H, int64_t row, void *stream);
int asrk_relu_fwd_f32(float *x, int64_t n, void *stream);
int asrk_relu_bwd_f32(const float *y, const float *dy, float *dx, int64_t n, void *stream);
int asrk_maxpool2x2_fwd_f32(const float *x, float *y, uint8_t *idx, int B, int H, int W, int C,
                            int64_t osb, int64_t osh, int64_t osw, int64_t osc, void *stream);
int asrk_maxpool2x2_bwd_f32(const float *dy, const uint8_t *idx, float *dx, int B, int H, int W, int C,
                            int64_t osb, int64_t osh, int64_t osw, int64_t osc, void *stream);

int asrk_adadelta_step_f32(float *param, const float *grad, float *square_avg, float *acc_delta,
                           int64_t n, double lr, double rho, double eps, const float *clip_coef,
                           void *stream);
int asrk_adam_step_f32(float *param, const float *grad, float *exp_avg, float *exp_avg_sq, int64_t n,
                       double lr, double beta1, double beta2, double eps, int64_t step,
                       const float *clip_coef, void *stream);
int asrk_adadelta_multi_f32(int count, float *const *params, const float *const *grads,
                            float *const *square_avg, float *const *acc_delta, const int64_t *numel,
                            double lr, double rho, double eps, const float *clip_coef, void *stream);
int asrk_adam_multi_f32(int count, float *const *params, const float *const *grads,
                        float *const *exp_avg, float *const *exp_avg_sq, const int64_t *numel,
                        double lr, double beta1, double beta2, double eps, int64_t step,
                        const float *clip_coef, void *stream);

size_t asrk_grad_norm_ws_bytes(int count, const int64_t *numel);
int asrk_grad_norm_multi_f32(int count, const float *const *grads, const int64_t *numel, float max_norm,
                             float *norm_out, float *coef_out, void *ws, size_t ws_bytes, void *stream);
int asrk_fill_f32(float *x, int64_t n, float value, void *stream);

int asrk_fbank_frames_f32(const float *wave, int64_t n_samples, const float *window, float *frames,
                          int m, int win, int shift, int ldf, float preemph, int remove_dc,
                          void *stream);
int asrk_power_spectrum_f32(const float *spec, float *power, int64_t m, int nb, void *stream);
int asrk_log_floor_f32(float *x, int64_t n, float eps, void *stream);
int asrk_delta_f32(const float *x, const float *filters, float *y, int C, int D, int T, int L,
                   void *stream);
int asrk_cmvn_f32(const float *x, float *y, int rows, int T, float eps, void *stream);
int asrk_transpose_f32(const float *x, float *y, int rows, int cols, void *stream);
int asrk_fbank_frames_batch_f32(const void *wave, int sample_bytes, int64_t ld_wave, const int64_t *n_samples_host,
                                const int64_t *frame_off, int B, int max_m, const float *window, float *frames,
                                int win, int shift, int ldf, float scale, float preemph, int remove_dc,
                                void *stream);
int asrk_delta_cmvn_batch_f32(const float *mel, const int64_t *frame_off, int B, int D, const float *filters, int C,
                              int L, int apply_cmvn, float eps, float *out, int Tmax, void *stream);
int asrk_fbank_logmel_batch_f32(const void *wave, int sample_bytes, int64_t ld_wave, const int64_t *n_samples_host,
                                const int64_t *frame_off, int B, int max_m, const float *window, const float *tw_fft,
                                const float *tw_unpack, const float *melT, const int *mel_range, int nmel, int ld_mel,
                                float *mel, int win, int shift, int log2n, float scale, float preemph, int remove_dc,
                                float eps, void *stream);

int asrk_fbank_frames_dither_f32(const float *wave, int64_t n_samples, const float *window, float *frames, int m,
                                 int win, int shift, int ldf, float preemph, int remove_dc, float dither, uint64_t key,
                                 void *stream);
int asrk_fbank_frames_batch_dither_f32(const void *wave, int sample_bytes, int64_t ld_wave,
                                       const int64_t *n_samples_host, const int64_t *frame_off, int B, int max_m,
                                       const float *window, float *frames, int win, int shift, int ldf, float scale,
                                       float preemph, int remove_dc, float dither, const uint64_t *keys, void *stream);
int asrk_fbank_logmel_batch_dither_f32(const void *wave, int sample_bytes, int64_t ld_wave,
                                       const int64_t *n_samples_host, const int64_t *frame_off, int B, int max_m,
                                       const float *window, const float *tw_fft, const float *tw_unpack,
                                       const float *melT, const int *mel_range, int nmel, int ld_mel, float *mel,
                                       int win, int shift, int log2n, float scale, float preemph, int remove_dc,
                                       float eps, float dither, const uint64_t *keys, void *stream);

int asrk_spec_augment_f32(const float *x, float *y, int B, int T, int ld, int D, int C, const int64_t *lens,
                          const int32_t *params, int n_fmask, int n_tmask, float fill, void *stream);

int asrk_resample_rows_f32(const void *x, int sample_bytes, int64_t ld_in, const int64_t *n_host, const int64_t *n_dev,
                           const int32_t *ratio_idx_host, const int32_t *ratio_idx_dev, int B,
                           const int32_t *ratios_host, const float *const *taps_host, int n_ratios, float *y,
                           int64_t ld_out, float scale, void *stream);

size_t asrk_reverb_mix_ws_bytes(int B, int64_t n_max);
int asrk_reverb_mix_f32(const void *x, int sample_bytes, int64_t ld_in, const int64_t *n_host, const int64_t *n_dev,
                        const float *rir, int64_t ld_r, const int32_t *rir_len_host, const int32_t *rir_len_dev,
                        const int32_t *rir_peak_host, const int32_t *rir_peak_dev, int R, const int32_t *rir_idx_host,
                        const int32_t *rir_idx_dev, const void *v, int64_t ld_v, const int64_t *m_host,
                        const int64_t *m_dev, const float *snr_lin_dev, int B, float *out, int64_t ld_out, float scale,
                        void *ws, size_t ws_bytes, void *stream);

int asrk_ctc_loss_fwd_f32(const float *lp, int64_t stride_t, int64_t stride_b, int T, int B,
                          int V, const int64_t *targets, int64_t tgt_stride, int Lmax,
                          const int64_t *input_lengths, const int64_t *target_lengths,
                          int blank, float *alpha, float *beta, float *lpg, float *nll,
                          void *stream);
int asrk_ctc_loss_bwd_f32(const float *lp, int64_t stride_t, int64_t stride_b, int T, int B,
                          int V, const int64_t *targets, int64_t tgt_stride, int Lmax,
                          const int64_t *input_lengths, const int64_t *target_lengths,
                          int blank, const float *alpha, const float *beta, const float *lpg,
                          const float *nll, const float *gscale, float *grad, int64_t g_stride_t,
                          int64_t g_stride_b, void *stream);

#define ASRK_CTC_ZERO_INFINITY 1
int asrk_ctc_loss_fwd_ex_f32(const float *lp, int64_t stride_t, int64_t stride_b, int T, int B, int V,
                             const int64_t *targets, int64_t tgt_stride, int Lmax, const int64_t *input_lengths,
                             const int64_t *target_lengths, int blank, float *alpha, float *beta, float *lpg,
                             float *nll, int flags, float *loss, int32_t *n_infeasible, void *stream);
int asrk_ctc_loss_bwd_ex_f32(const float *lp, int64_t stride_t, int64_t stride_b, int T, int B, int V,
                             const int64_t *targets, int64_t tgt_stride, int Lmax, const int64_t *input_lengths,
                             const int64_t *target_lengths, int blank, const float *alpha, const float *beta,
                             const float *lpg, const float *nll, const float *gscale, float *grad,
                             int64_t g_stride_t, int64_t g_stride_b, int flags, void *stream);

#define ASRK_ALIGN_BP_AUTO 0
#define ASRK_ALIGN_BP_LDS 1
#define ASRK_ALIGN_BP_GLOBAL 2
size_t asrk_ctc_align_ws_bytes(int B, int T, int Lmax, int flags);
int asrk_ctc_align_f32(const float *lp, int64_t stride_t, int64_t stride_b, int T, int B, int V,
                       const int64_t *targets, int64_t tgt_stride, int Lmax, const int64_t *input_lengths,
                       const int64_t *target_lengths, int blank, int flags, int32_t *states, int32_t *tokens,
                       int32_t *spans, float *score, int64_t *stamps, void *ws, size_t ws_bytes, void *stream);

int asrk_ctc_prefix_score_f32(const float *x, const float *r_prev, const int *prefix_len,
                              const int *last_char, const int *candidates, float *psi,
                              float *r_out, int n, int C, int T, int V, int blank, int eos,
                              float logzero, void *stream);
int asrk_ctc_prefix_score_multi_f32(const float *x, const int *row_mem, const int *mem_len, const float *r_prev,
                                    const int *prefix_len, const int *last_char, const int *candidates,
                                    float *psi, float *r_out, int n, int C, int T, int V, int U, int blank,
                                    int eos, float logzero, void *stream);

int asrk_flac_info(const char *path, int *sample_rate, int *channels, int *bits_per_sample,
                   int64_t *total_samples, uint8_t *md5_16);
int asrk_flac_decode_i32(const char *path, int32_t *out, int64_t capacity_samples,
                         int64_t *decoded_samples);

#ifdef __cplusplus
}
#endif
#endif
```

Baseline: 552,400 frames/s.

## Emit transposed activation panels from LSTM backward kernel and park dW_ih GEMMs

The bf16-split LSTM backward recurrence kernel now recomputes h = o*tanh(c) and writes split-bf16 transposed panels of the layer output (YT), and of the pyramid-reshaped input of the next layer up (XT), alongside the existing dG panels. The upper layer's input-weight gradient GEMM is parked until the lower layer's backward runs, so it can consume the XT panel emitted there instead of building a separate transposed panel from x. This removes separate transpose/split passes over activations, in exchange for extra LDS, extra global stores inside the latency-critical recurrent loop, and more complex deferral bookkeeping in Python.

```diff
diff --git a/end-to-end-asr-pytorch_amd/_lib.py b/end-to-end-asr-pytorch_amd/_lib.py
--- a/end-to-end-asr-pytorch_amd/_lib.py
+++ b/end-to-end-asr-pytorch_amd/_lib.py
@@ -101,6 +101,9 @@
                                                 c_vp, c_int, c_vp, c_vp, c_int, c_int, c_vp, c_int, c_vp]),
     "asrk_lstm_rec_bwd_pyr_panel_f32": (c_int, [c_vp, c_vp, c_vp, c_vp, c_vp, c_int, c_int, c_int, c_int,
                                                 c_vp, c_int, c_vp, c_vp, c_int, c_int, c_vp, c_vp, c_int, c_vp]),
+    "asrk_lstm_rec_bwd_pyr_panel2_f32": (c_int, [c_vp, c_vp, c_vp, c_vp, c_vp, c_int, c_int, c_int, c_int,
+                                                 c_vp, c_int, c_vp, c_vp, c_int, c_int, c_vp, c_vp, c_vp, c_vp, c_int,
+                                                 c_vp]),
     "asrk_gru_rec_fwd_f32": (c_int, [c_vp, c_vp, c_vp, c_vp, c_int, c_int, c_int, c_int,
                                      c_vp, c_int, c_vp, c_vp, c_int, c_int, c_int, c_vp]),
     "asrk_gru_rec_bwd_f32": (c_int, [c_vp, c_vp, c_vp, c_vp, c_vp, c_int, c_int, c_int, c_int,
diff --git a/end-to-end-asr-pytorch_amd/csrc/lstm_rec.hip b/end-to-end-asr-pytorch_amd/csrc/lstm_rec.hip
--- a/end-to-end-asr-pytorch_amd/csrc/lstm_rec.hip
+++ b/end-to-end-asr-pytorch_amd/csrc/lstm_rec.hip
@@ -189,7 +189,7 @@
                 if (!no_bf && NT == 1 && UB == 16 && BG == 16 && (H == 512 || H == 1024)) {
                     const int KS = H / 32, KL = H == 1024 ? 11 : 0;
                     best.bf = 1;
-                    best.lds = (size_t)4 * KL * 3 * 1024 + (size_t)2 * 4 * RED_PITCH * 16 + 2 * 6144 + 16;
+                    best.lds = (size_t)4 * KL * 3 * 1024 + (size_t)2 * 4 * RED_PITCH * 16 + 2 * 6144 + 1536 + 16;
                     best.xfloats = (size_t)ndir * nbg * T * ((size_t)4 * KS * 3 * 256 + canary_words(nwg));
                 }
                 return best;
@@ -229,7 +229,7 @@
 int rec_bwd_impl(bool gru, float *gates, const float *whh_f, const float *whh_r, const float *C,
                  const float *dY, int T, int B, int H, int ndir, void *xchg, int xchg_prefilled, void *ws,
                  float *db, int pyr_mode, int pyr_rate, int flags, void *stream, void *dg_panel = nullptr,
-                 void *dgt_panel = nullptr);
+                 void *dgt_panel = nullptr, void *yt_panel = nullptr, void *xt_panel = nullptr);
 
 }
 
@@ -422,15 +422,25 @@
                                                void *xchg, int xchg_prefilled, void *ws, float *db,
                                                int pyr_mode, int pyr_rate, void *dg_panel, void *dgt_panel, int flags,
                                                void *stream) {
-    if (!dg_panel && !dgt_panel) return ASRK_EINVAL;
+    return asrk_lstm_rec_bwd_pyr_panel2_f32(gates, whh_f, whh_r, C, dY, T, B, H, ndir, xchg, xchg_prefilled, ws, db,
+                                            pyr_mode, pyr_rate, dg_panel, dgt_panel, nullptr, nullptr, flags, stream);
+}
+
+extern "C" int asrk_lstm_rec_bwd_pyr_panel2_f32(float *gates, const float *whh_f, const float *whh_r,
+                                                const float *C, const float *dY, int T, int B, int H, int ndir,
+                                                void *xchg, int xchg_prefilled, void *ws, float *db,
+                                                int pyr_mode, int pyr_rate, void *dg_panel, void *dgt_panel,
+                                                void *yt_panel, void *xt_panel, int flags, void *stream) {
+    if (!dg_panel && !dgt_panel && !yt_panel && !xt_panel) return ASRK_EINVAL;
     return rec_bwd_impl(false, gates, whh_f, whh_r, C, dY, T, B, H, ndir, xchg, xchg_prefilled, ws, db,
-                        pyr_mode, pyr_rate, flags, stream, dg_panel, dgt_panel);
+                        pyr_mode, pyr_rate, flags, stream, dg_panel, dgt_panel, yt_panel, xt_panel);
 }
 
 namespace {
 int rec_bwd_impl(bool gru, float *gates, const float *whh_f, const float *whh_r, const float *C,
                  const float *dY, int T, int B, int H, int ndir, void *xchg, int xchg_prefilled, void *ws,
-                 float *db, int pyr_mode, int pyr_rate, int flags, void *stream, void *dg_panel, void *dgt_panel) {
+                 float *db, int pyr_mode, int pyr_rate, int flags, void *stream, void *dg_panel, void *dgt_panel,
+                 void *yt_panel, void *xt_panel) {
     const AsrkKnobs &kn = asrk_knobs_();
     if (flags < 0 || pyr_mode < 0 || pyr_mode > 2 || pyr_rate < 1) return ASRK_EINVAL;
     const bool dy_empty = pyr_mode == 1 && T / pyr_rate == 0;
@@ -468,6 +478,19 @@
         a.PT = reinterpret_cast<unsigned char *>(dgt_panel);
         a.pt_stride = asrk_split_panel_stride_(ndir * 4 * H, T * B);
     }
+    a.YT = a.XT = nullptr; a.yt_stride = a.xt_stride = 0;
+    if (yt_panel) {
+        if (!pl.bf || gru || B % 16 != 0 || (reinterpret_cast<uintptr_t>(yt_panel) & 15)) return ASRK_ESHAPE;
+        a.YT = reinterpret_cast<unsigned char *>(yt_panel);
+        a.yt_stride = asrk_split_panel_stride_(ndir * H, T * B);
+    }
+    if (xt_panel) {
+        if (!pl.bf || gru || B % 16 != 0 || (reinterpret_cast<uintptr_t>(xt_panel) & 15) || pyr_mode != 1 ||
+            T / pyr_rate == 0)
+            return ASRK_ESHAPE;
+        a.XT = reinterpret_cast<unsigned char *>(xt_panel);
+        a.xt_stride = asrk_split_panel_stride_(pyr_rate * ndir * H, (T / pyr_rate) * B);
+    }
     const bool one_launch = pl.ndir_l >= ndir && pl.nbg_l >= pl.nbg;
     a.rearm = (flags & ASRK_REC_REARM) && one_launch ? 1 : 0;
     a.no_dg = (flags & ASRK_REC_BWD_NO_DG) && (dg_panel || dgt_panel) ? 1 : 0;
diff --git a/end-to-end-asr-pytorch_amd/csrc/lstm_rec_bwd_bf.hip b/end-to-end-asr-pytorch_amd/csrc/lstm_rec_bwd_bf.hip
--- a/end-to-end-asr-pytorch_amd/csrc/lstm_rec_bwd_bf.hip
+++ b/end-to-end-asr-pytorch_amd/csrc/lstm_rec_bwd_bf.hip
@@ -3,7 +3,7 @@
 namespace asrk_rec {
 namespace {
 
-template <bool GRU, int KS, int NREG>
+template <bool GRU, int KS, int NREG, bool ACT>
 __global__ __launch_bounds__(256) void lstm_rec_bwd_bf_kernel(RecBwdArgs p) {
     extern __shared__ __attribute__((aligned(16))) float smem[];
     constexpr int CH = 8;
@@ -23,7 +23,8 @@
     f32x4 *red = reinterpret_cast<f32x4 *>(Wl + (size_t)4 * KL * 3 * 1024);
     unsigned char *stage = reinterpret_cast<unsigned char *>(red + 2 * 4 * RED_PITCH);
     unsigned char *stage_t = stage + 4 * 3 * 2 * 16 * 16;
-    int *abort_flag = reinterpret_cast<int *>(stage_t + 4 * 3 * 2 * 16 * 16);
+    unsigned char *stage_h = stage_t + 4 * 3 * 2 * 16 * 16;
+    int *abort_flag = reinterpret_cast<int *>(stage_h + 3 * 2 * 16 * 16);
 
     const int m16 = lane & 15, q4 = lane >> 4;
     bf16x8_t areg[NREG > 0 ? NREG : 1][3];
@@ -94,6 +95,29 @@
         pt_dst[i] = (size_t)(row >> 6) * p.pt_stride + (size_t)pl * 1024 + (row & 63) * 16;
         pt_half[i] = hb;
     }
+    constexpr bool act_panels = !GRU && ACT;
+    const bool tail_image = !GRU && (p.PT || act_panels);
+    auto emit_act = [&](int tt) {
+        if (tid >= 128 && tid < 224) {
+            const int k = tid - 128, hb = (k >> 4) & 1, pl = k >> 5;
+            const int yrow = dir * H + u0 + (k & 15);
+            const u32x4 v = *reinterpret_cast<const u32x4 *>(stage_h + k * 16);
+            if (p.YT) {
+                const int c = (tt * p.B + b0 + hb * 8) >> 3;
+                *reinterpret_cast<u32x4 *>(p.YT + (size_t)(yrow >> 6) * p.yt_stride + (size_t)c * 3072 + pl * 1024 +
+                                           (yrow & 63) * 16) = v;
+            }
+            if (p.XT) {
+                const int r = p.pyr_rate, tq = tt / r, tr = tt - tq * r;
+                if (tq < p.T / r) {
+                    const int row = tr * p.ldy + yrow;
+                    const int c = (tq * p.B + b0 + hb * 8) >> 3;
+                    *reinterpret_cast<u32x4 *>(p.XT + (size_t)(row >> 6) * p.xt_stride + (size_t)c * 3072 + pl * 1024 +
+                                               (row & 63) * 16) = v;
+                }
+            }
+        }
+    };
     const int xks = u0 >> 5, xq4 = (u0 & 31) >> 3;
     int ch_src[2], pg_row[2];
     unsigned ch_dst[2];
@@ -161,6 +185,7 @@
 
         REC_STAMP(0);
         if (s > 0) {
+            if (act_panels) emit_act(dir == 0 ? t + 1 : t - 1);
             __amdgpu_buffer_rsrc_t rs = __builtin_amdgcn_make_buffer_rsrc(
                 (void *)(xgroup + (size_t)(s - 1) * step_floats), 0, (int)(step_floats * 4), 0x00020000);
             u32x4 bf[CH][3];
@@ -241,6 +266,7 @@
         const float *redf = reinterpret_cast<const float *>(redw);
         float *xstep = xgroup + (size_t)s * step_floats;
         float dgs[4] = {0.f, 0.f, 0.f, 0.f}, xg[4] = {0.f, 0.f, 0.f, 0.f};
+        float hval = 0.f;
         if (c_valid) {
             float rec = 0.f;
 #pragma unroll
@@ -257,6 +283,7 @@
             } else {
                 const float dh = vdy + rec;
                 const float tc = fast_tanh(vc);
+                if (ACT) hval = vo * tc;
                 const float dcell = dh * vo * (1.f - tc * tc) + dc_carry;
                 dc_carry = dcell * vf;
                 dgs[0] = dcell * vg * vi * (1.f - vi);
@@ -307,26 +334,36 @@
                     }
             }
         }
+        if (act_panels) {
+            unsigned h0, h1, h2;
+            split3(hval, h0, h1, h2);
+            *reinterpret_cast<unsigned short *>(st_t + 12 * 512) = (unsigned short)h0;
+            *reinterpret_cast<unsigned short *>(st_t + 13 * 512) = (unsigned short)h1;
+            *reinterpret_cast<unsigned short *>(st_t + 14 * 512) = (unsigned short)h2;
+        }
         REC_STAMP(5);
         if (c_valid && !p.no_dg) {
             float *g = p.G + ((size_t)t * p.B + c_b) * p.ldg + dir * 4 * H + c_unit;
 #pragma unroll
             for (int r = 0; r < 4; ++r) g[(size_t)r * H] = dgs[r];
         }
-        if (!GRU && p.PT) {
+        if (tail_image) {
             __syncthreads();
-#pragma unroll
-            for (int i = 0; i < 2; ++i)
-                if (pt_on[i]) {
-                    const int c = (t * p.B + b0 + pt_half[i] * 8) >> 3;
-                    *reinterpret_cast<u32x4 *>(p.PT + pt_dst[i] + (size_t)c * 3072) =
-                        *reinterpret_cast<const u32x4 *>(stage_t + pt_src[i]);
-                }
+            if (p.PT) {
+#pragma unroll
+                for (int i = 0; i < 2; ++i)
+                    if (pt_on[i]) {
+                        const int c = (t * p.B + b0 + pt_half[i] * 8) >> 3;
+                        *reinterpret_cast<u32x4 *>(p.PT + pt_dst[i] + (size_t)c * 3072) =
+                            *reinterpret_cast<const u32x4 *>(stage_t + pt_src[i]);
+                    }
+            }
         }
         if (p.rearm && s >= 2)
             rearm_region(xgroup + (size_t)(s - 2) * step_floats, step_floats, wg, p.nwg, tid, (int)blockDim.x);
         REC_STAMP(6);
     }
+    if (act_panels && p.T > 0 && !*abort_flag) emit_act(dir == 0 ? 0 : p.T - 1);
     if (p.db && !*abort_flag) {
         __syncthreads();
         float *sdb = reinterpret_cast<float *>(red);
@@ -342,9 +379,9 @@
     }
 }
 
-template <bool GRU, int KS, int NREG>
+template <bool GRU, int KS, int NREG, bool ACT>
 int launch_bwd_bf(const RecBwdArgs &a, int grid, size_t lds, hipStream_t s) {
-    auto kern = lstm_rec_bwd_bf_kernel<GRU, KS, NREG>;
+    auto kern = lstm_rec_bwd_bf_kernel<GRU, KS, NREG, ACT>;
     ASRK_HIP(hipFuncSetAttribute(reinterpret_cast<const void *>(kern),
                                  hipFuncAttributeMaxDynamicSharedMemorySize, (int)lds));
     hipLaunchKernelGGL(kern, dim3(grid), dim3(256), lds, s, a);
@@ -355,8 +392,14 @@
 }
 
 int launch_bwd_bf(bool gru, const RecBwdArgs &a, const BwdPlan &pl, int grid, hipStream_t s) {
-    if (a.H == 1024) return gru ? launch_bwd_bf<true, 32, 21>(a, grid, pl.lds, s) : launch_bwd_bf<false, 32, 21>(a, grid, pl.lds, s);
-    return gru ? launch_bwd_bf<true, 16, 16>(a, grid, pl.lds, s) : launch_bwd_bf<false, 16, 16>(a, grid, pl.lds, s);
+    const bool act = !gru && (a.YT || a.XT);
+    if (a.H == 1024)
+        return gru ? launch_bwd_bf<true, 32, 21, false>(a, grid, pl.lds, s)
+                   : act ? launch_bwd_bf<false, 32, 21, true>(a, grid, pl.lds, s)
+                         : launch_bwd_bf<false, 32, 21, false>(a, grid, pl.lds, s);
+    return gru ? launch_bwd_bf<true, 16, 16, false>(a, grid, pl.lds, s)
+               : act ? launch_bwd_bf<false, 16, 16, true>(a, grid, pl.lds, s)
+                     : launch_bwd_bf<false, 16, 16, false>(a, grid, pl.lds, s);
 }
 
 }
diff --git a/end-to-end-asr-pytorch_amd/csrc/lstm_rec_common.h b/end-to-end-asr-pytorch_amd/csrc/lstm_rec_common.h
--- a/end-to-end-asr-pytorch_amd/csrc/lstm_rec_common.h
+++ b/end-to-end-asr-pytorch_amd/csrc/lstm_rec_common.h
@@ -48,6 +48,8 @@
     size_t pg_stride;
     unsigned char *PT;
     size_t pt_stride;
+    unsigned char *YT, *XT;
+    size_t yt_stride, xt_stride;
 };
 
 #define REC_STAMP_W(ph)                                                                       \
diff --git a/end-to-end-asr-pytorch_amd/ops.py b/end-to-end-asr-pytorch_amd/ops.py
--- a/end-to-end-asr-pytorch_amd/ops.py
+++ b/end-to-end-asr-pytorch_amd/ops.py
@@ -166,7 +166,7 @@
         _lib.check(rc, "lstm grid sync")
 
 
-_defer = {"enabled": True, "side": {}, "pending": {}, "cb_armed": False, "release": []}
+_defer = {"enabled": True, "side": {}, "pending": {}, "cb_armed": False, "release": [], "parked": {}}
 
 
 def set_deferred_weight_grads(flag):
@@ -187,8 +187,40 @@
     return _defer["side"].get(dev) if dev in _defer["pending"] else None
 
 
+def _arm_end_of_backward():
+    if not _defer["cb_armed"]:
+        try:
+            torch.autograd.Variable._execution_engine.queue_callback(_end_of_backward)
+            _defer["cb_armed"] = True
+        except RuntimeError:
+            return False
+    return True
+
+
+def _park_dw_ih(rec):
+    _defer["parked"][rec["x"].data_ptr()] = rec
+    if not _arm_end_of_backward():
+        _flush_dw_ih(_defer["parked"].pop(rec["x"].data_ptr()))
+
+
+def _flush_dw_ih(rec, xt=None):
+    M, Din = rec["M"], rec["Din"]
+    with torch.cuda.stream(rec["stream"]):
+        pXT = xt if xt is not None else SplitPanel(rec["x"], Din, Din, M, True)
+        for rows, m0, out in rec["gemms"]:
+            gemm_panels(rows, Din, M, rec["pGT"], m0, 0, pXT, 0, 0, out, Din)
+    for pnl in rec["release"]:
+        if _defer["pending"]:
+            _defer["release"].append(pnl)
+        else:
+            pnl.release()
+
+
 def _end_of_backward():
     _defer["cb_armed"] = False
+    parked, _defer["parked"] = _defer["parked"], {}
+    for rec in parked.values():
+        _flush_dw_ih(rec)
     join_deferred()
     rel, _defer["release"] = _defer["release"], []
     for pnl in rel:
@@ -272,12 +304,8 @@
         done = torch.cuda.Event()
         done.record(self.side)
         _defer["pending"][self.device] = done
-        if not _defer["cb_armed"]:
-            try:
-                torch.autograd.Variable._execution_engine.queue_callback(_end_of_backward)
-                _defer["cb_armed"] = True
-            except RuntimeError:
-                join_deferred()
+        if not _arm_end_of_backward():
+            join_deferred()
         return False
 
 
@@ -342,13 +370,15 @@
 import weakref as _weakref
 _REC_PANELS = _os.environ.get("ASRK_REC_PANELS", "1") != "0"
 _REC_SKIP_DG = True
+_REC_ACT_PANELS = _os.environ.get("ASRK_REC_ACT_PANELS", "1") != "0"
 _panel_pool = {"free": {}, "bytes": 0, "tick": 0, "seen": {}, "stats": {"hit": 0, "miss": 0, "skipped": 0, "evicted": 0}}
 _panel_state = {"hint": False, "handover": None,
-                "stats": {"emitted": 0, "consumed": 0, "dg": 0, "dgt": 0, "no_dg": 0, "dw_ih_splitk": 0}}
+                "stats": {"emitted": 0, "consumed": 0, "dg": 0, "dgt": 0, "no_dg": 0, "dw_ih_splitk": 0, "yt": 0, "xt": 0,
+                          "parked": 0}}
 
 
 class _BlankPanel:
-    __slots__ = ("buf", "rows", "K", "flags", "key")
+    __slots__ = ("buf", "rows", "K", "flags", "key", "mode")
 
     @staticmethod
     def take(rows, K, device):
@@ -373,7 +403,7 @@
         return _BlankPanel(rows, K, key, buf)
 
     def __init__(self, rows, K, key, buf):
-        self.rows, self.K, self.flags, self.key, self.buf = rows, K, 0, key, buf
+        self.rows, self.K, self.flags, self.key, self.buf, self.mode = rows, K, 0, key, buf, 0
 
     def release(self):
         n = self.buf.numel()
@@ -712,11 +742,11 @@
 SIDE_REVERSE = "SIDE_REVERSE"
 IH_PANELS, IH_SPLITK, IH_F32 = "panels", "panels_splitk", "f32"
 LstmBwdPlan = collections.namedtuple("LstmBwdPlan", "pG pGT db_in_kernel skip_dg rows_ih dw_ih_route dw_hh_panels "
-                                                    "schedule defer_release")
+                                                    "schedule defer_release pYT pXT park_dw_ih")
 
 
 def lstm_bwd_plan(T, B, Din, H, ndir, has_bias, needs_dx, stacked, can_defer, to_scratch, beside_bptt, bf_bwd, share_env,
-                  skip_dg_switch, takes_split, take_panel):
+                  skip_dg_switch, takes_split, take_panel, take_act_panel=None, x_from_concat_panel=False, xt_wanted=None):
     M = T * B
     pG = pGT = None
     if bf_bwd and needs_dx and stacked and takes_split(M, Din, 8 * H):
@@ -744,7 +774,16 @@
         schedule = SIDE_REVERSE_SHARED
     panels = bool(share0) and schedule != SIDE_REVERSE
     route = IH_SPLITK if narrow_ih else IH_PANELS if panels and wide_ih else IH_F32
-    return LstmBwdPlan(pG, pGT, db_in_kernel, skip_dg, rows_ih, route, panels, schedule, schedule == SIDE_REVERSE_SHARED)
+    pYT = pXT = None
+    if take_act_panel is not None and pGT is not None:
+        if panels:
+            pYT = take_act_panel(ndir * H, M)
+        if xt_wanted is not None:
+            pXT = take_act_panel(*xt_wanted)
+    park = bool(take_act_panel is not None and x_from_concat_panel and pGT is not None and schedule == STREAM
+                and route == IH_PANELS and can_defer and to_scratch)
+    return LstmBwdPlan(pG, pGT, db_in_kernel, skip_dg, rows_ih, route, panels, schedule, schedule == SIDE_REVERSE_SHARED,
+                       pYT, pXT, park)
 
 
 class LSTMLayerFn(Function):
@@ -763,6 +802,7 @@
         G = torch.empty((M, ndir * 4 * H), dtype=torch.float32, device=dev)
         w_ih_f, w_hh_f = _f32c(w_ih_f), _f32c(w_hh_f)
         w_stack = None
+        ctx.x_from_concat_panel = False
         if ndir == 2:
             w_ih_r, w_hh_r = _f32c(w_ih_r), _f32c(w_hh_r)
         if ndir == 2 and H >= 768 and _os.environ.get("ASRK_STACK_DIRS", "1") != "0":
@@ -787,6 +827,7 @@
                 gemm_panels(M, 8 * H, Din, x_panel, 0, 0, pW, 0, 0, G, 8 * H, bias=b1, bias2=b2)
                 del pW
                 _panel_state["stats"]["consumed"] += 1
+                ctx.x_from_concat_panel = x_panel.mode == 1
             else:
                 gemm(0, 1, M, 8 * H, Din, xc, Din, w_stack, Din, G, 8 * H, bias=b1, bias2=b2)
             if x_panel is not None:
@@ -809,6 +850,7 @@
             out_panel = _BlankPanel.take((T // r_) * B, r_ * ndir * H, dev)
         if out_panel is not None:
             _panel_state["stats"]["emitted"] += 1
+            out_panel.mode = mode
             _lib.check(L.asrk_lstm_rec_fwd_pyr_panel_f32(_p(G), _p(w_hh_f), _p(w_hh_r), _p(Y), _p(C), T, B, H, ndir,
                                                          _p(xc_.buf), xc_.prefilled, _p(ws), _p(Y2), mode, rate,
                                                          _p(out_panel.buf), xc_.flags, _stream()), "lstm_rec_fwd")
@@ -824,6 +866,7 @@
         ctx.save_for_backward(xc, w_ih_f, w_hh_f, w_ih_r, w_hh_r, G, C, Y, w_stack)
         ctx.consumed = False
         out = Y2 if mode else Y.view(T, B, ndir * H)
+        ctx.out_ptr = out.data_ptr() if mode == 1 and out.numel() else None
         if _panel_state["handover"] is not None:
             _panel_state["handover"][2].release()
             _panel_state["handover"] = None
@@ -847,31 +890,47 @@
         ws = lstm_workspace(dev)
         needs_dx = ctx.needs_input_grad[0]
         w_ih, w_hh = (w_ih_f, w_ih_r), (w_hh_f, w_hh_r)
+        parked = _defer["parked"].get(ctx.out_ptr) if ctx.out_ptr is not None else None
+        if parked is not None and not (parked["x"]._version == parked["version"] and
+                                       tuple(parked["x"].shape) == (T // rate, B, rate * ldy) and
+                                       parked["stream"] == torch.cuda.current_stream(dev)):
+            parked = None
         with _bptt_launch(L, T, B, H, ndir, ctx.has_bias, G, dev) as (xc_, db_all):
             plan = lstm_bwd_plan(T, B, Din, H, ndir, ctx.has_bias, needs_dx, w_stack is not None,
                                  _can_defer(w_ih_f, w_hh_f, w_ih_r, w_hh_r, *ctx.bias_refs),
                                  not grad_has_destination(*w_ih[:ndir]), _defer_beside_bptt(),
                                  bool(_REC_PANELS and L.asrk_lstm_plan_is_bf(T, B, H, ndir, 1, rec_flags(1))),
                                  _os.environ.get("ASRK_SHARE_PANELS", "1") != "0", _REC_SKIP_DG, gemm_takes_split,
-                                 lambda rows, K: _BlankPanel.take(rows, K, dev))
-            pG, pGT = plan.pG, plan.pGT
+                                 lambda rows, K: _BlankPanel.take(rows, K, dev),
+                                 (lambda rows, K: _BlankPanel.take(rows, K, dev)) if _REC_ACT_PANELS else None,
+                                 ctx.x_from_concat_panel,
+                                 (rate * ldy, (T // rate) * B) if parked is not None else None)
+            pG, pGT, pYT, pXT = plan.pG, plan.pGT, plan.pYT, plan.pXT
             stats = _panel_state["stats"]
             stats["dg"] += pG is not None
             stats["dgt"] += pGT is not None
             stats["no_dg"] += plan.skip_dg
             stats["dw_ih_splitk"] += (plan.dw_ih_route == IH_SPLITK) * (1 if plan.rows_ih == 8 * H else ndir)
+            stats["yt"] += pYT is not None
+            stats["xt"] += pXT is not None
             db = db_all if plan.db_in_kernel else None
             if pG is not None or pGT is not None:
-                _lib.check(L.asrk_lstm_rec_bwd_pyr_panel_f32(_p(G), _p(w_hh_f), _p(w_hh_r), _p(C), _p(dYc), T, B, H,
-                                                             ndir, _p(xc_.buf), xc_.prefilled, _p(ws), _p(db), mode, rate,
-                                                             _p(pG.buf if pG is not None else None),
-                                                             _p(pGT.buf if pGT is not None else None),
-                                                             xc_.flags | (ASRK_REC_BWD_NO_DG if plan.skip_dg else 0),
-                                                             _stream()), "lstm_rec_bwd")
+                _lib.check(L.asrk_lstm_rec_bwd_pyr_panel2_f32(_p(G), _p(w_hh_f), _p(w_hh_r), _p(C), _p(dYc), T, B, H,
+                                                              ndir, _p(xc_.buf), xc_.prefilled, _p(ws), _p(db), mode, rate,
+                                                              _p(pG.buf if pG is not None else None),
+                                                              _p(pGT.buf if pGT is not None else None),
+                                                              _p(pYT.buf if pYT is not None else None),
+                                                              _p(pXT.buf if pXT is not None else None),
+                                                              xc_.flags | (ASRK_REC_BWD_NO_DG if plan.skip_dg else 0),
+                                                              _stream()), "lstm_rec_bwd")
             else:
                 _lib.check(L.asrk_lstm_rec_bwd_pyr_f32(_p(G), _p(w_hh_f), _p(w_hh_r), _p(C), _p(dYc), T, B, H,
                                                        ndir, _p(xc_.buf), xc_.prefilled, _p(ws), _p(db), mode, rate,
                                                        xc_.flags, _stream()), "lstm_rec_bwd")
+        if parked is not None:
+            _flush_dw_ih(_defer["parked"].pop(ctx.out_ptr), pXT)
+            if pXT is not None:
+                pXT.release()
         dG = G
         f32 = dict(dtype=torch.float32, device=dev)
         dx = None
@@ -890,6 +949,9 @@
                     gemm(0, 0, M, Din, 4 * H, dG[:, 4 * H:], ldg, w_ih_r, Din, dx, Din, beta=1.0)
             dx = dx.view(T, B, Din)
         panels = {} if pGT is None else {"dGT": pGT}
+        if pYT is not None:
+            panels["YT"] = pYT
+        parked_gemms = []
         dw_ih_stack = []
 
         def panel(name, src, ld, rows):
@@ -905,7 +967,10 @@
             if not (stacked and dw_ih_stack):
                 out = torch.empty((8 * H, Din), **f32) if stacked else grad_out(w_ih[d], (4 * H, Din), dev)
                 m0 = 0 if stacked else d * 4 * H
-                if plan.dw_ih_route == IH_F32:
+                if plan.park_dw_ih:
+                    alias = torch.empty(0, **f32).set_(out.untyped_storage(), out.storage_offset(), out.shape, out.stride())
+                    parked_gemms.append((plan.rows_ih, m0, alias))
+                elif plan.dw_ih_route == IH_F32:
                     gemm(1, 0, plan.rows_ih, Din, M, dG[:, m0:], ldg, xc, Din, out, Din)
                 else:
                     dg_gemm(plan.rows_ih, Din, M, m0, 0, panel("XT", xc, Din, Din), 0, 0, out, Din,
@@ -955,7 +1020,16 @@
                 g1 = param_grads(1)
                 side.keep(*g1)
             grads = [param_grads(0), g1]
-        if pGT is not None:
+        if pYT is not None:
+            if plan.defer_release or _defer["pending"]:
+                _defer["release"].append(pYT)
+            else:
+                pYT.release()
+        if parked_gemms:
+            stats["parked"] += 1
+            _park_dw_ih({"x": xc, "version": xc._version, "stream": torch.cuda.current_stream(dev), "M": M, "Din": Din,
+                         "pGT": pGT, "gemms": parked_gemms, "release": [pGT]})
+        elif pGT is not None:
             if plan.defer_release or _defer["pending"]:
                 _defer["release"].append(pGT)
             else:
diff --git a/include/asrk.h b/include/asrk.h
--- a/include/asrk.h
+++ b/include/asrk.h
@@ -128,6 +128,11 @@
                                     const float *dY, int T, int B, int H, int ndir, void *xchg,
                                     int xchg_prefilled, void *ws, float *db, int pyr_mode, int pyr_rate,
                                     void *dg_panel, void *dgt_panel, int flags, void *stream);
+int asrk_lstm_rec_bwd_pyr_panel2_f32(float *gates, const float *whh_f, const float *whh_r, const float *C,
+                                     const float *dY, int T, int B, int H, int ndir, void *xchg,
+                                     int xchg_prefilled, void *ws, float *db, int pyr_mode, int pyr_rate,
+                                     void *dg_panel, void *dgt_panel, void *yt_panel, void *xt_panel, int flags,
+                                     void *stream);
 int asrk_lstm_rec_fwd_len_f32(float *G, const float *whh_f, const float *whh_r, float *Y, float *C,
                               const int64_t *lens, int T, int B, int H, int ndir, void *xchg,
                               int xchg_prefilled, void *ws, float *Y2, int pyr_mode, int pyr_rate, int flags,
```

New measurement: 555,800 frames/s, median of 6. Within noise of the previous version (+0.6%).
